# oss0430/SRFRD

Measured on NVIDIA B200. Metric: training seqs/sec; full-catalogue top-10 users/sec, higher is better.
Workload: dtype bf16

## Files before the change

### include/srfrd_b200.h

```cpp
#ifndef SRFRD_B200_H
#define SRFRD_B200_H

#include <stddef.h>
#include <stdint.h>

#ifdef __cplusplus
extern "C" {
#endif

#define SRFRD_ABI_VERSION 9
#if defined(__GNUC__)
#define SRFRD_API __attribute__((visibility("default")))
#else
#define SRFRD_API
#endif

SRFRD_API const char* srfrd_last_error(void);
SRFRD_API int srfrd_abi_version(void);
SRFRD_API int srfrd_device_check(void);

SRFRD_API int srfrd_embed_ln_fwd(const float* item_table, int64_t n_rows, int D, const float* pos_table,
                       const float* aux_table, int64_t n_aux, int F, int mode, const int64_t* seq,
                       const int64_t* aux_ids, int64_t B, int L, float item_scale, const float* ln_w,
                       const float* ln_b, float eps, void* x0_bf16, float* x0_f32, void* q_bf16, float* stats,
                       int ldx, float drop_p, uint64_t drop_seed, uint32_t drop_stream, const float* drop_step,
                       void* stream);

SRFRD_API int srfrd_srfu_labels(const int64_t* fake_ids, int64_t B, int L, int kind, int64_t* labels, void* stream);

SRFRD_API int srfrd_embed_bwd(const void* dx0_bf16, int ldx, const int64_t* seq, const int64_t* aux_ids, int64_t B, int L,
                    int D, int F, int mode, float item_scale, float* d_item, float* d_aux, void* stream);

SRFRD_API int srfrd_layernorm_fwd(const void* x_bf16, int ldx, const float* w, const float* b, float eps, void* y_bf16,
                        float* y_f32, int ldy, float* stats, int64_t T, int H, int64_t row_stride,
                        int64_t row_offset, void* stream);
SRFRD_API int srfrd_layernorm_bwd(const void* dy_bf16, const float* dy_f32, int lddy, const void* x_bf16, int ldx,
                        const float* stats, const float* w, const void* add_bf16, int ldadd,
                        const int64_t* row_ids, void* dx_bf16, int lddx, float* dw, float* db, int64_t T, int H,
                        void* stream);

typedef struct {
  const float* bias;
  const void* residual;
  const void* gate;
  const int64_t* row_ids;
  void* out_bf16;
  float* out_f32;
  int ldr, ldg, ldc;
  int relu;
  float drop_p;
  uint32_t drop_stream;
  uint64_t drop_seed;
  const float* drop_step;
  void* ln_out_bf16;
  const float* ln_w;
  const float* ln_b;
  float* ln_stats;
  int ld_ln;
  float ln_eps;
} srfrd_gemm_epilogue_t;

SRFRD_API int srfrd_gemm_tn(const void* A_bf16, int lda, const void* B_bf16, int ldb, int M, int N, int K,
                  const srfrd_gemm_epilogue_t* ep, void* stream);
SRFRD_API int srfrd_gemm_tn_plan(int M, int N, int K, int has_aux, int bf16_out, int fused_ln, int* out);
SRFRD_API int srfrd_gemm_debug_read(long long* host_dst);
SRFRD_API int srfrd_attn_debug_read(long long* host_dst);

SRFRD_API int srfrd_gemm_wgrad(const void* dY_bf16, int lda, const void* X_bf16, int ldb, int64_t T, int Mo, int No,
                     float* dW, int ldw, float* dbias, void* stream);
SRFRD_API int srfrd_gemm_ref(const void* A, int lda, const void* B, int ldb, float* C, int ldc, int M, int N, int K,
                   int a_mn_major, int b_mn_major, void* stream);

SRFRD_API int srfrd_colsum(const void* X_bf16, int64_t M, int N, int64_t ld, float* out, void* stream);
SRFRD_API int srfrd_add_segments(float* in, int64_t n, int seg_in, int seg_out, float* out, void* stream);

SRFRD_API int srfrd_dropout_apply(const void* x_bf16, int ldx, void* out_bf16, int ldo, int64_t M, int N, float drop_p,
                        uint64_t seed, uint32_t stream_id, const float* drop_step, void* stream);

typedef struct {
  const float* src; int src_ld;
  void* dst; int dst_ld;
  void* dst_t; int dst_t_ld;
  int rows, cols;
  int dst_is_f32;
} srfrd_cast_desc_t;
SRFRD_API int srfrd_cast_weights(const srfrd_cast_desc_t* descs_dev, int n, void* stream);
SRFRD_API int srfrd_f32_to_bf16_split(const float* src, int64_t src_ld, const int64_t* row_index, void* hi, void* lo,
                            int64_t rows, int cols, int dst_ld, void* stream);

SRFRD_API int srfrd_attention_fwd(const void* q, int ldq, const void* k, const void* v, int ldkv, void* o, int ldo,
                        float* stats, int64_t B, int L, int H, int heads, float drop_p, uint64_t seed, uint32_t stream_id,
                        const float* drop_step, void* stream);
SRFRD_API int srfrd_attention_bwd(const void* dout, int lddo, const void* q, int ldq, const void* k, const void* v, int ldkv,
                        const void* o, int ldo, float* stats, void* dq, int lddq, void* dk, void* dv, int lddkv, int64_t B,
                        int L, int H, int heads, float drop_p, uint64_t seed, uint32_t stream_id, const float* drop_step,
                        void* stream);

SRFRD_API int srfrd_score_fwd(const float* h, int ldh, const float* item_table, const float* fake_table, const int64_t* pos,
                    const int64_t* neg, const int64_t* prs, const int64_t* nrs, int64_t T, int D, int F, float* zp,
                    float* zn, void* stream);
SRFRD_API int srfrd_score_bwd(const float* h, int ldh, const float* item_table, const float* fake_table, const int64_t* pos,
                    const int64_t* neg, const int64_t* prs, const int64_t* nrs, const float* dzp, const float* dzn,
                    int64_t T, int D, int F, float* dh, int lddh, float* d_item, float* d_fake, void* stream);
SRFRD_API int srfrd_score_loss_fused(const float* h, int ldh, const float* item_table, const float* fake_table,
                           const int64_t* pos, const int64_t* neg, const int64_t* prs, const int64_t* nrs,
                           const float* w_pos, const float* w_neg, const float* norm, int64_t T, int D, int F,
                           float* zp, float* zn, float* loss_acc, float* dh, int lddh, float* d_item, float* d_fake,
                           void* stream);
SRFRD_API int srfrd_weight_sums(const int64_t* pos, const float* w_pos, const float* w_neg, int64_t T, float* out2,
                      void* stream);
SRFRD_API int srfrd_loss_finalize(float* acc2, const float* norm2, float* loss, void* stream);

SRFRD_API int srfrd_adam_tick(float* state3, float beta1, float beta2, void* stream);
SRFRD_API int srfrd_adam_step(float* p, float* g, float* m, float* v, int64_t n, float lr, float beta1, float beta2, float eps,
                    const float* state3, int zero_grad, void* stream);

SRFRD_API int srfrd_adam_step_fused(float* p, float* g, float* m, float* v, int64_t n, float lr, float beta1, float beta2,
                          float eps, float* state8, int zero_grad, float* acc2, const float* norm2, float* loss,
                          void* stream, const int64_t* l2_seg, int l2_n_seg, const float* l2_coef, const float* l2_reg);

SRFRD_API int srfrd_param_l2_plan(const int64_t* seg_host, int n_seg, int64_t* n_chunks);
SRFRD_API int srfrd_param_l2(const float* p, const int64_t* seg, int n_seg, int64_t n_chunks, float l2, float* coef,
                   float* reg, double* ws, void* stream);

#define SRFRD_TOPK_KMAX 64
SRFRD_API int srfrd_catalogue_topk_plan(int64_t U, int64_t n_rows, int64_t row_lo, int D, int n_split, int* chunks_out,
                                        int k);
SRFRD_API int srfrd_catalogue_topk_kmax(int D, int n_split, int* kmax_out);
SRFRD_API int srfrd_catalogue_topk(const void* feats_bf16, int64_t U, int64_t u_pad, int n_split, const void* table_bf16,
                         int64_t n_rows, int64_t row_lo, int64_t id_base, int D, int ld_feats, int ld_table,
                         int chunks, float* part_scores, int* part_ids, float* packed_out, void* stream, int k);
SRFRD_API int srfrd_merge_topk(const float* scores, const int* ids, int64_t U, int nlists, int k, float* out_scores,
                     int64_t* out_ids, void* stream);
SRFRD_API int srfrd_merge_topk_packed(const float* packed, int64_t U, int nlists, int k, float* out_scores,
                            int64_t* out_ids, void* stream);
SRFRD_API int srfrd_catalogue_rank(const void* feats_bf16, int64_t U, int64_t u_pad, int n_split,
                                   const void* table_bf16, int64_t n_rows, int64_t row_lo, int64_t id_base,
                                   int D, int ld_feats, int ld_table,
                                   const void* target_rows_bf16, int ld_target, const int64_t* target_ids,
                                   float* target_scores, int* rank_out, void* stream);

SRFRD_API int srfrd_sample_batch(const int64_t* offsets, const int* items, const int8_t* labels, const float* p_fake,
                       const int* eligible, int n_eligible, int itemnum, int B, int L, int policy, uint64_t seed,
                       const float* step, int64_t* users, int64_t* seq, int64_t* rsq, int64_t* pos, int64_t* prs,
                       int64_t* neg, int64_t* nrs, float* w_pos, void* stream);

SRFRD_API int srfrd_sample_candidates(const int64_t* offsets, const int* items, const int* users0, const int* target,
                            int64_t U, int itemnum, int C, uint64_t seed, int64_t* cand, void* stream);
SRFRD_API int srfrd_candidate_rank(const float* feats, int ldf, const float* item_table, int64_t n_rows, int D,
                         const int64_t* cand, int64_t U, int C, const float* fake_table, int F,
                         const int64_t* user_label, float* logits, int ldl, int* rank, int* err_flag, void* stream);
SRFRD_API int srfrd_add_user_term(float* logits, int ldl, int64_t U, int I, const float* feats_tail, int ldf,
                        const float* fake_table, const int64_t* label, int F, void* stream);

typedef struct {
  int* rows;
  int* cnt;
  int* seq_first;
  int* tok_row;
  int* row_tok;
  int64_t* row_ids;
  int* row_info;
  int* tile_row0;
  int* last_row;
  int64_t cap;
} srfrd_pack_t;
SRFRD_API int srfrd_pack_plan(const int64_t* seq, const int64_t* keep, int64_t B, int L, const srfrd_pack_t* pk, void* stream);
SRFRD_API int srfrd_set_row_limit(const int* rows_dev);
SRFRD_API int srfrd_embed_ln_fwd_packed(const float* item_table, int64_t n_rows, int D, const float* pos_table,
                              const float* aux_table, int64_t n_aux, int F, int mode, const int64_t* seq,
                              const int64_t* aux_ids, int64_t B, int L, float item_scale, const float* ln_w,
                              const float* ln_b, float eps, void* x0_bf16, void* q_bf16, float* stats, int ldx,
                              float drop_p, uint64_t drop_seed, uint32_t drop_stream, const float* drop_step,
                              const int* row_tok, const int* rows_dev, int64_t cap_rows, void* stream);
SRFRD_API int srfrd_layernorm_fwd_rows(const void* x_bf16, int ldx, const float* w, const float* b, float eps, float* y_f32,
                             int ldy, const int* row_index, int64_t n, int H, void* stream);
SRFRD_API int srfrd_attention_packed_supported(int L, int H, int heads);
SRFRD_API int srfrd_attention_packed_oproj_supported(int L, int H, int heads);
SRFRD_API int srfrd_attention_fwd_packed(const void* q, int ldq, const void* k, const void* v, int ldkv, void* o, int ldo,
                               const srfrd_pack_t* pk, int L, int H, int heads, float drop_p, uint64_t seed,
                               uint32_t stream_id, const float* drop_step, void* stream, const void* wo, int ldw,
                               const float* bo, const void* res, int ldres, const float* ln_w, const float* ln_b,
                               float ln_eps, float* ln_stats, void* r, int ldr, void* y, int ldy);
SRFRD_API int srfrd_attention_bwd_packed(const void* dout, int lddo, const void* q, int ldq, const void* k, const void* v,
                               int ldkv, void* dq, int lddq, void* dk, void* dv, int lddkv, const srfrd_pack_t* pk,
                               int L, int H, int heads, float drop_p, uint64_t seed, uint32_t stream_id,
                               const float* drop_step, void* stream, const void* dr, int lddr, const void* woT, int ldw);
SRFRD_API int srfrd_score_loss_fused_packed(const float* h, int ldh, const float* item_table, const float* fake_table,
                                  const int64_t* pos, const int64_t* neg, const int64_t* prs, const int64_t* nrs,
                                  const float* w_pos, const float* w_neg, const float* norm, int D, int F,
                                  float* loss_acc, float* dh, int lddh, float* d_item, float* d_fake,
                                  const int* row_tok, const int* rows_dev, int64_t cap_rows, void* stream);
SRFRD_API int srfrd_embed_bwd_packed(const void* dx0_bf16, int ldx, const int64_t* seq, const int64_t* aux_ids,
                           const int* row_tok, const int* rows_dev, int64_t cap_rows, int L, int D, int F, int mode,
                           float item_scale, float* d_item, float* d_aux, float* d_pos, void* stream);

typedef struct {
  const float* bias1; const float* bias2;
  const void* gate; int ldg;
  int relu1;
  float drop1_p, drop2_p; uint32_t drop1_stream, drop2_stream; uint64_t drop_seed; const float* drop_step;
  const void* residual; int ldr;
  int residual_is_a;
  const int64_t* row_ids;
  void* mid_out; int ldm;
  void* out; int ldc;
  void* ln_out; int ld_ln; const float* ln_w; const float* ln_b; float* ln_stats; float ln_eps;
} srfrd_mlp2_t;
SRFRD_API int srfrd_mlp2_tn(const void* A_bf16, int lda, const void* W1_bf16, int ldw1, const void* W2_bf16, int ldw2, int M, int N,
                  const srfrd_mlp2_t* ep, void* stream);

SRFRD_API int srfrd_attention_live_items(const int* tok_row, int64_t B, int L, int heads, int* q_lo, int* items, int* n_live,
                               void* stream);
SRFRD_API int srfrd_set_attention_live(const int* q_lo, const int* items, const int* n_live, const int* tok_row);

typedef struct {
  const void* src; int ld_s;
  void* dst; int ld_d;
  int W;
  int mode;
} srfrd_repack_part_t;
SRFRD_API int srfrd_unpack_rows(const srfrd_repack_part_t* parts, int n_parts, const srfrd_pack_t* pk, int64_t B, int L,
                      void* stream);
SRFRD_API int srfrd_pack_rows(const srfrd_repack_part_t* parts, int n_parts, const srfrd_pack_t* pk, int64_t B, int L,
                    void* stream);

SRFRD_API int srfrd_dp_adam_step(float* const* grad_ptrs_dev, float* const* param_ptrs_dev, uint32_t* const* signal_ptrs_dev,
                       int rank, int world, int64_t n, float* m, float* v, float lr, float beta1, float beta2, float eps,
                       float* state8, const float* norm2, uint32_t* local4, void* stream, const int64_t* l2_seg,
                       int l2_n_seg, const float* l2_coef, const float* l2_reg);

#ifdef __cplusplus
}
#endif
#endif
```

### srfrd_b200/_lib.py

```python
from __future__ import annotations

import ctypes as C
import os

_HERE = os.path.dirname(os.path.abspath(__file__))
LIB_PATH = os.environ.get("SRFRD_B200_LIB") or os.path.join(_HERE, "lib", "libsrfrd_b200.so")

vp, i32, i64, f32, u32, u64 = C.c_void_p, C.c_int, C.c_int64, C.c_float, C.c_uint32, C.c_uint64


class GemmEpilogue(C.Structure):
    _fields_ = [("bias", vp), ("residual", vp), ("gate", vp), ("row_ids", vp), ("out_bf16", vp), ("out_f32", vp),
                ("ldr", i32), ("ldg", i32), ("ldc", i32), ("relu", i32), ("drop_p", f32), ("drop_stream", u32),
                ("drop_seed", u64), ("drop_step", vp),
                ("ln_out_bf16", vp), ("ln_w", vp), ("ln_b", vp), ("ln_stats", vp), ("ld_ln", i32), ("ln_eps", f32)]


class CastDesc(C.Structure):
    _fields_ = [("src", vp), ("src_ld", i32), ("dst", vp), ("dst_ld", i32), ("dst_t", vp), ("dst_t_ld", i32),
                ("rows", i32), ("cols", i32), ("dst_is_f32", i32)]


class Mlp2Epilogue(C.Structure):
    _fields_ = [("bias1", vp), ("bias2", vp), ("gate", vp), ("ldg", i32), ("relu1", i32), ("drop1_p", f32), ("drop2_p", f32),
                ("drop1_stream", u32), ("drop2_stream", u32), ("drop_seed", u64), ("drop_step", vp), ("residual", vp), ("ldr", i32),
                ("residual_is_a", i32), ("row_ids", vp), ("mid_out", vp), ("ldm", i32), ("out", vp), ("ldc", i32),
                ("ln_out", vp), ("ld_ln", i32), ("ln_w", vp), ("ln_b", vp), ("ln_stats", vp), ("ln_eps", f32)]


class PackDesc(C.Structure):
    _fields_ = [("rows", vp), ("cnt", vp), ("seq_first", vp), ("tok_row", vp), ("row_tok", vp), ("row_ids", vp),
                ("row_info", vp), ("tile_row0", vp), ("last_row", vp), ("cap", i64)]


class RepackPart(C.Structure):
    _fields_ = [("src", vp), ("ld_s", i32), ("dst", vp), ("ld_d", i32), ("W", i32), ("mode", i32)]


SIGNATURES = {
    "srfrd_abi_version": [],
    "srfrd_device_check": [],
    "srfrd_embed_ln_fwd": [vp, i64, i32, vp, vp, i64, i32, i32, vp, vp, i64, i32, f32, vp, vp, f32, vp, vp, vp, vp, i32,
                           f32, u64, u32, vp, vp],
    "srfrd_srfu_labels": [vp, i64, i32, i32, vp, vp],
    "srfrd_embed_bwd": [vp, i32, vp, vp, i64, i32, i32, i32, i32, f32, vp, vp, vp],
    "srfrd_layernorm_fwd": [vp, i32, vp, vp, f32, vp, vp, i32, vp, i64, i32, i64, i64, vp],
    "srfrd_layernorm_bwd": [vp, vp, i32, vp, i32, vp, vp, vp, i32, vp, vp, i32, vp, vp, i64, i32, vp],
    "srfrd_gemm_tn": [vp, i32, vp, i32, i32, i32, i32, C.POINTER(GemmEpilogue), vp],
    "srfrd_mlp2_tn": [vp, i32, vp, i32, vp, i32, i32, i32, C.POINTER(Mlp2Epilogue), vp],
    "srfrd_gemm_tn_plan": [i32, i32, i32, i32, i32, i32, vp],
    "srfrd_gemm_debug_read": [vp],
    "srfrd_attn_debug_read": [vp],
    "srfrd_gemm_wgrad": [vp, i32, vp, i32, i64, i32, i32, vp, i32, vp, vp],
    "srfrd_gemm_ref": [vp, i32, vp, i32, vp, i32, i32, i32, i32, i32, i32, vp],
    "srfrd_colsum": [vp, i64, i32, i64, vp, vp],
    "srfrd_add_segments": [vp, i64, i32, i32, vp, vp],
    "srfrd_dropout_apply": [vp, i32, vp, i32, i64, i32, f32, u64, u32, vp, vp],
    "srfrd_cast_weights": [vp, i32, vp],
    "srfrd_f32_to_bf16_split": [vp, i64, vp, vp, vp, i64, i32, i32, vp],
    "srfrd_attention_fwd": [vp, i32, vp, vp, i32, vp, i32, vp, i64, i32, i32, i32, f32, u64, u32, vp, vp],
    "srfrd_attention_bwd": [vp, i32, vp, i32, vp, vp, i32, vp, i32, vp, vp, i32, vp, vp, i32, i64, i32, i32, i32, f32, u64,
                            u32, vp, vp],
    "srfrd_score_fwd": [vp, i32, vp, vp, vp, vp, vp, vp, i64, i32, i32, vp, vp, vp],
    "srfrd_score_bwd": [vp, i32, vp, vp, vp, vp, vp, vp, vp, vp, i64, i32, i32, vp, i32, vp, vp, vp],
    "srfrd_score_loss_fused": [vp, i32, vp, vp, vp, vp, vp, vp, vp, vp, vp, i64, i32, i32, vp, vp, vp, vp, i32, vp, vp, vp],
    "srfrd_weight_sums": [vp, vp, vp, i64, vp, vp],
    "srfrd_loss_finalize": [vp, vp, vp, vp],
    "srfrd_adam_tick": [vp, f32, f32, vp],
    "srfrd_adam_step": [vp, vp, vp, vp, i64, f32, f32, f32, f32, vp, i32, vp],
    "srfrd_adam_step_fused": [vp, vp, vp, vp, i64, f32, f32, f32, f32, vp, i32, vp, vp, vp, vp, vp, i32, vp, vp],
    "srfrd_param_l2_plan": [C.POINTER(i64), i32, C.POINTER(i64)],
    "srfrd_param_l2": [vp, vp, i32, i64, f32, vp, vp, vp, vp],
    "srfrd_catalogue_topk_plan": [i64, i64, i64, i32, i32, C.POINTER(i32), i32],
    "srfrd_catalogue_topk_kmax": [i32, i32, C.POINTER(i32)],
    "srfrd_catalogue_topk": [vp, i64, i64, i32, vp, i64, i64, i64, i32, i32, i32, i32, vp, vp, vp, vp, i32],
    "srfrd_merge_topk_packed": [vp, i64, i32, i32, vp, vp, vp],
    "srfrd_catalogue_rank": [vp, i64, i64, i32, vp, i64, i64, i64, i32, i32, i32, vp, i32, vp, vp, vp, vp],
    "srfrd_attention_live_items": [vp, i64, i32, i32, vp, vp, vp, vp],
    "srfrd_set_attention_live": [vp, vp, vp, vp],
    "srfrd_merge_topk": [vp, vp, i64, i32, i32, vp, vp, vp],
    "srfrd_unpack_rows": [C.POINTER(RepackPart), i32, C.POINTER(PackDesc), i64, i32, vp],
    "srfrd_pack_rows": [C.POINTER(RepackPart), i32, C.POINTER(PackDesc), i64, i32, vp],
    "srfrd_dp_adam_step": [vp, vp, vp, i32, i32, i64, vp, vp, f32, f32, f32, f32, vp, vp, vp, vp, vp, i32, vp, vp],
    "srfrd_pack_plan": [vp, vp, i64, i32, C.POINTER(PackDesc), vp],
    "srfrd_set_row_limit": [vp],
    "srfrd_embed_ln_fwd_packed": [vp, i64, i32, vp, vp, i64, i32, i32, vp, vp, i64, i32, f32, vp, vp, f32, vp, vp, vp, i32,
                                  f32, u64, u32, vp, vp, vp, i64, vp],
    "srfrd_layernorm_fwd_rows": [vp, i32, vp, vp, f32, vp, i32, vp, i64, i32, vp],
    "srfrd_attention_packed_supported": [i32, i32, i32],
    "srfrd_attention_packed_oproj_supported": [i32, i32, i32],
    "srfrd_attention_fwd_packed": [vp, i32, vp, vp, i32, vp, i32, C.POINTER(PackDesc), i32, i32, i32, f32, u64, u32, vp, vp,
                                   vp, i32, vp, vp, i32, vp, vp, f32, vp, vp, i32, vp, i32],
    "srfrd_attention_bwd_packed": [vp, i32, vp, i32, vp, vp, i32, vp, i32, vp, vp, i32, C.POINTER(PackDesc), i32, i32, i32,
                                   f32, u64, u32, vp, vp, vp, i32, vp, i32],
    "srfrd_score_loss_fused_packed": [vp, i32, vp, vp, vp, vp, vp, vp, vp, vp, vp, i32, i32, vp, vp, i32, vp, vp, vp, vp,
                                      i64, vp],
    "srfrd_embed_bwd_packed": [vp, i32, vp, vp, vp, vp, i64, i32, i32, i32, i32, f32, vp, vp, vp, vp],
    "srfrd_sample_candidates": [vp, vp, vp, vp, i64, i32, i32, u64, vp, vp],
    "srfrd_candidate_rank": [vp, i32, vp, i64, i32, vp, i64, i32, vp, i32, vp, vp, i32, vp, vp, vp],
    "srfrd_add_user_term": [vp, i32, i64, i32, vp, i32, vp, vp, i32, vp],
    "srfrd_sample_batch": [vp, vp, vp, vp, vp, i32, i32, i32, i32, i32, u64, vp, vp, vp, vp, vp, vp, vp, vp, vp, vp],
}

_lib = None
_device_ok = False
launch_count = 0


def load() -> C.CDLL:
    global _lib
    if _lib is not None:
        return _lib
    if not os.path.exists(LIB_PATH):
        raise RuntimeError(
            f"srfrd_b200: {LIB_PATH} is not built. Run `make -C srfrd_b200/csrc` (needs nvcc, sm_100a). "
            "There is no CPU fallback.")
    lib = C.CDLL(LIB_PATH)
    lib.srfrd_last_error.restype = C.c_char_p
    lib.srfrd_last_error.argtypes = []
    for name, argtypes in SIGNATURES.items():
        fn = getattr(lib, name)
        fn.argtypes = argtypes
        fn.restype = C.c_int
    if lib.srfrd_abi_version() != 9:
        raise RuntimeError("srfrd_b200: ABI version mismatch between _lib.py and the built library")
    _lib = lib
    return lib


def require_device() -> None:
    global _device_ok
    if _device_ok:
        return
    lib = load()
    if lib.srfrd_device_check() != 0:
        raise RuntimeError("srfrd_b200: " + lib.srfrd_last_error().decode())
    _device_ok = True


_profile = None


def set_profile(records) -> None:
    global _profile
    _profile = records


def call(name: str, *args) -> None:
    global launch_count
    lib = _lib or load()
    if _profile is not None:
        import torch
        e0, e1 = torch.cuda.Event(enable_timing=True), torch.cuda.Event(enable_timing=True)
        e0.record()
        rc = getattr(lib, name)(*args)
        e1.record()
        _profile.append((name, args, e0, e1))
    else:
        rc = getattr(lib, name)(*args)
    if rc != 0:
        raise RuntimeError(f"{name}: {lib.srfrd_last_error().decode()}")
    launch_count += 1
```

### srfrd_b200/csrc/ffn.cu

```cuda
#include <stdlib.h>

#include "common.cuh"
#include "srfrd_b200.h"

namespace srfrd {

static constexpr int MLP_THREADS = 160;
static constexpr int MT = 128;
static constexpr int MBLK = MT * 64 * 2;

struct MlpParams {
  int M, N, kb;
  int K, kbk;
  int single;
  int relu2; const bf16* gate2; int ldg2;
  const int* rows_dev;
  const float *bias1, *bias2;
  const bf16* gate; int ldg;
  int relu1;
  uint64_t drop_seed; const float* drop_step;
  uint32_t thresh1, thresh2, stream1, stream2; float scale1, scale2;
  const bf16* residual; int ldr;
  int residual_is_a;
  const int64_t* row_ids;
  const float *ln_w, *ln_b; float* ln_stats; float ln_eps; int has_ln;
};

__device__ __forceinline__ uint32_t swz_chunk(int r, int j) { return (uint32_t)(r * 128 + ((j ^ (r & 7)) << 4)); }
__device__ __forceinline__ void mlp_bar_sync() { asm volatile("bar.sync 1, 128;" ::: "memory"); }
__device__ __forceinline__ void mlp_tma_store(const CUtensorMap* tmap, const void* smem_src, int c0, int c1) {
  asm volatile("cp.async.bulk.tensor.2d.global.shared::cta.bulk_group [%0, {%2, %3}], [%1];" ::"l"(tmap),
               "r"(smem_u32(smem_src)), "r"(c0), "r"(c1)
               : "memory");
}
__device__ __forceinline__ void unpack8_bf16(const uint4& u, float* f) {
  const uint32_t w[4] = {u.x, u.y, u.z, u.w};
#pragma unroll
  for (int i = 0; i < 4; ++i) { f[2 * i] = __uint_as_float(w[i] << 16); f[2 * i + 1] = __uint_as_float(w[i] & 0xffff0000u); }
}

__global__ void __launch_bounds__(MLP_THREADS, 2)
mlp2_kernel(const __grid_constant__ CUtensorMap tmA, const __grid_constant__ CUtensorMap tmW1,
            const __grid_constant__ CUtensorMap tmW2, const __grid_constant__ CUtensorMap tmMid,
            const __grid_constant__ CUtensorMap tmOut, const __grid_constant__ CUtensorMap tmLn, MlpParams p) {
  extern __shared__ uint8_t smem_raw[];
  uint8_t* smem = reinterpret_cast<uint8_t*>((reinterpret_cast<uintptr_t>(smem_raw) + 1023) & ~uintptr_t(1023));
  const int wblk = (p.N * 128 + 1023) & ~1023;
  const int ablk = max(p.kb, p.kbk);
  uint8_t* sW1 = smem;
  uint8_t* sW2 = sW1 + p.kbk * wblk;
  uint8_t* sA = sW2 + (p.single ? 0 : p.kb) * wblk;
  uint8_t* sM = sA + ablk * MBLK;
  float* sb1 = reinterpret_cast<float*>(sM + p.kb * MBLK);
  float* sb2 = sb1 + 128;
  float* slw = sb2 + 128;
  float* slb = slw + 128;
  uint64_t* bars = reinterpret_cast<uint64_t*>(slb + 128);
  uint64_t *w_full = bars, *a_full = bars + 1, *a_free = bars + 2, *acc1_full = bars + 3, *mid_ready = bars + 4,
           *acc2_full = bars + 5;
  uint32_t* tmem_slot = reinterpret_cast<uint32_t*>(bars + 6);
  const int warp = threadIdx.x >> 5, lane = threadIdx.x & 31;

  if (warp == 4 && lane == 0) {
    tma_prefetch_desc(&tmA); tma_prefetch_desc(&tmW1); tma_prefetch_desc(&tmW2); tma_prefetch_desc(&tmMid);
    tma_prefetch_desc(&tmOut);
    if (p.has_ln) tma_prefetch_desc(&tmLn);
    mbar_init(w_full, 1); mbar_init(a_full, 1); mbar_init(a_free, 1); mbar_init(acc1_full, 1); mbar_init(mid_ready, 1);
    mbar_init(acc2_full, 1);
    fence_barrier_init();
  }
  if (warp == 4) { tmem_alloc(tmem_slot, 256); tmem_relinquish(); }
  pdl_prologue_done();
  const int M = p.rows_dev ? min(p.M, __ldg(p.rows_dev)) : p.M;
  const int n_tiles = (M + MT - 1) / MT;
  for (int i = threadIdx.x; i < 128; i += blockDim.x) {
    sb1[i] = (p.bias1 && i < p.N) ? __ldg(p.bias1 + i) : 0.f;
    sb2[i] = (p.bias2 && i < p.N) ? __ldg(p.bias2 + i) : 0.f;
    slw[i] = (p.has_ln && i < p.N) ? __ldg(p.ln_w + i) : 0.f;
    slb[i] = (p.has_ln && i < p.N) ? __ldg(p.ln_b + i) : 0.f;
  }
  tc_fence_before();
  __syncthreads();
  tc_fence_after();
  const uint32_t tmem_base = *tmem_slot;
  const uint32_t tAcc1 = tmem_base, tAcc2 = tmem_base + 128;

  if (warp == 4) {
    if ((int)blockIdx.x < n_tiles && elect_one()) {
      mbar_expect_tx(w_full, (p.kbk + (p.single ? 0 : p.kb)) * p.N * 128);
      for (int kb = 0; kb < p.kbk; ++kb) tma_load_2d(sW1 + kb * wblk, &tmW1, w_full, kb * 64, 0, SRFRD_EVICT_LAST);
      if (!p.single)
        for (int kb = 0; kb < p.kb; ++kb) tma_load_2d(sW2 + kb * wblk, &tmW2, w_full, kb * 64, 0, SRFRD_EVICT_LAST);
    }
    __syncwarp();
    const uint32_t idesc = umma_idesc_bf16(MT, p.N, 0, 0);
    const uint64_t dA = umma_smem_desc(smem_u32(sA), 0, 1024), dM = umma_smem_desc(smem_u32(sM), 0, 1024);
    const uint64_t dW1 = umma_smem_desc(smem_u32(sW1), 0, 1024), dW2 = umma_smem_desc(smem_u32(sW2), 0, 1024);
    uint32_t ph = 0;
    for (int tile = blockIdx.x; tile < n_tiles; tile += gridDim.x, ph ^= 1) {
      mbar_wait(a_free, ph ^ 1);
      if (elect_one()) {
        mbar_expect_tx(a_full, p.kbk * MBLK);
        for (int kb = 0; kb < p.kbk; ++kb) tma_load_2d(sA + kb * MBLK, &tmA, a_full, kb * 64, tile * MT, SRFRD_EVICT_FIRST);
      }
      __syncwarp();
      if (tile == (int)blockIdx.x) mbar_wait(w_full, 0);
      mbar_wait(a_full, ph);
      tc_fence_after();
      if (elect_one()) {
        for (int kb = 0; kb < p.kbk; ++kb) {
          const int ksteps = min(4, (p.K - kb * 64 + 15) / 16);
          for (int k = 0; k < ksteps; ++k)
            umma_bf16(p.single ? tAcc2 : tAcc1, dA + (uint64_t)(kb * (MBLK >> 4) + 2 * k),
                      dW1 + (uint64_t)(kb * (wblk >> 4) + 2 * k), idesc, (kb | k) != 0);
        }
        umma_commit(p.single ? acc2_full : acc1_full);
      }
      __syncwarp();
      if (p.single) continue;
      mbar_wait(mid_ready, ph);
      tc_fence_after();
      if (elect_one()) {
        for (int kb = 0; kb < p.kb; ++kb) {
          const int ksteps = min(4, (p.N - kb * 64 + 15) / 16);
          for (int k = 0; k < ksteps; ++k)
            umma_bf16(tAcc2, dM + (uint64_t)(kb * (MBLK >> 4) + 2 * k), dW2 + (uint64_t)(kb * (wblk >> 4) + 2 * k), idesc, (kb | k) != 0);
        }
        umma_commit(acc2_full);
      }
      __syncwarp();
    }
  } else {
    const int r = warp * 32 + lane;
    const uint32_t lane_off = (uint32_t)(warp * 32) << 16;
    const uint64_t seed = (p.thresh1 | p.thresh2) ? mix_seed(p.drop_seed, p.drop_step) : 0;
    const bool issuer = threadIdx.x == 0;
    uint32_t ph = 0;
    for (int tile = blockIdx.x; tile < n_tiles; tile += gridDim.x, ph ^= 1) {
      const int64_t row = (int64_t)tile * MT + r;
      const bool rok = row < M;
      if (!p.single) {
      mbar_wait(acc1_full, ph);
      tc_fence_after();
#pragma unroll 1
      for (int c = 0; c < p.N; c += 16) {
        uint32_t raw[16];
        tmem_ld16(tAcc1 + lane_off + c, raw);
        uint4 g0 = make_uint4(0, 0, 0, 0), g1 = g0;
        if (p.gate && rok) {
          const uint4* gp = reinterpret_cast<const uint4*>(p.gate + row * p.ldg + c);
          g0 = __ldg(gp); g1 = __ldg(gp + 1);
        }
        tmem_ld_wait();
        float v[16], gv[16];
        if (p.gate) { unpack8_bf16(g0, gv); unpack8_bf16(g1, gv + 8); }
#pragma unroll
        for (int i = 0; i < 16; ++i) {
          float x = __uint_as_float(raw[i]) + sb1[c + i];
          if (p.thresh1)
            x = dropout_keep(seed, p.stream1, (uint64_t)row * (uint64_t)p.N + (uint64_t)(c + i), p.thresh1) ? x * p.scale1 : 0.f;
          if (p.relu1) x = fmaxf(x, 0.f);
          if (p.gate) x = gv[i] > 0.f ? x : 0.f;
          v[i] = x;
        }
        uint8_t* blk = sM + (c >> 6) * MBLK;
        const int j = (c & 63) >> 3;
        *reinterpret_cast<uint4*>(blk + swz_chunk(r, j)) =
            make_uint4(pack_bf16x2(v[0], v[1]), pack_bf16x2(v[2], v[3]), pack_bf16x2(v[4], v[5]), pack_bf16x2(v[6], v[7]));
        *reinterpret_cast<uint4*>(blk + swz_chunk(r, j + 1)) =
            make_uint4(pack_bf16x2(v[8], v[9]), pack_bf16x2(v[10], v[11]), pack_bf16x2(v[12], v[13]), pack_bf16x2(v[14], v[15]));
      }
      tc_fence_before();
      fence_proxy_async();
      mlp_bar_sync();
      if (issuer) {
        mbar_arrive(mid_ready);
        for (int kb = 0; kb < p.kb; ++kb) mlp_tma_store(&tmMid, sM + kb * MBLK, kb * 64, tile * MT);
        asm volatile("cp.async.bulk.commit_group;" ::: "memory");
      }
      }
      const float rowm = (p.row_ids && rok) ? ((__ldg(p.row_ids + row) != 0) ? 1.f : 0.f) : 1.f;
      mbar_wait(acc2_full, ph);
      tc_fence_after();
      float ln_sum = 0.f, ln_sq = 0.f;
#pragma unroll 1
      for (int c = 0; c < p.N; c += 16) {
        uint32_t raw[16];
        tmem_ld16(tAcc2 + lane_off + c, raw);
        uint8_t* blk = sA + (c >> 6) * MBLK;
        const int j = (c & 63) >> 3;
        uint4 r0 = make_uint4(0, 0, 0, 0), r1 = r0;
        if (p.residual_is_a && c < p.K) {
          r0 = *reinterpret_cast<const uint4*>(blk + swz_chunk(r, j));
          r1 = *reinterpret_cast<const uint4*>(blk + swz_chunk(r, j + 1));
        } else if (p.residual && rok) {
          const uint4* rp = reinterpret_cast<const uint4*>(p.residual + row * p.ldr + c);
          r0 = __ldg(rp); r1 = __ldg(rp + 1);
        }
        uint4 q0 = make_uint4(0, 0, 0, 0), q1 = q0;
        if (p.gate2 && rok) {
          const uint4* gp = reinterpret_cast<const uint4*>(p.gate2 + row * p.ldg2 + c);
          q0 = __ldg(gp); q1 = __ldg(gp + 1);
        }
        tmem_ld_wait();
        float v[16], rv[16], gv2[16];
        unpack8_bf16(r0, rv); unpack8_bf16(r1, rv + 8);
        if (p.gate2) { unpack8_bf16(q0, gv2); unpack8_bf16(q1, gv2 + 8); }
#pragma unroll
        for (int i = 0; i < 16; ++i) {
          float x = __uint_as_float(raw[i]) + sb2[c + i];
          if (p.thresh2)
            x = dropout_keep(seed, p.stream2, (uint64_t)row * (uint64_t)p.N + (uint64_t)(c + i), p.thresh2) ? x * p.scale2 : 0.f;
          if (p.relu2) x = fmaxf(x, 0.f);
          if (p.gate2) x = gv2[i] > 0.f ? x : 0.f;
          x += rv[i];
          v[i] = x * rowm;
        }
        const uint4 p0 = make_uint4(pack_bf16x2(v[0], v[1]), pack_bf16x2(v[2], v[3]), pack_bf16x2(v[4], v[5]), pack_bf16x2(v[6], v[7]));
        const uint4 p1 = make_uint4(pack_bf16x2(v[8], v[9]), pack_bf16x2(v[10], v[11]), pack_bf16x2(v[12], v[13]), pack_bf16x2(v[14], v[15]));
        *reinterpret_cast<uint4*>(blk + swz_chunk(r, j)) = p0;
        *reinterpret_cast<uint4*>(blk + swz_chunk(r, j + 1)) = p1;
        if (p.has_ln) {
          float q[16];
          unpack8_bf16(p0, q); unpack8_bf16(p1, q + 8);
#pragma unroll
          for (int i = 0; i < 16; ++i) { ln_sum += q[i]; ln_sq = fmaf(q[i], q[i], ln_sq); }
        }
      }
      tc_fence_before();
      if (p.has_ln) {
        if (issuer) asm volatile("cp.async.bulk.wait_group.read 0;" ::: "memory");
        mlp_bar_sync();
        const float invn = 1.f / (float)p.N;
        const float mean = ln_sum * invn;
        const float var = fmaxf(ln_sq * invn - mean * mean, 0.f);
        const float rstd = rsqrtf(var + p.ln_eps), nb = -mean * rstd;
#pragma unroll 1
        for (int c = 0; c < p.N; c += 8) {
          const int j = (c & 63) >> 3;
          const uint4 xv = *reinterpret_cast<const uint4*>(sA + (c >> 6) * MBLK + swz_chunk(r, j));
          float q[8], y[8];
          unpack8_bf16(xv, q);
#pragma unroll
          for (int i = 0; i < 8; ++i) y[i] = fmaf(fmaf(q[i], rstd, nb), slw[c + i], slb[c + i]);
          *reinterpret_cast<uint4*>(sM + (c >> 6) * MBLK + swz_chunk(r, j)) =
              make_uint4(pack_bf16x2(y[0], y[1]), pack_bf16x2(y[2], y[3]), pack_bf16x2(y[4], y[5]), pack_bf16x2(y[6], y[7]));
        }
        if (p.ln_stats && rok) *reinterpret_cast<float2*>(p.ln_stats + 2 * row) = make_float2(mean, rstd);
      }
      fence_proxy_async();
      mlp_bar_sync();
      if (issuer) {
        for (int kb = 0; kb < p.kb; ++kb) mlp_tma_store(&tmOut, sA + kb * MBLK, kb * 64, tile * MT);
        if (p.has_ln)
          for (int kb = 0; kb < p.kb; ++kb) mlp_tma_store(&tmLn, sM + kb * MBLK, kb * 64, tile * MT);
        asm volatile("cp.async.bulk.commit_group;" ::: "memory");
        asm volatile("cp.async.bulk.wait_group.read 0;" ::: "memory");
        mbar_arrive(a_free);
      }
    }
    if (issuer) asm volatile("cp.async.bulk.wait_group 0;" ::: "memory");
  }
  tc_fence_before();
  __syncthreads();
  if (warp == 4) { tc_fence_after(); tmem_dealloc(tmem_base, 256); }
}

}

using namespace srfrd;

static int mlp_launch(MlpParams& p, const void* A, int lda, const void* W1, int ldw1, const void* W2, int ldw2, void* mid_out,
                      int ldm, void* out, int ldc, void* ln_out, int ld_ln, cudaStream_t stream) {
  p.kb = (p.N + 63) / 64; p.kbk = (p.K + 63) / 64; p.rows_dev = row_limit();
  p.has_ln = ln_out != nullptr;
  CUtensorMap tmA, tmW1, tmW2, tmMid, tmOut, tmLn;
  if (int rc = make_tmap_bf16_2d(&tmA, A, p.M, p.K, lda, MT, 64)) return rc;
  if (int rc = make_tmap_bf16_2d(&tmW1, W1, p.N, p.K, ldw1, p.N, 64)) return rc;
  tmW2 = tmW1; tmMid = tmA;
  if (!p.single) {
    if (int rc = make_tmap_bf16_2d(&tmW2, W2, p.N, p.N, ldw2, p.N, 64)) return rc;
    if (int rc = make_tmap_bf16_2d(&tmMid, mid_out, p.M, p.N, ldm, MT, 64)) return rc;
  }
  if (int rc = make_tmap_bf16_2d(&tmOut, out, p.M, p.N, ldc, MT, 64)) return rc;
  tmLn = tmOut;
  if (p.has_ln) if (int rc = make_tmap_bf16_2d(&tmLn, ln_out, p.M, p.N, ld_ln, MT, 64)) return rc;
  const int wblk = (p.N * 128 + 1023) & ~1023;
  const int ablk = p.kb > p.kbk ? p.kb : p.kbk;
  const size_t smem = 1024 + (size_t)(p.kbk + (p.single ? 0 : p.kb)) * wblk + (size_t)(ablk + p.kb) * MBLK + 4 * 128 * sizeof(float) + 128;
  static bool attr = false;
  if (!attr) {
    SRFRD_CUDA(cudaFuncSetAttribute(mlp2_kernel, cudaFuncAttributeMaxDynamicSharedMemorySize, 200 * 1024));
    attr = true;
  }
  SRFRD_REQUIRE(smem <= 200 * 1024, "mlp2_tn: shared memory %zu too large", smem);
  int64_t grid = ((int64_t)p.M + MT - 1) / MT;
  if (grid > 2 * num_sms()) grid = 2 * num_sms();
  SRFRD_CUDA(launch_pdl(mlp2_kernel, dim3((unsigned)grid), dim3(MLP_THREADS), smem, stream, tmA, tmW1, tmW2, tmMid, tmOut, tmLn, p));
  SRFRD_LAUNCH_CHECK();
  return 0;
}

namespace srfrd {
bool gemm_small_eligible(int M, int N, int K, const srfrd_gemm_epilogue_t* ep, int lda, int ldb) {
  if (!ep->out_bf16 || ep->out_f32 || N > 128 || N % 16 || K > 128 || K % 8 || lda % 8 || ldb % 8 || ep->ldc % 8) return false;
  if (((uintptr_t)ep->out_bf16 & 15) || (ep->residual && (ep->ldr % 8 || ((uintptr_t)ep->residual & 15)))) return false;
  if (ep->gate && (ep->ldg % 8 || ((uintptr_t)ep->gate & 15))) return false;
  if (ep->residual && ep->gate) return false;
  if (ep->ln_out_bf16 && (!ep->ln_w || !ep->ln_b || ep->ld_ln % 8 || ((uintptr_t)ep->ln_out_bf16 & 15))) return false;
  { const char* e = getenv("SRFRD_LEAN_GEMM"); if (!e || e[0] != '1') return false; }
  return row_limit() != nullptr || M <= 32768;
}
int gemm_small_launch(const void* A, int lda, const void* B, int ldb, int M, int N, int K, const srfrd_gemm_epilogue_t* ep,
                      cudaStream_t stream) {
  MlpParams p = {};
  p.M = M; p.N = N; p.K = K; p.single = 1;
  p.bias2 = ep->bias; p.relu2 = ep->relu; p.gate2 = (const bf16*)ep->gate; p.ldg2 = ep->ldg;
  p.residual = (const bf16*)ep->residual; p.ldr = ep->ldr;
  p.residual_is_a = (ep->residual == A && ep->ldr == lda && N <= K) ? 1 : 0;
  if (p.residual_is_a) p.residual = nullptr;
  p.row_ids = ep->row_ids;
  p.drop_seed = ep->drop_seed; p.drop_step = ep->drop_step; p.stream2 = ep->drop_stream;
  p.thresh2 = ep->drop_p > 0.f ? (uint32_t)((double)ep->drop_p * 4294967296.0) : 0;
  p.scale2 = ep->drop_p > 0.f ? 1.f / (1.f - ep->drop_p) : 1.f;
  p.scale1 = 1.f;
  p.ln_w = ep->ln_w; p.ln_b = ep->ln_b; p.ln_stats = ep->ln_stats; p.ln_eps = ep->ln_eps;
  return mlp_launch(p, A, lda, B, ldb, nullptr, 0, nullptr, 0, ep->out_bf16, ep->ldc, ep->ln_out_bf16, ep->ld_ln, stream);
}
}

extern "C" int srfrd_mlp2_tn(const void* A, int lda, const void* W1, int ldw1, const void* W2, int ldw2, int M, int N,
                             const srfrd_mlp2_t* ep, void* stream_) {
  cudaStream_t stream = (cudaStream_t)stream_;
  SRFRD_REQUIRE(A && W1 && W2 && ep && ep->mid_out && ep->out, "mlp2_tn: null pointer");
  SRFRD_REQUIRE(M > 0 && N >= 16 && N <= 128 && N % 16 == 0, "mlp2_tn: N = K must be a multiple of 16 up to 128 (got %d)", N);
  SRFRD_REQUIRE(lda % 8 == 0 && ldw1 % 8 == 0 && ldw2 % 8 == 0 && ep->ldm % 8 == 0 && ep->ldc % 8 == 0 && lda >= N && ldw1 >= N &&
                    ldw2 >= N && ep->ldm >= N && ep->ldc >= N, "mlp2_tn: bad leading dimensions");
  SRFRD_REQUIRE(!ep->gate || (ep->ldg % 8 == 0 && ((uintptr_t)ep->gate & 15) == 0), "mlp2_tn: bad gate");
  SRFRD_REQUIRE(!ep->residual || (ep->ldr % 8 == 0 && ((uintptr_t)ep->residual & 15) == 0), "mlp2_tn: bad residual");
  SRFRD_REQUIRE(!ep->ln_out || (ep->ln_w && ep->ln_b && ep->ld_ln % 8 == 0 && ep->ld_ln >= N), "mlp2_tn: bad LayerNorm arguments");
  SRFRD_REQUIRE(ep->drop1_p >= 0.f && ep->drop1_p < 1.f && ep->drop2_p >= 0.f && ep->drop2_p < 1.f, "mlp2_tn: dropout p must be in [0, 1)");
  MlpParams p = {};
  p.M = M; p.N = N; p.K = N; p.single = 0;
  p.bias1 = ep->bias1; p.bias2 = ep->bias2; p.gate = (const bf16*)ep->gate; p.ldg = ep->ldg; p.relu1 = ep->relu1;
  p.drop_seed = ep->drop_seed; p.drop_step = ep->drop_step; p.stream1 = ep->drop1_stream; p.stream2 = ep->drop2_stream;
  p.thresh1 = ep->drop1_p > 0.f ? (uint32_t)((double)ep->drop1_p * 4294967296.0) : 0;
  p.thresh2 = ep->drop2_p > 0.f ? (uint32_t)((double)ep->drop2_p * 4294967296.0) : 0;
  p.scale1 = ep->drop1_p > 0.f ? 1.f / (1.f - ep->drop1_p) : 1.f;
  p.scale2 = ep->drop2_p > 0.f ? 1.f / (1.f - ep->drop2_p) : 1.f;
  p.residual = (const bf16*)ep->residual; p.ldr = ep->ldr;
  p.residual_is_a = (ep->residual == nullptr && ep->residual_is_a) || (ep->residual == A && ep->ldr == lda);
  if (p.residual_is_a) p.residual = nullptr;
  p.row_ids = ep->row_ids;
  p.ln_w = ep->ln_w; p.ln_b = ep->ln_b; p.ln_stats = ep->ln_stats; p.ln_eps = ep->ln_eps;
  return mlp_launch(p, A, lda, W1, ldw1, W2, ldw2, ep->mid_out, ep->ldm, ep->out, ep->ldc, ep->ln_out, ep->ld_ln, stream);
}
```

### srfrd_b200/csrc/loss_scatter_adam.cu

```cuda
#include "common.cuh"
#include "srfrd_b200.h"

namespace srfrd {

static constexpr int MAXC = 16;

struct ScoreParams {
  const float* h; int ldh;
  const float* item_table;
  const float* fake_table;
  const int64_t *pos, *neg, *prs, *nrs;
  const float *w_pos, *w_neg;
  const float* norm;
  const float *dzp_in, *dzn_in;
  float *zp, *zn;
  float* loss_acc;
  float* dh; int lddh;
  float* d_item; float* d_fake;
  int64_t T; int D, F;
  int mode;
  const int* row_tok;
  const int* rows_dev;
  int group;
};

__device__ __forceinline__ float softplus(float x) { return fmaxf(x, 0.f) + log1pf(__expf(-fabsf(x))); }
__device__ __forceinline__ float sigmoidf(float x) { return 1.f / (1.f + __expf(-x)); }

template <int NC>
__global__ void __launch_bounds__(256, (NC <= 9 ? 2 : 1)) score_kernel(ScoreParams p) {
  __shared__ float red[2][8];
  pdl_prologue_done();
  const int lane = threadIdx.x & 31, warp = threadIdx.x >> 5, nw = blockDim.x >> 5;
  const int64_t warp0 = (int64_t)blockIdx.x * nw + warp, nwarps = (int64_t)gridDim.x * nw;
  const int W = p.D + (p.fake_table ? p.F : 0);
  float lp_acc = 0.f, ln_acc = 0.f;
  float inv_np = 0.f, inv_nn = 0.f;
  if (p.mode == 1) {
    const float a = __ldg(p.norm), b = __ldg(p.norm + 1);
    inv_np = a > 0.f ? 1.f / a : 0.f;
    inv_nn = b > 0.f ? 1.f / b : 0.f;
  }
  float fk1[NC], fk2[NC];
#pragma unroll
  for (int i = 0; i < NC; ++i) fk1[i] = fk2[i] = 0.f;
  const bool dh_vec = p.dh && (p.lddh == W) && (W % 4 == 0) && ((reinterpret_cast<uintptr_t>(p.dh) & 15) == 0);
  if (p.rows_dev) p.T = min(p.T, (int64_t)__ldg(p.rows_dev));
  const int G = p.group;
  for (int64_t t0 = warp0 * G; t0 < p.T; t0 += nwarps * G) {
    const int64_t tl = t0 + lane;
    bool in = lane < G && tl < p.T;
    int my_tok = 0;
    if (p.row_tok && in) { my_tok = __ldg(p.row_tok + tl); in = my_tok >= 0; }
    const int64_t my_src = p.row_tok ? (int64_t)my_tok : tl;
    int64_t my_pid = 0, my_nid = 0, my_pf = 0, my_nf = 0;
    float my_a = 0.f, my_b = 0.f;
    bool my_active = false;
    if (in) {
      my_pid = __ldg(p.pos + my_src);
      my_nid = __ldg(p.neg + my_src);
      if (p.mode == 1) {
        my_a = p.w_pos ? __ldg(p.w_pos + my_src) : (my_pid != 0 ? 1.f : 0.f);
        my_b = p.w_neg ? __ldg(p.w_neg + my_src) : my_a;
        my_active = (my_a != 0.f) || (my_b != 0.f) || p.zp;
      } else if (p.mode == 2) {
        my_a = __ldg(p.dzp_in + my_src);
        my_b = __ldg(p.dzn_in + my_src);
        my_active = (my_a != 0.f) || (my_b != 0.f);
      } else {
        my_active = true;
      }
      if (p.fake_table && my_active) { my_pf = __ldg(p.prs + my_src); my_nf = __ldg(p.nrs + my_src); }
    }
    unsigned mask = __ballot_sync(0xffffffffu, my_active);
    if (p.dh) {
      const int nrow = (int)min((int64_t)G, p.T - t0);
      if (dh_vec) {
        const int per_row = W >> 2, total = nrow * per_row;
        float4* base = reinterpret_cast<float4*>(p.dh + t0 * p.lddh);
        for (int i = lane; i < total; i += 32)
          if (!((mask >> (i / per_row)) & 1u)) base[i] = make_float4(0.f, 0.f, 0.f, 0.f);
      } else {
        for (int r = 0; r < nrow; ++r) {
          if ((mask >> r) & 1u) continue;
          for (int c = lane; c < W; c += 32) p.dh[(t0 + r) * p.lddh + c] = 0.f;
        }
      }
    }
    struct Tok {
      int64_t t, tsrc, pid, nid; int pf, nf; float ta, tb;
      float hv[NC], ep[NC], en[NC];
    };
    auto fetch = [&](Tok& k, int r) {
      k.t = t0 + r;
      k.tsrc = p.row_tok ? (int64_t)__shfl_sync(0xffffffffu, my_tok, r) : k.t;
      k.pid = __shfl_sync(0xffffffffu, my_pid, r); k.nid = __shfl_sync(0xffffffffu, my_nid, r);
      k.pf = (int)__shfl_sync(0xffffffffu, (int)my_pf, r); k.nf = (int)__shfl_sync(0xffffffffu, (int)my_nf, r);
      k.ta = __shfl_sync(0xffffffffu, my_a, r); k.tb = __shfl_sync(0xffffffffu, my_b, r);
#pragma unroll
      for (int i = 0; i < NC; ++i) {
        const int c = lane + 32 * i;
        k.hv[i] = k.ep[i] = k.en[i] = 0.f;
        if (c < W) {
          k.hv[i] = p.h[k.t * p.ldh + c];
          if (c < p.D) {
            k.ep[i] = __ldg(p.item_table + k.pid * p.D + c);
            k.en[i] = __ldg(p.item_table + k.nid * p.D + c);
          } else {
            k.ep[i] = __ldg(p.fake_table + (int64_t)k.pf * p.F + (c - p.D));
            k.en[i] = __ldg(p.fake_table + (int64_t)k.nf * p.F + (c - p.D));
          }
        }
      }
    };
    auto finish = [&](const Tok& k) {
      float sp = 0.f, sn = 0.f;
#pragma unroll
      for (int i = 0; i < NC; ++i) { sp = fmaf(k.hv[i], k.ep[i], sp); sn = fmaf(k.hv[i], k.en[i], sn); }
      const float zp = warp_sum(sp), zn = warp_sum(sn);
      if (p.zp && lane == 0) { p.zp[k.tsrc] = zp; p.zn[k.tsrc] = zn; }
      if (p.mode == 0) return;
      float dzp = k.ta, dzn = k.tb;
      if (p.mode == 1) {
        lp_acc += k.ta * softplus(-zp);
        ln_acc += k.tb * softplus(zn);
        dzp = k.ta * (sigmoidf(zp) - 1.f) * inv_np;
        dzn = k.tb * sigmoidf(zn) * inv_nn;
      }
#pragma unroll
      for (int i = 0; i < NC; ++i) {
        const int c = lane + 32 * i;
        if (c < W) {
          if (p.dh) p.dh[k.t * p.lddh + c] = dzp * k.ep[i] + dzn * k.en[i];
          if (c < p.D) {
            if (p.d_item && k.pid != 0 && dzp != 0.f) red_add_f32(p.d_item + k.pid * p.D + c, dzp * k.hv[i]);
            if (p.d_item && k.nid != 0 && dzn != 0.f) red_add_f32(p.d_item + k.nid * p.D + c, dzn * k.hv[i]);
          } else {
            const float gp = dzp * k.hv[i], gn = dzn * k.hv[i];
            fk1[i] += (k.pf == 1 ? gp : 0.f) + (k.nf == 1 ? gn : 0.f);
            fk2[i] += (k.pf == 2 ? gp : 0.f) + (k.nf == 2 ? gn : 0.f);
          }
        }
      }
    };
    if (NC <= 4) {
      if (mask) {
        Tok cur, nxt;
        { const int r = __ffs(mask) - 1; mask &= mask - 1; fetch(cur, r); }
        while (true) {
          const bool more = mask != 0;
          if (more) { const int r = __ffs(mask) - 1; mask &= mask - 1; fetch(nxt, r); }
          finish(cur);
          if (!more) break;
          cur = nxt;
        }
      }
    } else {
      while (mask) {
        const int r = __ffs(mask) - 1;
        mask &= mask - 1;
        Tok cur;
        fetch(cur, r);
        finish(cur);
      }
    }
  }
  if (p.d_fake) {
#pragma unroll
    for (int i = 0; i < NC; ++i) {
      const int c = lane + 32 * i;
      if (c >= p.D && c < W) {
        if (fk1[i] != 0.f) red_add_f32(p.d_fake + 1 * p.F + (c - p.D), fk1[i]);
        if (fk2[i] != 0.f) red_add_f32(p.d_fake + 2 * p.F + (c - p.D), fk2[i]);
      }
    }
  }
  if (p.mode == 1 && p.loss_acc) {
    if (lane == 0) { red[0][warp] = lp_acc; red[1][warp] = ln_acc; }
    __syncthreads();
    if (threadIdx.x == 0) {
      float a = 0.f, b = 0.f;
      for (int w = 0; w < nw; ++w) { a += red[0][w]; b += red[1][w]; }
      red_add_f32(p.loss_acc, a);
      red_add_f32(p.loss_acc + 1, b);
    }
  }
}

__global__ void __launch_bounds__(256) weight_sums_kernel(const int64_t* pos, const float* w_pos, const float* w_neg,
                                                          int64_t T, float* out) {
  __shared__ float red[2][8];
  float a = 0.f, b = 0.f;
  for (int64_t t = (int64_t)blockIdx.x * blockDim.x + threadIdx.x; t < T; t += (int64_t)gridDim.x * blockDim.x) {
    const float wp = w_pos ? w_pos[t] : (pos[t] != 0 ? 1.f : 0.f);
    a += wp;
    b += w_neg ? w_neg[t] : wp;
  }
  a = warp_sum(a); b = warp_sum(b);
  const int lane = threadIdx.x & 31, warp = threadIdx.x >> 5;
  if (lane == 0) { red[0][warp] = a; red[1][warp] = b; }
  __syncthreads();
  if (threadIdx.x == 0) {
    a = b = 0.f;
    for (int w = 0; w < (int)(blockDim.x >> 5); ++w) { a += red[0][w]; b += red[1][w]; }
    red_add_f32(out, a);
    red_add_f32(out + 1, b);
  }
}

__global__ void loss_finalize_kernel(float* acc, const float* norm, float* loss) {
  pdl_prologue_done();
  const float a = norm[0] > 0.f ? acc[0] / norm[0] : 0.f;
  const float b = norm[1] > 0.f ? acc[1] / norm[1] : 0.f;
  loss[0] = a + b;
  acc[0] = 0.f; acc[1] = 0.f;
}

struct EmbedBwdParams {
  const bf16* dx0; int ldx;
  const int64_t* seq;
  const int64_t* aux_ids;
  int L, D, F, mode;
  float item_scale;
  float* d_item;
  float* d_aux;
};

__global__ void embed_bwd_kernel(EmbedBwdParams p) {
  extern __shared__ int64_t ids[];
  pdl_prologue_done();
  const int64_t b = blockIdx.x;
  const int c = threadIdx.x;
  const int H = p.D + (p.mode == 1 ? p.F : 0);
  for (int l = threadIdx.x; l < p.L; l += blockDim.x) {
    ids[l] = p.seq[b * p.L + l];
    ids[p.L + l] = (p.mode == 1 && p.aux_ids) ? p.aux_ids[b * p.L + l] : 0;
  }
  __syncthreads();
  if (c >= H) return;
  float acc1 = 0.f, acc2 = 0.f, accu = 0.f;
  for (int l = 0; l < p.L; ++l) {
    const int64_t id = ids[l];
    if (id == 0) continue;
    const float v = bf2f(p.dx0[(b * p.L + l) * p.ldx + c]);
    if (c < p.D) {
      red_add_f32(p.d_item + id * p.D + c, v * p.item_scale);
      accu += v;
    } else {
      const int64_t f = ids[p.L + l];
      if (f == 1) acc1 += v;
      else if (f == 2) acc2 += v;
    }
  }
  if (p.mode == 1 && c >= p.D && p.d_aux) {
    if (acc1 != 0.f) red_add_f32(p.d_aux + 1 * p.F + (c - p.D), acc1);
    if (acc2 != 0.f) red_add_f32(p.d_aux + 2 * p.F + (c - p.D), acc2);
  }
  if (p.mode == 2 && c < p.D && p.d_aux && accu != 0.f)
    red_add_f32(p.d_aux + p.aux_ids[b] * p.D + c, accu);
}

static constexpr int EB_SLICE = 64;
__global__ void __launch_bounds__(512) embed_bwd_packed_kernel(EmbedBwdParams p, const int* row_tok, const int* rows_dev, int64_t cap,
                                                              float* d_pos) {
  extern __shared__ float spos[];
  pdl_prologue_done();
  const int x = threadIdx.x, y = threadIdx.y, RPB = blockDim.y;
  const int c = blockIdx.y * EB_SLICE + x;
  const int H = p.D + (p.mode == 1 ? p.F : 0);
  const int tid = y * blockDim.x + x, nthr = blockDim.x * blockDim.y;
  const bool pos_slice = blockIdx.y * EB_SLICE < p.D;
  if (pos_slice) for (int i = tid; i < p.L * EB_SLICE; i += nthr) spos[i] = 0.f;
  __syncthreads();
  const int64_t M = min(cap, (int64_t)__ldg(rows_dev));
  float acc1 = 0.f, acc2 = 0.f;
  for (int64_t r = (int64_t)blockIdx.x * RPB + y; r < M; r += (int64_t)gridDim.x * RPB) {
    const int tok = __ldg(row_tok + r);
    if (tok < 0 || c >= H) continue;
    const int64_t id = __ldg(p.seq + tok);
    if (id == 0) continue;
    const float v = bf2f(p.dx0[r * p.ldx + c]);
    if (c < p.D) {
      red_add_f32(p.d_item + id * p.D + c, v * p.item_scale);
      atomicAdd(&spos[(tok % p.L) * EB_SLICE + x], v);
      if (p.mode == 2 && p.d_aux) red_add_f32(p.d_aux + p.aux_ids[tok / p.L] * p.D + c, v);
    } else if (p.aux_ids) {
      const int64_t f = __ldg(p.aux_ids + tok);
      if (f == 1) acc1 += v;
      else if (f == 2) acc2 += v;
    }
  }
  if (p.mode == 1 && c >= p.D && c < H && p.d_aux) {
    if (acc1 != 0.f) red_add_f32(p.d_aux + 1 * p.F + (c - p.D), acc1);
    if (acc2 != 0.f) red_add_f32(p.d_aux + 2 * p.F + (c - p.D), acc2);
  }
  __syncthreads();
  if (d_pos && pos_slice)
    for (int i = tid; i < p.L * EB_SLICE; i += nthr) {
      const int l = i / EB_SLICE, cc = blockIdx.y * EB_SLICE + i % EB_SLICE;
      if (cc < p.D && spos[i] != 0.f) red_add_f32(d_pos + l * p.D + cc, spos[i]);
    }
}

__global__ void add_segments_kernel(float* in, int64_t n, int seg_in, int seg_out, float* out) {
  pdl_prologue_done();
  const int64_t i = (int64_t)blockIdx.x * blockDim.x + threadIdx.x;
  if (i >= n) return;
  const int c = (int)(i % seg_in);
  if (c < seg_out) out[(i / seg_in) * seg_out + c] += in[i];
  in[i] = 0.f;
}

__global__ void adam_tick_kernel(float* state, float beta1, float beta2) {
  pdl_prologue_done();
  const float step = state[0] + 1.f;
  state[0] = step;
  state[1] = (float)(1.0 - pow((double)beta1, (double)step));
  state[2] = (float)(1.0 - pow((double)beta2, (double)step));
  state[3] = __uint_as_float(__float_as_uint(state[3]) + 1u);
}

static constexpr int64_t L2_CHUNK = 8192;

__device__ __forceinline__ void l2_chunk_prefix(const int64_t* seg, int n_seg, int64_t* s_c0) {
  const int t = threadIdx.x;
  s_c0[t + 1] = t < n_seg ? (seg[2 * t + 1] + L2_CHUNK - 1) / L2_CHUNK : 0;
  if (t == 0) s_c0[0] = 0;
  __syncthreads();
  for (int d = 1; d < L2_THREADS; d <<= 1) {
    const int64_t a = t >= d ? s_c0[t + 1 - d] : 0;
    __syncthreads();
    s_c0[t + 1] += a;
    __syncthreads();
  }
}

__device__ __forceinline__ double block_sum_f64(double x, double* s_red) {
#pragma unroll
  for (int o = 16; o > 0; o >>= 1) x += __shfl_xor_sync(0xffffffffu, x, o);
  if ((threadIdx.x & 31) == 0) s_red[threadIdx.x >> 5] = x;
  __syncthreads();
  double s = 0.0;
  if (threadIdx.x == 0)
    for (int w = 0; w < L2_THREADS / 32; ++w) s += s_red[w];
  __syncthreads();
  return s;
}

__global__ void __launch_bounds__(L2_THREADS) param_l2_kernel(const float* __restrict__ p, const int64_t* __restrict__ seg,
                                                               int n_seg, int64_t n_chunks, float l2, float* coef, float* reg,
                                                               double* ws) {
  __shared__ int64_t s_c0[L2_THREADS + 1];
  __shared__ double s_red[L2_THREADS / 32];
  __shared__ double s_norm[L2_THREADS];
  __shared__ bool s_last;
  pdl_prologue_done();
  l2_chunk_prefix(seg, n_seg, s_c0);
  double* part = ws + 1;
  for (int64_t c = blockIdx.x; c < n_chunks; c += gridDim.x) {
    int lo = 0, hi = n_seg - 1;
    while (lo < hi) {
      const int mid = (lo + hi + 1) >> 1;
      if (s_c0[mid] <= c) lo = mid; else hi = mid - 1;
    }
    const int64_t off = seg[2 * lo], numel = seg[2 * lo + 1];
    const int64_t b = (c - s_c0[lo]) * L2_CHUNK;
    const int64_t e = min(numel, b + L2_CHUNK);
    const float4* p4 = reinterpret_cast<const float4*>(p + off);
    double acc = 0.0;
#pragma unroll
    for (int k = 0; k < (int)(L2_CHUNK / 4 / L2_THREADS); ++k) {
      const int64_t j = b + 4 * ((int64_t)k * L2_THREADS + threadIdx.x);
      if (j < e) {
        const float4 x = __ldcg(p4 + j / 4);
        const float xs[4] = {x.x, x.y, x.z, x.w};
#pragma unroll
        for (int q = 0; q < 4; ++q)
          if (j + q < e) acc = fma((double)xs[q], (double)xs[q], acc);
      }
    }
    const double s = block_sum_f64(acc, s_red);
    if (threadIdx.x == 0) part[c] = s;
  }
  __threadfence();
  __syncthreads();
  if (threadIdx.x == 0) s_last = atomicAdd(reinterpret_cast<unsigned*>(ws), 1u) == gridDim.x - 1;
  __syncthreads();
  if (!s_last) return;
  __threadfence();
  const int warp = threadIdx.x >> 5, lane = threadIdx.x & 31;
  for (int t = warp; t < n_seg; t += L2_THREADS / 32) {
    double s = 0.0;
    for (int64_t c = s_c0[t] + lane; c < s_c0[t + 1]; c += 32) s += __ldcg(part + c);
#pragma unroll
    for (int o = 16; o > 0; o >>= 1) s += __shfl_xor_sync(0xffffffffu, s, o);
    if (lane == 0) {
      const double nrm = sqrt(s);
      s_norm[t] = nrm;
      coef[t] = nrm > 0.0 ? (float)((double)l2 / nrm) : 0.f;
    }
  }
  __syncthreads();
  if (threadIdx.x == 0) {
    double tot = 0.0;
    for (int t = 0; t < n_seg; ++t) tot += s_norm[t];
    reg[0] = (float)((double)l2 * tot);
    *reinterpret_cast<unsigned*>(ws) = 0u;
  }
}

template <bool L2>
__global__ void __launch_bounds__(256) adam_fused_kernel(float* __restrict__ p, float* __restrict__ g, float* __restrict__ m,
                                                         float* __restrict__ v, int64_t n, float lr, float beta1, float beta2,
                                                         float eps, float* state, int zero_grad, float* acc, const float* norm,
                                                         float* loss, L2Segments l2s) {
  __shared__ float s_bc[2];
  pdl_prologue_done();
  if (threadIdx.x == 0) {
    const float step = state[0] + 1.f;
    s_bc[0] = (float)(1.0 - pow((double)beta1, (double)step));
    s_bc[1] = (float)(1.0 - pow((double)beta2, (double)step));
  }
  if (blockIdx.x == 0 && threadIdx.x == 32 && acc) {
    const float a = norm[0] > 0.f ? acc[0] / norm[0] : 0.f;
    const float b = norm[1] > 0.f ? acc[1] / norm[1] : 0.f;
    if constexpr (L2) loss[0] = a + b + l2s.reg[0];
    else loss[0] = a + b;
    acc[0] = 0.f; acc[1] = 0.f;
  }
  int64_t* s_off = nullptr;
  float* s_coef = nullptr;
  if constexpr (L2) {
    s_off = l2_smem().off;
    s_coef = l2_smem().coef;
    l2_load_starts(l2s, s_off, s_coef);
  }
  __syncthreads();
  const float step_size = lr / s_bc[0];
  const float inv_sqrt_bc2 = rsqrtf(s_bc[1]);
  const int64_t n4 = n >> 2;
  int t = 0;
  if constexpr (L2) t = l2_find(s_off, l2s.n_seg, (int64_t)blockIdx.x * blockDim.x + threadIdx.x);
  for (int64_t i = (int64_t)blockIdx.x * blockDim.x + threadIdx.x; i < n4; i += (int64_t)gridDim.x * blockDim.x) {
    float4 pp = reinterpret_cast<float4*>(p)[i], gg = reinterpret_cast<float4*>(g)[i];
    float4 mm = reinterpret_cast<float4*>(m)[i], vv = reinterpret_cast<float4*>(v)[i];
    float* pa = &pp.x; float* ga = &gg.x; float* ma = &mm.x; float* va = &vv.x;
    if constexpr (L2) {
      t = l2_advance(s_off, l2s.n_seg, t, i);
      const float c = s_coef[t];
#pragma unroll
      for (int j = 0; j < 4; ++j) ga[j] += c * pa[j];
    }
#pragma unroll
    for (int j = 0; j < 4; ++j) {
      ma[j] = beta1 * ma[j] + (1.f - beta1) * ga[j];
      va[j] = beta2 * va[j] + (1.f - beta2) * ga[j] * ga[j];
      pa[j] -= step_size * ma[j] / (sqrtf(va[j]) * inv_sqrt_bc2 + eps);
    }
    reinterpret_cast<float4*>(p)[i] = pp;
    reinterpret_cast<float4*>(m)[i] = mm;
    reinterpret_cast<float4*>(v)[i] = vv;
    if (zero_grad) reinterpret_cast<float4*>(g)[i] = make_float4(0.f, 0.f, 0.f, 0.f);
  }
  if (blockIdx.x == 0 && threadIdx.x < (n & 3)) {
    const int64_t i = (n4 << 2) + threadIdx.x;
    m[i] = beta1 * m[i] + (1.f - beta1) * g[i];
    v[i] = beta2 * v[i] + (1.f - beta2) * g[i] * g[i];
    p[i] -= step_size * m[i] / (sqrtf(v[i]) * inv_sqrt_bc2 + eps);
    if (zero_grad) g[i] = 0.f;
  }
  __syncthreads();
  if (threadIdx.x == 0) {
    int* done = reinterpret_cast<int*>(state + 4);
    if (atomicAdd(done, 1) == (int)gridDim.x - 1) {
      *done = 0;
      state[0] = state[0] + 1.f;
      state[1] = s_bc[0];
      state[2] = s_bc[1];
      state[3] = __uint_as_float(__float_as_uint(state[3]) + 1u);
    }
  }
}

__global__ void __launch_bounds__(256) adam_kernel(float* __restrict__ p, float* __restrict__ g, float* __restrict__ m,
                                                   float* __restrict__ v, int64_t n, float lr, float beta1, float beta2,
                                                   float eps, const float* __restrict__ state, int zero_grad) {
  pdl_prologue_done();
  const float step_size = lr / state[1];
  const float inv_sqrt_bc2 = rsqrtf(state[2]);
  const int64_t n4 = n >> 2;
  for (int64_t i = (int64_t)blockIdx.x * blockDim.x + threadIdx.x; i < n4; i += (int64_t)gridDim.x * blockDim.x) {
    float4 pp = reinterpret_cast<float4*>(p)[i], gg = reinterpret_cast<float4*>(g)[i];
    float4 mm = reinterpret_cast<float4*>(m)[i], vv = reinterpret_cast<float4*>(v)[i];
    float* pa = &pp.x; float* ga = &gg.x; float* ma = &mm.x; float* va = &vv.x;
#pragma unroll
    for (int j = 0; j < 4; ++j) {
      ma[j] = beta1 * ma[j] + (1.f - beta1) * ga[j];
      va[j] = beta2 * va[j] + (1.f - beta2) * ga[j] * ga[j];
      pa[j] -= step_size * ma[j] / (sqrtf(va[j]) * inv_sqrt_bc2 + eps);
    }
    reinterpret_cast<float4*>(p)[i] = pp;
    reinterpret_cast<float4*>(m)[i] = mm;
    reinterpret_cast<float4*>(v)[i] = vv;
    if (zero_grad) reinterpret_cast<float4*>(g)[i] = make_float4(0.f, 0.f, 0.f, 0.f);
  }
  if (blockIdx.x == 0 && threadIdx.x < (n & 3)) {
    const int64_t i = (n4 << 2) + threadIdx.x;
    m[i] = beta1 * m[i] + (1.f - beta1) * g[i];
    v[i] = beta2 * v[i] + (1.f - beta2) * g[i] * g[i];
    p[i] -= step_size * m[i] / (sqrtf(v[i]) * inv_sqrt_bc2 + eps);
    if (zero_grad) g[i] = 0.f;
  }
}

}

using namespace srfrd;

static int score_launch(ScoreParams& p, void* stream) {
  const int W = p.D + (p.fake_table ? p.F : 0);
  SRFRD_REQUIRE(W <= 32 * MAXC, "score: width %d unsupported", W);
  if (p.T == 0) return 0;
  if (p.group != 8) p.group = 32;
  int64_t blocks = (p.T + 8 * p.group - 1) / (8 * p.group);
  const int64_t cap = (int64_t)num_sms() * 8;
  if (blocks > cap) blocks = cap;
  const int nc = (W + 31) / 32;
#define SCORE_CALL(NC) SRFRD_CUDA(launch_pdl(score_kernel<NC>, dim3((unsigned)blocks), dim3(256), 0, (cudaStream_t)stream, p))
  if (nc <= 1) SCORE_CALL(1);
  else if (nc <= 2) SCORE_CALL(2);
  else if (nc <= 3) SCORE_CALL(3);
  else if (nc <= 4) SCORE_CALL(4);
  else if (nc <= 6) SCORE_CALL(6);
  else if (nc <= 9) SCORE_CALL(9);
  else SCORE_CALL(MAXC);
#undef SCORE_CALL
  SRFRD_LAUNCH_CHECK();
  return 0;
}

extern "C" int srfrd_score_fwd(const float* h, int ldh, const float* item_table, const float* fake_table,
                               const int64_t* pos, const int64_t* neg, const int64_t* prs, const int64_t* nrs,
                               int64_t T, int D, int F, float* zp, float* zn, void* stream) {
  SRFRD_REQUIRE(h && item_table && pos && neg && zp && zn, "score_fwd: null pointer");
  SRFRD_REQUIRE(!fake_table || (prs && nrs), "score_fwd: fake ids required with a fake table");
  ScoreParams p = {};
  p.h = h; p.ldh = ldh; p.item_table = item_table; p.fake_table = fake_table; p.pos = pos; p.neg = neg; p.prs = prs;
  p.nrs = nrs; p.T = T; p.D = D; p.F = F; p.zp = zp; p.zn = zn; p.mode = 0;
  return score_launch(p, stream);
}

extern "C" int srfrd_score_bwd(const float* h, int ldh, const float* item_table, const float* fake_table,
                               const int64_t* pos, const int64_t* neg, const int64_t* prs, const int64_t* nrs,
                               const float* dzp, const float* dzn, int64_t T, int D, int F, float* dh, int lddh,
                               float* d_item, float* d_fake, void* stream) {
  SRFRD_REQUIRE(h && item_table && pos && neg && dzp && dzn && dh, "score_bwd: null pointer");
  SRFRD_REQUIRE(!fake_table || (prs && nrs), "score_bwd: fake ids required with a fake table");
  ScoreParams p = {};
  p.h = h; p.ldh = ldh; p.item_table = item_table; p.fake_table = fake_table; p.pos = pos; p.neg = neg; p.prs = prs;
  p.nrs = nrs; p.T = T; p.D = D; p.F = F; p.dzp_in = dzp; p.dzn_in = dzn; p.dh = dh; p.lddh = lddh; p.d_item = d_item;
  p.d_fake = d_fake; p.mode = 2;
  return score_launch(p, stream);
}

extern "C" int srfrd_score_loss_fused(const float* h, int ldh, const float* item_table, const float* fake_table,
                                      const int64_t* pos, const int64_t* neg, const int64_t* prs, const int64_t* nrs,
                                      const float* w_pos, const float* w_neg, const float* norm, int64_t T, int D,
                                      int F, float* zp, float* zn, float* loss_acc, float* dh, int lddh, float* d_item,
                                      float* d_fake, void* stream) {
  SRFRD_REQUIRE(h && item_table && pos && neg && norm && loss_acc, "score_loss_fused: null pointer");
  SRFRD_REQUIRE(!fake_table || (prs && nrs), "score_loss_fused: fake ids required with a fake table");
  SRFRD_REQUIRE((zp == nullptr) == (zn == nullptr), "score_loss_fused: pass both logit outputs or neither");
  ScoreParams p = {};
  p.h = h; p.ldh = ldh; p.item_table = item_table; p.fake_table = fake_table; p.pos = pos; p.neg = neg; p.prs = prs;
  p.nrs = nrs; p.w_pos = w_pos; p.w_neg = w_neg; p.norm = norm; p.T = T; p.D = D; p.F = F; p.zp = zp; p.zn = zn;
  p.loss_acc = loss_acc; p.dh = dh; p.lddh = lddh; p.d_item = d_item; p.d_fake = d_fake; p.mode = 1;
  return score_launch(p, stream);
}

extern "C" int srfrd_score_loss_fused_packed(const float* h, int ldh, const float* item_table, const float* fake_table,
                                             const int64_t* pos, const int64_t* neg, const int64_t* prs, const int64_t* nrs,
                                             const float* w_pos, const float* w_neg, const float* norm, int D, int F,
                                             float* loss_acc, float* dh, int lddh, float* d_item, float* d_fake,
                                             const int* row_tok, const int* rows_dev, int64_t cap_rows, void* stream) {
  SRFRD_REQUIRE(h && item_table && pos && neg && norm && loss_acc && row_tok && rows_dev, "score_loss_fused_packed: null pointer");
  SRFRD_REQUIRE(!fake_table || (prs && nrs), "score_loss_fused_packed: fake ids required with a fake table");
  ScoreParams p = {};
  p.h = h; p.ldh = ldh; p.item_table = item_table; p.fake_table = fake_table; p.pos = pos; p.neg = neg; p.prs = prs;
  p.nrs = nrs; p.w_pos = w_pos; p.w_neg = w_neg; p.norm = norm; p.T = cap_rows; p.D = D; p.F = F;
  p.loss_acc = loss_acc; p.dh = dh; p.lddh = lddh; p.d_item = d_item; p.d_fake = d_fake; p.mode = 1;
  p.row_tok = row_tok; p.rows_dev = rows_dev; p.group = 8;
  return score_launch(p, stream);
}

extern "C" int srfrd_weight_sums(const int64_t* pos, const float* w_pos, const float* w_neg, int64_t T, float* out2,
                                 void* stream) {
  SRFRD_REQUIRE(pos && out2, "weight_sums: null pointer");
  SRFRD_CUDA(cudaMemsetAsync(out2, 0, 2 * sizeof(float), (cudaStream_t)stream));
  if (T == 0) return 0;
  int64_t blocks = (T + 2047) / 2048;
  if (blocks > num_sms() * 2) blocks = num_sms() * 2;
  weight_sums_kernel<<<(unsigned)blocks, 256, 0, (cudaStream_t)stream>>>(pos, w_pos, w_neg, T, out2);
  SRFRD_LAUNCH_CHECK();
  return 0;
}

extern "C" int srfrd_loss_finalize(float* acc2, const float* norm2, float* loss, void* stream) {
  SRFRD_REQUIRE(acc2 && norm2 && loss, "loss_finalize: null pointer");
  SRFRD_CUDA(launch_pdl(loss_finalize_kernel, dim3(1), dim3(1), 0, (cudaStream_t)stream, acc2, norm2, loss));
  SRFRD_LAUNCH_CHECK();
  return 0;
}

extern "C" int srfrd_embed_bwd(const void* dx0, int ldx, const int64_t* seq, const int64_t* aux_ids, int64_t B, int L,
                               int D, int F, int mode, float item_scale, float* d_item, float* d_aux, void* stream) {
  SRFRD_REQUIRE(dx0 && seq && d_item, "embed_bwd: null pointer");
  SRFRD_REQUIRE(mode >= 0 && mode <= 2, "embed_bwd: bad mode");
  SRFRD_REQUIRE(mode != 2 || aux_ids, "embed_bwd: labels required for mode 2");
  const int H = D + (mode == 1 ? F : 0);
  SRFRD_REQUIRE(H <= 1024, "embed_bwd: width %d unsupported", H);
  if (B == 0) return 0;
  EmbedBwdParams p;
  p.dx0 = (const bf16*)dx0; p.ldx = ldx; p.seq = seq; p.aux_ids = aux_ids; p.L = L; p.D = D; p.F = F; p.mode = mode;
  p.item_scale = item_scale; p.d_item = d_item; p.d_aux = d_aux;
  const int threads = (H + 31) & ~31;
  SRFRD_CUDA(launch_pdl(embed_bwd_kernel, dim3((unsigned)B), dim3(threads), 2 * L * sizeof(int64_t), (cudaStream_t)stream, p));
  SRFRD_LAUNCH_CHECK();
  return 0;
}

extern "C" int srfrd_embed_bwd_packed(const void* dx0, int ldx, const int64_t* seq, const int64_t* aux_ids,
                                      const int* row_tok, const int* rows_dev, int64_t cap_rows, int L, int D, int F,
                                      int mode, float item_scale, float* d_item, float* d_aux, float* d_pos, void* stream) {
  SRFRD_REQUIRE(dx0 && seq && d_item && row_tok && rows_dev, "embed_bwd_packed: null pointer");
  SRFRD_REQUIRE(mode >= 0 && mode <= 2, "embed_bwd_packed: bad mode");
  SRFRD_REQUIRE(mode != 2 || aux_ids, "embed_bwd_packed: labels required for mode 2");
  const int H = D + (mode == 1 ? F : 0);
  SRFRD_REQUIRE(H <= 512, "embed_bwd_packed: width %d unsupported", H);
  if (cap_rows == 0) return 0;
  EmbedBwdParams p;
  p.dx0 = (const bf16*)dx0; p.ldx = ldx; p.seq = seq; p.aux_ids = aux_ids; p.L = L; p.D = D; p.F = F; p.mode = mode;
  p.item_scale = item_scale; p.d_item = d_item; p.d_aux = d_aux;
  const int slices = (H + EB_SLICE - 1) / EB_SLICE;
  const int tx = EB_SLICE, ty = 8;
  const size_t smem = (size_t)L * EB_SLICE * sizeof(float);
  SRFRD_REQUIRE(smem <= 200 * 1024, "embed_bwd_packed: L = %d too long for the shared positional accumulator", L);
  static bool attr = false;
  if (!attr) {
    SRFRD_CUDA(cudaFuncSetAttribute(embed_bwd_packed_kernel, cudaFuncAttributeMaxDynamicSharedMemorySize, 200 * 1024));
    attr = true;
  }
  int per_sm = (int)((200 * 1024) / (smem + 1024));
  if (per_sm > 4) per_sm = 4;
  if (per_sm < 1) per_sm = 1;
  int64_t gx = ((int64_t)num_sms() * per_sm + slices - 1) / slices;
  const int64_t need = (cap_rows + ty - 1) / ty;
  if (gx > need) gx = need;
  if (gx < 1) gx = 1;
  const dim3 grid((unsigned)gx, (unsigned)slices);
  SRFRD_CUDA(launch_pdl(embed_bwd_packed_kernel, grid, dim3(tx, ty), smem, (cudaStream_t)stream, p, row_tok, rows_dev, cap_rows,
                        d_pos));
  SRFRD_LAUNCH_CHECK();
  return 0;
}

extern "C" int srfrd_add_segments(float* in, int64_t n, int seg_in, int seg_out, float* out, void* stream) {
  SRFRD_REQUIRE(in && out && seg_in > 0 && seg_out <= seg_in, "add_segments: bad arguments");
  if (n == 0) return 0;
  SRFRD_CUDA(launch_pdl(add_segments_kernel, dim3((unsigned)((n + 255) / 256)), dim3(256), 0, (cudaStream_t)stream, in, n, seg_in,
                        seg_out, out));
  SRFRD_LAUNCH_CHECK();
  return 0;
}

extern "C" int srfrd_adam_tick(float* state3, float beta1, float beta2, void* stream) {
  SRFRD_REQUIRE(state3, "adam_tick: null state");
  SRFRD_CUDA(launch_pdl(adam_tick_kernel, dim3(1), dim3(1), 0, (cudaStream_t)stream, state3, beta1, beta2));
  SRFRD_LAUNCH_CHECK();
  return 0;
}

extern "C" int srfrd_adam_step(float* p, float* g, float* m, float* v, int64_t n, float lr, float beta1, float beta2,
                               float eps, const float* state3, int zero_grad, void* stream) {
  SRFRD_REQUIRE(p && g && m && v && state3, "adam_step: null pointer");
  SRFRD_REQUIRE((((uintptr_t)p | (uintptr_t)g | (uintptr_t)m | (uintptr_t)v) & 15) == 0, "adam_step: buffers must be 16-byte aligned");
  if (n == 0) return 0;
  int64_t blocks = (n / 4 + 255) / 256;
  if (blocks < 1) blocks = 1;
  if (blocks > num_sms() * 8) blocks = num_sms() * 8;
  SRFRD_CUDA(launch_pdl(adam_kernel, dim3((unsigned)blocks), dim3(256), 0, (cudaStream_t)stream, p, g, m, v, n, lr, beta1, beta2,
                        eps, state3, zero_grad));
  SRFRD_LAUNCH_CHECK();
  return 0;
}

extern "C" int srfrd_adam_step_fused(float* p, float* g, float* m, float* v, int64_t n, float lr, float beta1, float beta2,
                                     float eps, float* state8, int zero_grad, float* acc2, const float* norm2, float* loss,
                                     void* stream, const int64_t* l2_seg, int l2_n_seg, const float* l2_coef,
                                     const float* l2_reg) {
  SRFRD_REQUIRE(p && g && m && v && state8, "adam_step_fused: null pointer");
  SRFRD_REQUIRE(!acc2 || (norm2 && loss), "adam_step_fused: the loss read-out needs norm and loss");
  SRFRD_REQUIRE((((uintptr_t)p | (uintptr_t)g | (uintptr_t)m | (uintptr_t)v) & 15) == 0, "adam_step_fused: buffers must be 16-byte aligned");
  const bool l2 = l2_seg != nullptr;
  SRFRD_REQUIRE(!l2 || (l2_coef && l2_reg && acc2), "adam_step_fused: the l2 term needs coef, reg and the loss read-out");
  SRFRD_REQUIRE(!l2 || (l2_n_seg >= 1 && l2_n_seg <= L2_THREADS && n % 4 == 0),
                "adam_step_fused: l2 needs 1..%d segments and n a multiple of 4", L2_THREADS);
  int64_t blocks = (n / 4 + 255) / 256;
  if (blocks < 1) blocks = 1;
  if (blocks > num_sms() * 8) blocks = num_sms() * 8;
  const L2Segments l2s{l2_seg, l2_n_seg, l2_coef, l2_reg};
  if (l2)
    SRFRD_CUDA(launch_pdl(adam_fused_kernel<true>, dim3((unsigned)blocks), dim3(256), 0, (cudaStream_t)stream, p, g, m, v, n,
                          lr, beta1, beta2, eps, state8, zero_grad, acc2, norm2, loss, l2s));
  else
    SRFRD_CUDA(launch_pdl(adam_fused_kernel<false>, dim3((unsigned)blocks), dim3(256), 0, (cudaStream_t)stream, p, g, m, v, n,
                          lr, beta1, beta2, eps, state8, zero_grad, acc2, norm2, loss, l2s));
  SRFRD_LAUNCH_CHECK();
  return 0;
}

extern "C" int srfrd_param_l2_plan(const int64_t* seg_host, int n_seg, int64_t* n_chunks) {
  SRFRD_REQUIRE(seg_host && n_chunks, "param_l2_plan: null pointer");
  SRFRD_REQUIRE(n_seg >= 1 && n_seg <= L2_THREADS, "param_l2_plan: %d segments (1..%d supported)", n_seg, L2_THREADS);
  int64_t c = 0, end = 0;
  for (int t = 0; t < n_seg; ++t) {
    const int64_t off = seg_host[2 * t], numel = seg_host[2 * t + 1];
    SRFRD_REQUIRE(off % 4 == 0 && off >= end && numel >= 0, "param_l2_plan: segment %d must start 4-aligned after the last", t);
    end = off + numel;
    c += (numel + L2_CHUNK - 1) / L2_CHUNK;
  }
  *n_chunks = c;
  return 0;
}

extern "C" int srfrd_param_l2(const float* p, const int64_t* seg, int n_seg, int64_t n_chunks, float l2, float* coef,
                              float* reg, double* ws, void* stream) {
  SRFRD_REQUIRE(p && seg && coef && reg && ws, "param_l2: null pointer");
  SRFRD_REQUIRE(((uintptr_t)p & 15) == 0, "param_l2: the parameter buffer must be 16-byte aligned");
  SRFRD_REQUIRE(n_seg >= 1 && n_seg <= L2_THREADS && n_chunks >= 0, "param_l2: bad segment / chunk count");
  int64_t grid = n_chunks < 1 ? 1 : n_chunks;
  if (grid > num_sms() * 8) grid = num_sms() * 8;
  SRFRD_CUDA(launch_pdl(param_l2_kernel, dim3((unsigned)grid), dim3(L2_THREADS), 0, (cudaStream_t)stream, p, seg, n_seg,
                        n_chunks, l2, coef, reg, ws));
  SRFRD_LAUNCH_CHECK();
  return 0;
}
```

### srfrd_b200/engine.py

```python
from __future__ import annotations

import math
import os
from contextlib import contextmanager, nullcontext
from dataclasses import dataclass
from typing import Dict, List, Optional, Tuple

import torch

from . import ops

bf16 = torch.bfloat16
LN_EPS = 1e-8

KINDS = ("SRFR", "SRFRN", "SRFU_B", "SRFU_F", "SRFU_R", "SASRec")


@dataclass
class ModelSpec:
    kind: str
    item_number: int
    max_len: int
    D: int
    F: int = 0
    n_labels: int = 0
    num_blocks: int = 2
    num_heads: int = 1
    dropout: float = 0.0

    def __post_init__(self):
        if self.kind not in KINDS:
            raise ValueError(f"unknown model kind {self.kind}")
        if self.H % self.num_heads:
            raise ValueError("hidden size must be divisible by num_heads")
        if (self.H // self.num_heads) % 2:
            raise ValueError(f"srfrd_b200: head width {self.H // self.num_heads} must be even (bf16 pairs)")

    @property
    def H(self) -> int:
        return self.D + self.F if self.kind in ("SRFR", "SRFRN") else self.D

    @property
    def Dout(self) -> int:
        return self.H if self.kind == "SRFRN" else self.D

    @property
    def Hp(self) -> int:
        return (self.H + 15) // 16 * 16

    @property
    def Dp(self) -> int:
        return (self.D + 15) // 16 * 16

    @property
    def Doutp(self) -> int:
        return self.Hp if self.kind == "SRFRN" else self.Dp

    @property
    def padded(self) -> bool:
        return self.Hp != self.H or self.Dp != self.D

    @property
    def mode(self) -> int:
        return 1 if self.kind in ("SRFR", "SRFRN") else (2 if self.kind.startswith("SRFU") else 0)

    @property
    def item_scale(self) -> float:
        return float(self.D ** 0.5) if self.kind == "SASRec" else 1.0

    @property
    def item_key(self) -> str:
        return "item_emb.weight" if self.kind == "SASRec" else "embedding_layer.item_embed.weight"

    @property
    def pos_key(self) -> str:
        return "pos_emb.weight" if self.kind == "SASRec" else "embedding_layer.pos_embed.weight"

    @property
    def aux_key(self) -> Optional[str]:
        if self.mode == 1:
            return "embedding_layer.fake_embed.weight"
        if self.mode == 2:
            return "embedding_layer.user_label_embed.weight"
        return None

    def param_shapes(self) -> List[Tuple[str, Tuple[int, ...]]]:
        H, D, L, N = self.H, self.D, self.max_len, self.item_number
        out: List[Tuple[str, Tuple[int, ...]]] = []
        if self.kind == "SASRec":
            out += [("item_emb.weight", (N + 1, D)), ("pos_emb.weight", (L, D))]
        elif self.mode == 1:
            out += [("embedding_layer.item_embed.weight", (N + 1, D)),
                    ("embedding_layer.fake_embed.weight", (3, self.F)),
                    ("embedding_layer.pos_embed.weight", (L, D))]
        else:
            out += [("embedding_layer.item_embed.weight", (N + 1, D)),
                    ("embedding_layer.user_label_embed.weight", (self.n_labels, D)),
                    ("embedding_layer.pos_embed.weight", (L, D))]
        for i in range(self.num_blocks):
            out += [(f"attention_layernorms.{i}.weight", (H,)), (f"attention_layernorms.{i}.bias", (H,))]
        for i in range(self.num_blocks):
            out += [(f"attention_layers.{i}.in_proj_weight", (3 * H, H)), (f"attention_layers.{i}.in_proj_bias", (3 * H,)),
                    (f"attention_layers.{i}.out_proj.weight", (H, H)), (f"attention_layers.{i}.out_proj.bias", (H,))]
        for i in range(self.num_blocks):
            out += [(f"forward_layernorms.{i}.weight", (H,)), (f"forward_layernorms.{i}.bias", (H,))]
        for i in range(self.num_blocks):
            out += [(f"forward_layers.{i}.conv1.weight", (H, H, 1)), (f"forward_layers.{i}.conv1.bias", (H,)),
                    (f"forward_layers.{i}.conv2.weight", (H, H, 1)), (f"forward_layers.{i}.conv2.bias", (H,))]
        if self.kind == "SRFR":
            out += [("last_conv.weight", (D, H, 1)), ("last_conv.bias", (D,))]
        out += [("last_layernorm.weight", (self.Dout,)), ("last_layernorm.bias", (self.Dout,))]
        return out


class FlatParams:

    def __init__(self, spec: ModelSpec, device, alloc=None):
        self.spec = spec
        self.offsets: Dict[str, Tuple[int, Tuple[int, ...]]] = {}
        off = 0
        for name, shape in spec.param_shapes():
            n = int(math.prod(shape))
            self.offsets[name] = (off, shape)
            off += (n + 3) // 4 * 4
        self.numel = off
        zeros = (lambda n: alloc(n).zero_()) if alloc is not None else (lambda n: torch.zeros(n, dtype=torch.float32, device=device))
        self.data_ext = zeros(off + 4)
        self.data = self.data_ext[:off]
        self.data_tail = self.data_ext[off:]
        self.grad_bucket = zeros(off + 4)
        self.grad = self.grad_bucket[:off]
        self.grad_tail = self.grad_bucket[off:]

    def segments(self) -> List[Tuple[int, int]]:
        return [(off, int(math.prod(shape))) for off, shape in self.offsets.values()]

    def view(self, name: str, grad: bool = False) -> torch.Tensor:
        off, shape = self.offsets[name]
        buf = self.grad if grad else self.data
        return buf[off:off + int(math.prod(shape))].view(shape)

    def mat(self, name: str, grad: bool = False) -> torch.Tensor:
        v = self.view(name, grad)
        return v.view(v.shape[0], -1)


class HotPath:

    def __init__(self, spec: ModelSpec, params: FlatParams):
        self.spec, self.P = spec, params
        self.device = params.data.device
        self._ws_tokens = 0
        self._ws: Dict[str, torch.Tensor] = {}
        self.ws_generation = 0
        self.fwd_version = 0
        self.host_drop_counter = 0
        self._build_shadows()
        self.step_state = torch.zeros(8, dtype=torch.float32, device=self.device)
        self.side = torch.cuda.Stream(device=self.device)
        self.side2 = torch.cuda.Stream(device=self.device)
        self.overlap = os.environ.get("SRFRD_OVERLAP", "1") != "0"
        self.drop_seed = 0x5EED5EED
        self.saved: Optional[dict] = None
        self._plans: Dict[Tuple[int, int], ops.PackedPlan] = {}
        self.packed_default = os.environ.get("SRFRD_PACKED", "1") != "0"
        self.fuse_ffn = os.environ.get("SRFRD_FUSE_FFN", "1") != "0"

    def _build_shadows(self):
        s, P, dev = self.spec, self.P, self.device
        H, D, Hp, Dp = s.H, s.D, s.Hp, s.Dp
        self.sh: Dict[str, torch.Tensor] = {}
        self.vsh: Dict[str, torch.Tensor] = {}
        entries = []
        zb = lambda r, c: torch.zeros(r, c, dtype=bf16, device=dev)

        def vec(name, src, n_pad, dst_off=0, dst=None):
            if not s.padded:
                return
            if dst is None:
                dst = self.vsh.setdefault(name, torch.zeros(n_pad, dtype=torch.float32, device=dev))
            entries.append((src.view(1, -1), dst[dst_off:dst_off + src.numel()].view(1, -1), None))

        for i in range(s.num_blocks):
            win = P.mat(f"attention_layers.{i}.in_proj_weight")
            bin_ = P.view(f"attention_layers.{i}.in_proj_bias")
            self.sh[f"wq{i}"] = zb(Hp, Hp)
            self.sh[f"wkv{i}"] = zb(2 * Hp, Hp)
            self.sh[f"wqT{i}"] = zb(Hp, Hp)
            self.sh[f"wkvT{i}"] = zb(Hp, 2 * Hp)
            entries.append((win[:H], self.sh[f"wq{i}"][:H, :H], self.sh[f"wqT{i}"][:H, :H]))
            entries.append((win[H:2 * H], self.sh[f"wkv{i}"][:H, :H], self.sh[f"wkvT{i}"][:H, :H]))
            entries.append((win[2 * H:], self.sh[f"wkv{i}"][Hp:Hp + H, :H], self.sh[f"wkvT{i}"][:H, Hp:Hp + H]))
            vec(f"bq{i}", bin_[:H], Hp)
            vec(f"bkv{i}", bin_[H:2 * H], 2 * Hp)
            vec(f"bkv{i}", bin_[2 * H:], 2 * Hp, dst_off=Hp)
            for tag, key in (("wo", f"attention_layers.{i}.out_proj"), ("w1", f"forward_layers.{i}.conv1"),
                             ("w2", f"forward_layers.{i}.conv2")):
                self.sh[f"{tag}{i}"] = zb(Hp, Hp)
                self.sh[f"{tag}T{i}"] = zb(Hp, Hp)
                entries.append((P.mat(key + ".weight"), self.sh[f"{tag}{i}"][:H, :H], self.sh[f"{tag}T{i}"][:H, :H]))
                vec(f"b{tag[1]}{i}", P.view(key + ".bias"), Hp)
        if s.kind == "SRFR":
            self.sh["wc"] = zb(Dp, Hp)
            self.sh["wcT"] = zb(Hp, Dp)
            entries.append((P.mat("last_conv.weight"), self.sh["wc"][:D, :H], self.sh["wcT"][:H, :D]))
            vec("bc", P.view("last_conv.bias"), Dp)
        self._cast_table, self._cast_n = ops.make_cast_table(entries, dev)
        self.shadows_version = -1

    def bias(self, tag: str, i: Optional[int] = None) -> torch.Tensor:
        s, P = self.spec, self.P
        if s.padded:
            return self.vsh[tag if i is None else f"{tag}{i}"]
        if tag == "bq":
            return P.view(f"attention_layers.{i}.in_proj_bias")[:s.H]
        if tag == "bkv":
            return P.view(f"attention_layers.{i}.in_proj_bias")[s.H:]
        if tag == "bc":
            return P.view("last_conv.bias")
        key = {"bo": f"attention_layers.{i}.out_proj.bias", "b1": f"forward_layers.{i}.conv1.bias",
               "b2": f"forward_layers.{i}.conv2.bias"}[tag]
        return P.view(key)

    def refresh_shadows(self):
        ops.cast_weights(self._cast_table, self._cast_n)

    @contextmanager
    def _branch(self, second: bool = False):
        if not self.overlap:
            yield
            return
        main = torch.cuda.current_stream()
        st = self.side2 if second else self.side
        st.wait_stream(main)
        with torch.cuda.stream(st):
            yield

    def _join(self, second: bool = False):
        if self.overlap:
            torch.cuda.current_stream().wait_stream(self.side2 if second else self.side)

    def _workspace(self, T: int, L: int) -> Dict[str, torch.Tensor]:
        if T <= self._ws_tokens:
            return self._ws
        s, dev = self.spec, self.device
        Lmax = max(L, s.max_len)
        H, nb = s.Hp, s.num_blocks
        ws: Dict[str, torch.Tensor] = {}

        def act(name, w=H, dtype=bf16):
            ws[name] = torch.zeros(T, w, dtype=dtype, device=dev)

        for i in range(nb + 1):
            act(f"x{i}")
        for i in range(nb):
            for n in ("Q", "q", "o", "r", "y", "h1"):
                act(f"{n}{i}")
            act(f"kv{i}", 2 * H)
            act(f"st1_{i}", 2, torch.float32)
            act(f"st2_{i}", 2, torch.float32)
            if Lmax > 128:
                ws[f"ast{i}"] = torch.zeros(T * s.num_heads, 4, dtype=torch.float32, device=dev)
        if s.kind == "SRFR":
            act("c", s.Dp)
        act("stF", 2, torch.float32)
        act("hfin", s.Doutp, torch.float32)
        act("dh", s.Doutp, torch.float32)
        for n in ("gA", "gC", "gD", "gX"):
            act(n)
        for i in range(nb):
            for n in ("gda1_", "gdr_", "gdq_"):
                act(f"{n}{i}")
            act(f"gdz_{i}")
            act(f"gdkv_{i}", 2 * H)
        if s.kind == "SRFR":
            act("gc", s.Dp)
        if s.dropout > 0:
            for i in range(nb):
                act(f"gE_{i}")
        ws["pos_tmp"] = torch.zeros(Lmax * H, dtype=torch.float32, device=dev)
        self._ws, self._ws_tokens = ws, T
        self.ws_generation += 1
        return ws

    def packed_ok(self, B: int, L: int) -> bool:
        return self.packed_mode(B, L) is not None

    def packed_mode(self, B: int, L: int) -> Optional[str]:
        s = self.spec
        if s.padded or s.H % 16 or s.D % 8 or B > 16384 or B < 1:
            return None
        if ops.attention_packed_supported(L, s.H, s.num_heads):
            return "tile"
        if os.environ.get("SRFRD_HYBRID", "1") != "0" and L <= 4096:
            return "hybrid"
        return None

    def _hybrid_ws(self, Td: int) -> Dict[str, torch.Tensor]:
        hw = getattr(self, "_hws", None)
        if hw is not None and hw["_rows"] >= Td:
            return hw
        s, dev = self.spec, self.device
        Hp = s.Hp
        hw = {"_rows": Td}
        z = lambda w: torch.zeros(Td, w, dtype=bf16, device=dev)
        for i in range(s.num_blocks):
            hw[f"qd{i}"], hw[f"kvd{i}"], hw[f"od{i}"] = z(Hp), z(2 * Hp), z(Hp)
        hw["dod"], hw["dqd"], hw["dkvd"] = z(Hp), z(Hp), z(2 * Hp)
        self._hws = hw
        self.ws_generation += 1
        return hw

    def _live_tiles(self, B: int, L: int) -> "ops.LiveTiles":
        key = (B, L)
        lt = getattr(self, "_lives", None)
        if lt is None:
            lt = self._lives = {}
        if key not in lt:
            if len(lt) >= 4:
                lt.clear()
                self.ws_generation += 1
            lt[key] = ops.LiveTiles(B, L, self.spec.num_heads, self.device)
        return lt[key]

    def _plan(self, B: int, L: int) -> "ops.PackedPlan":
        key = (B, L)
        if key not in self._plans:
            if len(self._plans) >= 4:
                self._plans.clear()
                self.ws_generation += 1
            self._plans[key] = ops.PackedPlan(B, L, self.device)
        return self._plans[key]

    def forward(self, seq: torch.Tensor, fake_ids: Optional[torch.Tensor], training: bool,
                last_only: bool = False, save: Optional[bool] = None, packed: bool = False,
                keep: Optional[torch.Tensor] = None) -> torch.Tensor:
        s, P = self.spec, self.P
        B, L = seq.shape
        if L > s.max_len:
            raise RuntimeError(f"sequence length {L} exceeds max_len {s.max_len} (pos_embed rows, SRFR_model.py:12)")
        if packed:
            return self._forward_packed(seq, fake_ids, training, last_only, save, keep)
        T, H, Hp, nb = B * L, s.H, s.Hp, s.num_blocks
        ws = self._workspace(T, L)
        self.fwd_version += 1
        p_drop = s.dropout if training else 0.0
        step = self.step_state[3:4] if p_drop > 0 else None
        seed = (self.drop_seed + self.host_drop_counter * 0x9E3779B97F4A7C15) & 0xFFFFFFFFFFFFFFFF
        seq = seq.contiguous()
        aux_ids = None
        if s.mode == 1:
            aux_ids = None if fake_ids is None else fake_ids.contiguous()
        elif s.mode == 2:
            aux_ids = torch.empty(B, dtype=torch.int64, device=self.device)
            ops.srfu_labels(fake_ids.contiguous(), {"SRFU_B": 0, "SRFU_F": 1, "SRFU_R": 2}[s.kind], aux_ids)
            need = {"SRFU_B": 3, "SRFU_F": L + 1, "SRFU_R": 11}[s.kind]
            if s.n_labels < need and B > 0 and int(aux_ids.max()) >= s.n_labels:
                raise IndexError(f"index out of range in self: {s.kind} user label {int(aux_ids.max())} needs "
                                 f"number_of_labels >= {need}, got {s.n_labels}")
        aux_table = P.view(s.aux_key) if s.aux_key else None
        x = [ws[f"x{i}"][:T] for i in range(nb + 1)]
        ops.embed_ln_fwd(P.view(s.item_key), P.view(s.pos_key), aux_table, s.mode, seq, aux_ids, s.item_scale,
                         P.view("attention_layernorms.0.weight"), P.view("attention_layernorms.0.bias"), LN_EPS,
                         x0_bf16=x[0], q_bf16=ws["Q0"][:T], stats=ws["st1_0"][:T],
                         drop_p=p_drop if s.kind == "SASRec" else 0.0, drop_seed=seed, drop_stream=1, drop_step=step)
        seq_flat = seq.view(-1)
        fuse_ln = (H == Hp) and Hp <= 128 and os.environ.get("SRFRD_FUSE_LN", "1") != "0"
        for i in range(nb):
            Q, q, kv, o, r, y, h1 = (ws[f"{n}{i}"][:T] for n in ("Q", "q", "kv", "o", "r", "y", "h1"))
            with self._branch():
                ops.gemm_tn(x[i], self.sh[f"wkv{i}"], out_bf16=kv, bias=self.bias("bkv", i))
            if i > 0 and not fuse_ln:
                ops.layernorm_fwd(x[i], P.view(f"attention_layernorms.{i}.weight"), P.view(f"attention_layernorms.{i}.bias"),
                                  LN_EPS, y_bf16=Q, stats=ws[f"st1_{i}"][:T], H=H)
            ops.gemm_tn(Q, self.sh[f"wq{i}"], out_bf16=q, bias=self.bias("bq", i))
            self._join()
            ops.attention_fwd(q, kv[:, :Hp], kv[:, Hp:], o, B, L, H, s.num_heads, p_drop, seed, 10 + 4 * i, step,
                              stats=ws.get(f"ast{i}"))
            if fuse_ln:
                ops.gemm_tn(o, self.sh[f"wo{i}"], out_bf16=r, bias=self.bias("bo", i), residual=Q, ln_out=y,
                            ln_w=P.view(f"forward_layernorms.{i}.weight"), ln_b=P.view(f"forward_layernorms.{i}.bias"),
                            ln_eps=LN_EPS, ln_stats=ws[f"st2_{i}"][:T])
            else:
                ops.gemm_tn(o, self.sh[f"wo{i}"], out_bf16=r, bias=self.bias("bo", i), residual=Q)
                ops.layernorm_fwd(r, P.view(f"forward_layernorms.{i}.weight"), P.view(f"forward_layernorms.{i}.bias"), LN_EPS,
                                  y_bf16=y, stats=ws[f"st2_{i}"][:T], H=H)
            ops.gemm_tn(y, self.sh[f"w1{i}"], out_bf16=h1, bias=self.bias("b1", i), relu=True,
                        drop_p=p_drop, drop_seed=seed, drop_stream=11 + 4 * i, drop_step=step)
            nxt = {}
            if fuse_ln and i + 1 < nb:
                nxt = dict(ln_out=ws[f"Q{i + 1}"][:T], ln_w=P.view(f"attention_layernorms.{i + 1}.weight"),
                           ln_b=P.view(f"attention_layernorms.{i + 1}.bias"), ln_eps=LN_EPS, ln_stats=ws[f"st1_{i + 1}"][:T])
            ops.gemm_tn(h1, self.sh[f"w2{i}"], out_bf16=x[i + 1], bias=self.bias("b2", i),
                        residual=y, row_ids=seq_flat, drop_p=p_drop, drop_seed=seed, drop_stream=12 + 4 * i, drop_step=step,
                        **nxt)
        fin_in = x[nb]
        if s.kind == "SRFR":
            ops.gemm_tn(x[nb], self.sh["wc"], out_bf16=ws["c"][:T], bias=self.bias("bc"))
            fin_in = ws["c"][:T]
        hfin = ws["hfin"][:T]
        if last_only:
            out = ws["hfin"][:B]
            ops.layernorm_fwd(fin_in, P.view("last_layernorm.weight"), P.view("last_layernorm.bias"), LN_EPS, y_f32=out,
                              T=B, H=s.Dout, row_stride=L, row_offset=L - 1)
            return out[:, :s.Dout]
        ops.layernorm_fwd(fin_in, P.view("last_layernorm.weight"), P.view("last_layernorm.bias"), LN_EPS, y_f32=hfin,
                          stats=ws["stF"][:T], H=s.Dout)
        if training if save is None else save:
            self.saved = dict(seq=seq, aux_ids=aux_ids, B=B, L=L, p_drop=p_drop, seed=seed, step=step,
                              version=self.fwd_version)
        return hfin.view(B, L, s.Doutp)[..., :s.Dout]

    def backward(self, dh: torch.Tensor, version: Optional[int] = None) -> None:
        s, P, sv = self.spec, self.P, self.saved
        if sv is None:
            raise RuntimeError("backward() without a training forward()")
        if sv["version"] != self.fwd_version or (version is not None and version != sv["version"]):
            raise RuntimeError("srfrd_b200: backward() of a stale forward -- another forward() (training, validation or "
                               "predict) ran on this model after the one being back-propagated and overwrote the shared "
                               "activation workspace; run backward() before the next forward()")
        if sv.get("plan") is not None:
            return self._backward_packed(dh)
        B, L = sv["B"], sv["L"]
        T, H, Hp, nb = B * L, s.H, s.Hp, s.num_blocks
        ws = self._ws
        seq_flat = sv["seq"].view(-1)
        p_drop, seed, step = sv["p_drop"], sv["seed"], sv["step"]
        gA, gC, gD, gX = (ws[n][:T] for n in ("gA", "gC", "gD", "gX"))
        G = lambda name: P.view(name, grad=True)
        GM = lambda name: P.mat(name, grad=True)
        x = [ws[f"x{i}"][:T] for i in range(nb + 1)]
        dz_top = ws[f"gdz_{nb - 1}"][:T]

        if s.kind == "SRFR":
            gc = ws["gc"][:T]
            ops.layernorm_bwd(dh, ws["c"][:T], ws["stF"][:T], P.view("last_layernorm.weight"), gc,
                              G("last_layernorm.weight"), G("last_layernorm.bias"), H=s.D)
            with self._branch():
                ops.gemm_wgrad(gc, x[nb], GM("last_conv.weight"), G("last_conv.bias"), Mo=s.D, No=H)
            ops.gemm_tn(gc, self.sh["wcT"], out_bf16=dz_top, row_ids=seq_flat)
        else:
            ops.layernorm_bwd(dh, x[nb], ws["stF"][:T], P.view("last_layernorm.weight"), dz_top,
                              G("last_layernorm.weight"), G("last_layernorm.bias"), row_ids=seq_flat, H=s.Dout)

        for i in reversed(range(nb)):
            Q, q, kv, o, r, y, h1 = (ws[f"{n}{i}"][:T] for n in ("Q", "q", "kv", "o", "r", "y", "h1"))
            dz, da1, dr, dq, dkv = (ws[f"{n}{i}"][:T] for n in ("gdz_", "gda1_", "gdr_", "gdq_", "gdkv_"))
            dx_out = ws[f"gdz_{i - 1}"][:T] if i > 0 else gA
            dz2 = dz
            if p_drop > 0:
                dz2 = ws[f"gE_{i}"][:T]
                ops.dropout_apply(dz, dz2, Hp, p_drop, seed, 12 + 4 * i, step)
            with self._branch():
                ops.gemm_wgrad(dz2, h1, GM(f"forward_layers.{i}.conv2.weight"), G(f"forward_layers.{i}.conv2.bias"), Mo=H, No=H)
            ops.gemm_tn(dz2, self.sh[f"w2T{i}"], out_bf16=da1, gate=h1, drop_p=p_drop, drop_seed=seed,
                        drop_stream=11 + 4 * i, drop_step=step)
            with self._branch():
                ops.gemm_wgrad(da1, y, GM(f"forward_layers.{i}.conv1.weight"), G(f"forward_layers.{i}.conv1.bias"), Mo=H, No=H)
            ops.gemm_tn(da1, self.sh[f"w1T{i}"], out_bf16=gC, residual=dz)
            ops.layernorm_bwd(gC, r, ws[f"st2_{i}"][:T], P.view(f"forward_layernorms.{i}.weight"), dr,
                              G(f"forward_layernorms.{i}.weight"), G(f"forward_layernorms.{i}.bias"), H=H)
            with self._branch():
                ops.gemm_wgrad(dr, o, GM(f"attention_layers.{i}.out_proj.weight"), G(f"attention_layers.{i}.out_proj.bias"),
                               Mo=H, No=H)
            ops.gemm_tn(dr, self.sh[f"woT{i}"], out_bf16=gC)
            ops.attention_bwd(gC, q, kv[:, :Hp], kv[:, Hp:], dq, dkv[:, :Hp], dkv[:, Hp:], B, L, H, s.num_heads, p_drop,
                              seed, 10 + 4 * i, step, o=o, stats=ws.get(f"ast{i}"))
            gin = GM(f"attention_layers.{i}.in_proj_weight")
            gbin = G(f"attention_layers.{i}.in_proj_bias")
            with self._branch():
                ops.gemm_wgrad(dq, Q, gin[:H], gbin[:H], Mo=H, No=H)
                if Hp == H:
                    ops.gemm_wgrad(dkv, x[i], gin[H:], gbin[H:], Mo=2 * H, No=H)
                else:
                    ops.gemm_wgrad(dkv[:, :Hp], x[i], gin[H:2 * H], gbin[H:2 * H], Mo=H, No=H)
                    ops.gemm_wgrad(dkv[:, Hp:], x[i], gin[2 * H:], gbin[2 * H:], Mo=H, No=H)
            with self._branch(second=True):
                ops.gemm_tn(dkv, self.sh[f"wkvT{i}"], out_bf16=gX)
            ops.gemm_tn(dq, self.sh[f"wqT{i}"], out_bf16=gD, residual=dr)
            self._join(second=True)
            ops.layernorm_bwd(gD, x[i], ws[f"st1_{i}"][:T], P.view(f"attention_layernorms.{i}.weight"), dx_out,
                              G(f"attention_layernorms.{i}.weight"), G(f"attention_layernorms.{i}.bias"),
                              add=gX, row_ids=seq_flat, H=H)

        dx0 = gA
        if s.kind == "SASRec" and p_drop > 0:
            ops.dropout_apply(gA, gC, H, p_drop, seed, 1, step)
            dx0 = gC
        aux_grad = G(s.aux_key) if s.aux_key else None
        ops.embed_bwd(dx0, sv["seq"], sv["aux_ids"], s.D, s.F if s.mode == 1 else 0, s.mode, s.item_scale,
                      G(s.item_key), aux_grad)
        pos_tmp = ws["pos_tmp"][:L * Hp]
        ops.colsum(dx0, pos_tmp, M=B, N=L * Hp, ld=L * Hp)
        ops.add_segments(pos_tmp, L * Hp, Hp, s.D, G(s.pos_key))
        self._join()
        self.saved = None

    def _forward_packed(self, seq, fake_ids, training, last_only, save, keep):
        s, P = self.spec, self.P
        B, L = seq.shape
        H, Hp, nb = s.H, s.Hp, s.num_blocks
        plan = self._plan(B, L)
        T = plan.cap
        ws = self._workspace(T, L)
        self.fwd_version += 1
        p_drop = s.dropout if training else 0.0
        step = self.step_state[3:4] if p_drop > 0 else None
        seed = (self.drop_seed + self.host_drop_counter * 0x9E3779B97F4A7C15) & 0xFFFFFFFFFFFFFFFF
        seq = seq.contiguous()
        aux_ids = None
        if s.mode == 1:
            aux_ids = None if fake_ids is None else fake_ids.contiguous()
        elif s.mode == 2:
            aux_ids = torch.empty(B, dtype=torch.int64, device=self.device)
            ops.srfu_labels(fake_ids.contiguous(), {"SRFU_B": 0, "SRFU_F": 1, "SRFU_R": 2}[s.kind], aux_ids)
            need = {"SRFU_B": 3, "SRFU_F": L + 1, "SRFU_R": 11}[s.kind]
            if s.n_labels < need and int(aux_ids.max()) >= s.n_labels:
                raise IndexError(f"index out of range in self: {s.kind} user label {int(aux_ids.max())} needs "
                                 f"number_of_labels >= {need}, got {s.n_labels}")
        aux_table = P.view(s.aux_key) if s.aux_key else None
        plan.build(seq, None if keep is None else keep.contiguous())
        hyb = self._hybrid_ws(B * L) if self.packed_mode(B, L) == "hybrid" else None
        live = None
        if hyb is not None and os.environ.get("SRFRD_LIVE_TILES", "1") != "0":
            live = self._live_tiles(B, L)
            live.build(plan)
        x = [ws[f"x{i}"][:T] for i in range(nb + 1)]
        row_ids = plan.row_ids
        fuse_ln = Hp <= 128 and os.environ.get("SRFRD_FUSE_LN", "1") != "0"
        fuse_oproj = self._fuse_oproj(hyb, L, fuse_ln) & 1
        with ops.row_limit(plan.rows):
            ops.embed_ln_fwd_packed(P.view(s.item_key), P.view(s.pos_key), aux_table, s.mode, seq, aux_ids, s.item_scale,
                                    P.view("attention_layernorms.0.weight"), P.view("attention_layernorms.0.bias"), LN_EPS,
                                    x[0], ws["Q0"][:T], ws["st1_0"][:T], plan,
                                    drop_p=p_drop if s.kind == "SASRec" else 0.0, drop_seed=seed, drop_stream=1, drop_step=step)
            for i in range(nb):
                Q, q, kv, o, r, y, h1 = (ws[f"{n}{i}"][:T] for n in ("Q", "q", "kv", "o", "r", "y", "h1"))
                with self._branch():
                    ops.gemm_tn(x[i], self.sh[f"wkv{i}"], out_bf16=kv, bias=self.bias("bkv", i))
                if i > 0 and not fuse_ln:
                    ops.layernorm_fwd(x[i], P.view(f"attention_layernorms.{i}.weight"), P.view(f"attention_layernorms.{i}.bias"),
                                      LN_EPS, y_bf16=Q, stats=ws[f"st1_{i}"][:T], H=H)
                ops.gemm_tn(Q, self.sh[f"wq{i}"], out_bf16=q, bias=self.bias("bq", i))
                self._join()
                if fuse_oproj:
                    ops.attention_fwd_packed(q, kv[:, :Hp], kv[:, Hp:], o, plan, L, H, s.num_heads, p_drop, seed, 10 + 4 * i, step,
                                             wo=self.sh[f"wo{i}"], bias=self.bias("bo", i), residual=Q, r=r, y=y,
                                             ln_w=P.view(f"forward_layernorms.{i}.weight"),
                                             ln_b=P.view(f"forward_layernorms.{i}.bias"), ln_eps=LN_EPS,
                                             ln_stats=ws[f"st2_{i}"][:T])
                elif hyb is None:
                    ops.attention_fwd_packed(q, kv[:, :Hp], kv[:, Hp:], o, plan, L, H, s.num_heads, p_drop, seed, 10 + 4 * i, step)
                else:
                    qd, kvd, od = hyb[f"qd{i}"][:B * L], hyb[f"kvd{i}"][:B * L], hyb[f"od{i}"][:B * L]
                    ops.unpack_rows([(q, qd, Hp, 0), (kv, kvd, 2 * Hp, 0)], plan)
                    with (live.active() if live is not None else nullcontext()):
                        ops.attention_fwd(qd, kvd[:, :Hp], kvd[:, Hp:], od, B, L, H, s.num_heads, p_drop, seed, 10 + 4 * i, step,
                                          stats=ws.get(f"ast{i}"))
                    ops.pack_rows([(od, o, Hp, 0)], plan)
                if fuse_oproj:
                    pass
                elif fuse_ln:
                    ops.gemm_tn(o, self.sh[f"wo{i}"], out_bf16=r, bias=self.bias("bo", i), residual=Q, ln_out=y,
                                ln_w=P.view(f"forward_layernorms.{i}.weight"), ln_b=P.view(f"forward_layernorms.{i}.bias"),
                                ln_eps=LN_EPS, ln_stats=ws[f"st2_{i}"][:T])
                else:
                    ops.gemm_tn(o, self.sh[f"wo{i}"], out_bf16=r, bias=self.bias("bo", i), residual=Q)
                    ops.layernorm_fwd(r, P.view(f"forward_layernorms.{i}.weight"), P.view(f"forward_layernorms.{i}.bias"),
                                      LN_EPS, y_bf16=y, stats=ws[f"st2_{i}"][:T], H=H)
                nxt = {}
                if fuse_ln and i + 1 < nb:
                    nxt = dict(ln_out=ws[f"Q{i + 1}"][:T], ln_w=P.view(f"attention_layernorms.{i + 1}.weight"),
                               ln_b=P.view(f"attention_layernorms.{i + 1}.bias"), ln_eps=LN_EPS,
                               ln_stats=ws[f"st1_{i + 1}"][:T])
                if self.fuse_ffn and Hp <= 128:
                    ops.mlp2_tn(y, self.sh[f"w1{i}"], self.sh[f"w2{i}"], h1, x[i + 1], bias1=self.bias("b1", i),
                                bias2=self.bias("b2", i), relu1=True, drop1_p=p_drop, drop2_p=p_drop, drop1_stream=11 + 4 * i,
                                drop2_stream=12 + 4 * i, drop_seed=seed, drop_step=step, residual_is_a=True, row_ids=row_ids,
                                **nxt)
                else:
                    ops.gemm_tn(y, self.sh[f"w1{i}"], out_bf16=h1, bias=self.bias("b1", i), relu=True,
                                drop_p=p_drop, drop_seed=seed, drop_stream=11 + 4 * i, drop_step=step)
                    ops.gemm_tn(h1, self.sh[f"w2{i}"], out_bf16=x[i + 1], bias=self.bias("b2", i), residual=y, row_ids=row_ids,
                                drop_p=p_drop, drop_seed=seed, drop_stream=12 + 4 * i, drop_step=step, **nxt)
            fin_in = x[nb]
            if s.kind == "SRFR":
                ops.gemm_tn(x[nb], self.sh["wc"], out_bf16=ws["c"][:T], bias=self.bias("bc"))
                fin_in = ws["c"][:T]
            if not last_only:
                ops.layernorm_fwd(fin_in, P.view("last_layernorm.weight"), P.view("last_layernorm.bias"), LN_EPS,
                                  y_f32=ws["hfin"][:T], stats=ws["stF"][:T], H=s.Dout)
        if last_only:
            out = ws["hfin"][:B]
            ops.layernorm_fwd_rows(fin_in, P.view("last_layernorm.weight"), P.view("last_layernorm.bias"), LN_EPS, out,
                                   plan.last_row, B, s.Dout)
            return out[:, :s.Dout]
        if training if save is None else save:
            self.saved = dict(seq=seq, aux_ids=aux_ids, B=B, L=L, p_drop=p_drop, seed=seed, step=step,
                              version=self.fwd_version, plan=plan, hyb=hyb, live=live)
        return ws["hfin"][:T]

    def _fuse_oproj(self, hyb, L, fuse_ln) -> int:
        s = self.spec
        if hyb is not None or s.num_heads != 1 or not fuse_ln or s.Hp != s.H:
            return 0
        return ops.attention_packed_oproj_supported(L, s.H, s.num_heads)

    def _backward_packed(self, dh: torch.Tensor) -> None:
        s, P, sv = self.spec, self.P, self.saved
        plan, hyb, live = sv["plan"], sv.get("hyb"), sv.get("live")
        B, L = sv["B"], sv["L"]
        T, H, Hp, nb = plan.cap, s.H, s.Hp, s.num_blocks
        ws = self._ws
        row_ids = plan.row_ids
        p_drop, seed, step = sv["p_drop"], sv["seed"], sv["step"]
        gA, gC, gD, gX = (ws[n][:T] for n in ("gA", "gC", "gD", "gX"))
        G = lambda name: P.view(name, grad=True)
        GM = lambda name: P.mat(name, grad=True)
        x = [ws[f"x{i}"][:T] for i in range(nb + 1)]
        dz_top = ws[f"gdz_{nb - 1}"][:T]
        fuse_oproj = self._fuse_oproj(hyb, L, Hp <= 128 and os.environ.get("SRFRD_FUSE_LN", "1") != "0") & 2
        with ops.row_limit(plan.rows):
            if s.kind == "SRFR":
                gc = ws["gc"][:T]
                ops.layernorm_bwd(dh, ws["c"][:T], ws["stF"][:T], P.view("last_layernorm.weight"), gc,
                                  G("last_layernorm.weight"), G("last_layernorm.bias"), H=s.D)
                with self._branch():
                    ops.gemm_wgrad(gc, x[nb], GM("last_conv.weight"), G("last_conv.bias"), Mo=s.D, No=H)
                ops.gemm_tn(gc, self.sh["wcT"], out_bf16=dz_top, row_ids=row_ids)
            else:
                ops.layernorm_bwd(dh, x[nb], ws["stF"][:T], P.view("last_layernorm.weight"), dz_top,
                                  G("last_layernorm.weight"), G("last_layernorm.bias"), row_ids=row_ids, H=s.Dout)
            for i in reversed(range(nb)):
                Q, q, kv, o, r, y, h1 = (ws[f"{n}{i}"][:T] for n in ("Q", "q", "kv", "o", "r", "y", "h1"))
                dz, da1, dr, dq, dkv = (ws[f"{n}{i}"][:T] for n in ("gdz_", "gda1_", "gdr_", "gdq_", "gdkv_"))
                dx_out = ws[f"gdz_{i - 1}"][:T] if i > 0 else gA
                dz2 = dz
                if p_drop > 0:
                    dz2 = ws[f"gE_{i}"][:T]
                    ops.dropout_apply(dz, dz2, Hp, p_drop, seed, 12 + 4 * i, step)
                with self._branch():
                    ops.gemm_wgrad(dz2, h1, GM(f"forward_layers.{i}.conv2.weight"), G(f"forward_layers.{i}.conv2.bias"), Mo=H, No=H)
                if self.fuse_ffn and Hp <= 128:
                    ops.mlp2_tn(dz2, self.sh[f"w2T{i}"], self.sh[f"w1T{i}"], da1, gC, gate=h1, drop1_p=p_drop,
                                drop1_stream=11 + 4 * i, drop_seed=seed, drop_step=step, residual=dz)
                    with self._branch():
                        ops.gemm_wgrad(da1, y, GM(f"forward_layers.{i}.conv1.weight"), G(f"forward_layers.{i}.conv1.bias"),
                                       Mo=H, No=H)
                else:
                    ops.gemm_tn(dz2, self.sh[f"w2T{i}"], out_bf16=da1, gate=h1, drop_p=p_drop, drop_seed=seed,
                                drop_stream=11 + 4 * i, drop_step=step)
                    with self._branch():
                        ops.gemm_wgrad(da1, y, GM(f"forward_layers.{i}.conv1.weight"), G(f"forward_layers.{i}.conv1.bias"),
                                       Mo=H, No=H)
                    ops.gemm_tn(da1, self.sh[f"w1T{i}"], out_bf16=gC, residual=dz)
                ops.layernorm_bwd(gC, r, ws[f"st2_{i}"][:T], P.view(f"forward_layernorms.{i}.weight"), dr,
                                  G(f"forward_layernorms.{i}.weight"), G(f"forward_layernorms.{i}.bias"), H=H)
                with self._branch():
                    ops.gemm_wgrad(dr, o, GM(f"attention_layers.{i}.out_proj.weight"),
                                   G(f"attention_layers.{i}.out_proj.bias"), Mo=H, No=H)
                if not fuse_oproj:
                    ops.gemm_tn(dr, self.sh[f"woT{i}"], out_bf16=gC)
                if fuse_oproj:
                    ops.attention_bwd_packed(None, q, kv[:, :Hp], kv[:, Hp:], dq, dkv[:, :Hp], dkv[:, Hp:], plan, L, H,
                                             s.num_heads, p_drop, seed, 10 + 4 * i, step, dr=dr, woT=self.sh[f"woT{i}"])
                elif hyb is None:
                    ops.attention_bwd_packed(gC, q, kv[:, :Hp], kv[:, Hp:], dq, dkv[:, :Hp], dkv[:, Hp:], plan, L, H,
                                             s.num_heads, p_drop, seed, 10 + 4 * i, step)
                else:
                    Td = B * L
                    qd, kvd, od = hyb[f"qd{i}"][:Td], hyb[f"kvd{i}"][:Td], hyb[f"od{i}"][:Td]
                    dod, dqd, dkvd = hyb["dod"][:Td], hyb["dqd"][:Td], hyb["dkvd"][:Td]
                    ops.unpack_rows([(gC, dod, Hp, 1)], plan)
                    with (live.active() if live is not None else nullcontext()):
                        ops.attention_bwd(dod, qd, kvd[:, :Hp], kvd[:, Hp:], dqd, dkvd[:, :Hp], dkvd[:, Hp:], B, L, H,
                                          s.num_heads, p_drop, seed, 10 + 4 * i, step, o=od, stats=ws.get(f"ast{i}"))
                    ops.pack_rows([(dqd, dq, Hp, 0), (dkvd, dkv, 2 * Hp, 1)], plan)
                gin = GM(f"attention_layers.{i}.in_proj_weight")
                gbin = G(f"attention_layers.{i}.in_proj_bias")
                with self._branch():
                    ops.gemm_wgrad(dq, Q, gin[:H], gbin[:H], Mo=H, No=H)
                    ops.gemm_wgrad(dkv, x[i], gin[H:], gbin[H:], Mo=2 * H, No=H)
                with self._branch(second=True):
                    ops.gemm_tn(dkv, self.sh[f"wkvT{i}"], out_bf16=gX)
                ops.gemm_tn(dq, self.sh[f"wqT{i}"], out_bf16=gD, residual=dr)
                self._join(second=True)
                ops.layernorm_bwd(gD, x[i], ws[f"st1_{i}"][:T], P.view(f"attention_layernorms.{i}.weight"), dx_out,
                                  G(f"attention_layernorms.{i}.weight"), G(f"attention_layernorms.{i}.bias"),
                                  add=gX, row_ids=row_ids, H=H)
            dx0 = gA
            if s.kind == "SASRec" and p_drop > 0:
                ops.dropout_apply(gA, gC, H, p_drop, seed, 1, step)
                dx0 = gC
        aux_grad = G(s.aux_key) if s.aux_key else None
        ops.embed_bwd_packed(dx0, sv["seq"], sv["aux_ids"], plan, s.D, s.F if s.mode == 1 else 0, s.mode, s.item_scale,
                             G(s.item_key), aux_grad, G(s.pos_key))
        self._join()
        self.saved = None

    def fake_table(self) -> Optional[torch.Tensor]:
        return self.P.view("embedding_layer.fake_embed.weight") if self.spec.kind == "SRFRN" else None

    def fake_table_grad(self) -> Optional[torch.Tensor]:
        return self.P.view("embedding_layer.fake_embed.weight", grad=True) if self.spec.kind == "SRFRN" else None
```

### srfrd_b200/ops.py

```python
from __future__ import annotations

import ctypes as C
from typing import Optional

import torch

from . import _lib
from contextlib import contextmanager

from ._lib import CastDesc, GemmEpilogue, Mlp2Epilogue, PackDesc, RepackPart, call

bf16 = torch.bfloat16


def _p(t: Optional[torch.Tensor]):
    return None if t is None else t.data_ptr()


def _stream():
    return torch.cuda.current_stream().cuda_stream


def _chk(t: torch.Tensor, dtype, name: str):
    if not t.is_cuda:
        raise RuntimeError(f"srfrd_b200: {name} must be a CUDA tensor (there is no CPU fallback)")
    if t.dtype != dtype:
        raise RuntimeError(f"srfrd_b200: {name} must be {dtype}, got {t.dtype}")
    if t.stride(-1) != 1:
        raise RuntimeError(f"srfrd_b200: {name} must be contiguous in its last dimension")


def embed_ln_fwd(item_table, pos_table, aux_table, mode, seq, aux_ids, item_scale, ln_w, ln_b, eps,
                 x0_bf16=None, x0_f32=None, q_bf16=None, stats=None, drop_p=0.0, drop_seed=0, drop_stream=0,
                 drop_step=None):
    _lib.require_device()
    B, L = seq.shape
    D = item_table.shape[1]
    F = aux_table.shape[1] if (aux_table is not None and mode == 1) else 0
    _chk(item_table, torch.float32, "item_table"); _chk(seq, torch.int64, "seq")
    ldx = (x0_bf16 if x0_bf16 is not None else q_bf16).stride(0) if (x0_bf16 is not None or q_bf16 is not None) else D + F
    call("srfrd_embed_ln_fwd", _p(item_table), item_table.shape[0], D, _p(pos_table), _p(aux_table),
         0 if aux_table is None else aux_table.shape[0], F, mode, _p(seq), _p(aux_ids), B, L, float(item_scale),
         _p(ln_w), _p(ln_b), float(eps), _p(x0_bf16), _p(x0_f32), _p(q_bf16), _p(stats), ldx, float(drop_p),
         int(drop_seed), int(drop_stream), _p(drop_step), _stream())


def srfu_labels(fake_ids, kind: int, labels):
    _lib.require_device()
    B, L = fake_ids.shape
    call("srfrd_srfu_labels", _p(fake_ids), B, L, kind, _p(labels), _stream())


def embed_bwd(dx0, seq, aux_ids, D, F, mode, item_scale, d_item, d_aux):
    B, L = seq.shape
    call("srfrd_embed_bwd", _p(dx0), dx0.stride(0), _p(seq), _p(aux_ids), B, L, D, F, mode, float(item_scale),
         _p(d_item), _p(d_aux), _stream())


def layernorm_fwd(x, w, b, eps, y_bf16=None, y_f32=None, stats=None, T=None, H=None, row_stride=1, row_offset=0):
    _lib.require_device()
    T = x.shape[0] if T is None else T
    H = x.shape[1] if H is None else H
    y = y_bf16 if y_bf16 is not None else y_f32
    call("srfrd_layernorm_fwd", _p(x), x.stride(0), _p(w), _p(b), float(eps), _p(y_bf16), _p(y_f32), y.stride(0),
         _p(stats), T, H, row_stride, row_offset, _stream())


def layernorm_bwd(dy, x, stats, w, dx, dw, db, add=None, row_ids=None, H=None):
    T = x.shape[0]
    H = x.shape[1] if H is None else H
    dyb = dy if dy.dtype == bf16 else None
    dyf = dy if dy.dtype == torch.float32 else None
    call("srfrd_layernorm_bwd", _p(dyb), _p(dyf), dy.stride(0), _p(x), x.stride(0), _p(stats), _p(w), _p(add),
         0 if add is None else add.stride(0), _p(row_ids), _p(dx), dx.stride(0), _p(dw), _p(db), T, H, _stream())


def gemm_tn(A, B, out_bf16=None, out_f32=None, bias=None, residual=None, gate=None, row_ids=None, relu=False,
            drop_p=0.0, drop_seed=0, drop_stream=0, drop_step=None, M=None, ln_out=None, ln_w=None, ln_b=None, ln_eps=0.0,
            ln_stats=None):
    _lib.require_device()
    M = A.shape[0] if M is None else M
    K = A.shape[1]
    N = B.shape[0]
    out = out_bf16 if out_bf16 is not None else out_f32
    ep = GemmEpilogue(_p(bias), _p(residual), _p(gate), _p(row_ids), _p(out_bf16), _p(out_f32),
                      0 if residual is None else residual.stride(0), 0 if gate is None else gate.stride(0),
                      out.stride(0), int(relu), float(drop_p), int(drop_stream), int(drop_seed), _p(drop_step),
                      _p(ln_out), _p(ln_w), _p(ln_b), _p(ln_stats), 0 if ln_out is None else ln_out.stride(0), float(ln_eps))
    call("srfrd_gemm_tn", _p(A), A.stride(0), _p(B), B.stride(0), M, N, K, C.byref(ep), _stream())


def gemm_wgrad(dY, X, dW, dbias=None, Mo=None, No=None):
    T = dY.shape[0]
    Mo = dY.shape[1] if Mo is None else Mo
    No = X.shape[1] if No is None else No
    call("srfrd_gemm_wgrad", _p(dY), dY.stride(0), _p(X), X.stride(0), T, Mo, No, _p(dW), dW.stride(0), _p(dbias),
         _stream())


def gemm_ref(A, B, Cout, a_mn_major=False, b_mn_major=False):
    _lib.require_device()
    M, N = Cout.shape
    K = A.shape[0] if a_mn_major else A.shape[1]
    call("srfrd_gemm_ref", _p(A), A.stride(0), _p(B), B.stride(0), _p(Cout), Cout.stride(0), M, N, K,
         int(a_mn_major), int(b_mn_major), _stream())


def colsum(X, out, M=None, N=None, ld=None):
    M = X.shape[0] if M is None else M
    N = X.shape[1] if N is None else N
    ld = X.stride(0) if ld is None else ld
    call("srfrd_colsum", _p(X), M, N, ld, _p(out), _stream())


def add_segments(src, n, seg_in, seg_out, out):
    call("srfrd_add_segments", _p(src), n, seg_in, seg_out, _p(out), _stream())


def dropout_apply(x, out, N, drop_p, seed, stream_id, drop_step=None):
    call("srfrd_dropout_apply", _p(x), x.stride(0), _p(out), out.stride(0), x.shape[0], N, float(drop_p), int(seed),
         int(stream_id), _p(drop_step), _stream())


def cast_weights(descs_dev, n):
    call("srfrd_cast_weights", _p(descs_dev), n, _stream())


def make_cast_table(entries, device):
    arr = (CastDesc * len(entries))()
    for i, (src, dst, dst_t) in enumerate(entries):
        is_f32 = int(dst is not None and dst.dtype == torch.float32)
        arr[i] = CastDesc(src.data_ptr(), src.stride(0), _p(dst), 0 if dst is None else dst.stride(0), _p(dst_t),
                          0 if dst_t is None else dst_t.stride(0), src.shape[0], src.shape[1], is_f32)
    raw = bytes(arr)
    host = torch.frombuffer(bytearray(raw), dtype=torch.uint8)
    return host.to(device), len(entries)


def f32_to_bf16_split(src, hi, lo=None, row_index=None):
    _lib.require_device()
    rows = src.shape[0] if row_index is None else row_index.numel()
    cols = src.shape[1]
    call("srfrd_f32_to_bf16_split", _p(src), src.stride(0), _p(row_index), _p(hi), _p(lo), rows, cols, hi.stride(0),
         _stream())


def attention_fwd(q, k, v, o, B, L, H, heads, drop_p=0.0, seed=0, stream_id=0, drop_step=None, stats=None):
    _lib.require_device()
    call("srfrd_attention_fwd", _p(q), q.stride(0), _p(k), _p(v), k.stride(0), _p(o), o.stride(0), _p(stats), B, L, H, heads,
         float(drop_p), int(seed), int(stream_id), _p(drop_step), _stream())


def attention_bwd(dout, q, k, v, dq, dk, dv, B, L, H, heads, drop_p=0.0, seed=0, stream_id=0, drop_step=None, o=None,
                  stats=None):
    call("srfrd_attention_bwd", _p(dout), dout.stride(0), _p(q), q.stride(0), _p(k), _p(v), k.stride(0), _p(o),
         0 if o is None else o.stride(0), _p(stats), _p(dq), dq.stride(0), _p(dk), _p(dv), dk.stride(0), B, L, H, heads,
         float(drop_p), int(seed), int(stream_id), _p(drop_step), _stream())


def score_fwd(h, item_table, fake_table, pos, neg, prs, nrs, zp, zn):
    _lib.require_device()
    T = pos.numel()
    D = item_table.shape[1]
    F = 0 if fake_table is None else fake_table.shape[1]
    call("srfrd_score_fwd", _p(h), h.stride(0), _p(item_table), _p(fake_table), _p(pos), _p(neg), _p(prs), _p(nrs), T,
         D, F, _p(zp), _p(zn), _stream())


def score_bwd(h, item_table, fake_table, pos, neg, prs, nrs, dzp, dzn, dh, d_item, d_fake):
    T = pos.numel()
    D = item_table.shape[1]
    F = 0 if fake_table is None else fake_table.shape[1]
    call("srfrd_score_bwd", _p(h), h.stride(0), _p(item_table), _p(fake_table), _p(pos), _p(neg), _p(prs), _p(nrs),
         _p(dzp), _p(dzn), T, D, F, _p(dh), dh.stride(0), _p(d_item), _p(d_fake), _stream())


def score_loss_fused(h, item_table, fake_table, pos, neg, prs, nrs, w_pos, w_neg, norm, loss_acc, dh, d_item, d_fake,
                     zp=None, zn=None):
    T = pos.numel()
    D = item_table.shape[1]
    F = 0 if fake_table is None else fake_table.shape[1]
    call("srfrd_score_loss_fused", _p(h), h.stride(0), _p(item_table), _p(fake_table), _p(pos), _p(neg), _p(prs),
         _p(nrs), _p(w_pos), _p(w_neg), _p(norm), T, D, F, _p(zp), _p(zn), _p(loss_acc), _p(dh),
         0 if dh is None else dh.stride(0), _p(d_item), _p(d_fake), _stream())


def weight_sums(pos, w_pos, w_neg, out2):
    _lib.require_device()
    call("srfrd_weight_sums", _p(pos), _p(w_pos), _p(w_neg), pos.numel(), _p(out2), _stream())


def loss_finalize(acc2, norm2, loss):
    call("srfrd_loss_finalize", _p(acc2), _p(norm2), _p(loss), _stream())


def adam_tick(state3, beta1, beta2):
    call("srfrd_adam_tick", _p(state3), float(beta1), float(beta2), _stream())


def adam_step(p, g, m, v, lr, beta1, beta2, eps, state3, zero_grad=True):
    _lib.require_device()
    call("srfrd_adam_step", _p(p), _p(g), _p(m), _p(v), p.numel(), float(lr), float(beta1), float(beta2), float(eps),
         _p(state3), int(zero_grad), _stream())


def adam_step_fused(p, g, m, v, lr, beta1, beta2, eps, state8, zero_grad=True, acc2=None, norm2=None, loss=None,
                    l2: Optional["ParamL2"] = None):
    _lib.require_device()
    call("srfrd_adam_step_fused", _p(p), _p(g), _p(m), _p(v), p.numel(), float(lr), float(beta1), float(beta2), float(eps),
         _p(state8), int(zero_grad), _p(acc2), _p(norm2), _p(loss), _stream(), *_l2_args(l2))


class ParamL2:

    def __init__(self, segments, l2: float, device):
        host = (C.c_int64 * (2 * len(segments)))(*[int(x) for s in segments for x in s])
        n_chunks = C.c_int64(0)
        call("srfrd_param_l2_plan", host, len(segments), C.byref(n_chunks))
        self.n_seg, self.n_chunks, self.l2 = len(segments), int(n_chunks.value), float(l2)
        self.seg = torch.tensor([int(x) for s in segments for x in s], dtype=torch.int64).to(device)
        self.coef = torch.zeros(self.n_seg, dtype=torch.float32, device=device)
        self.reg = torch.zeros(1, dtype=torch.float32, device=device)
        self.ws = torch.zeros(self.n_chunks + 1, dtype=torch.float64, device=device)

    def launch(self, p: torch.Tensor):
        _lib.require_device()
        _chk(p, torch.float32, "p")
        call("srfrd_param_l2", _p(p), _p(self.seg), self.n_seg, self.n_chunks, self.l2, _p(self.coef), _p(self.reg),
             _p(self.ws), _stream())


def _l2_args(l2: Optional[ParamL2]):
    return (None, 0, None, None) if l2 is None else (_p(l2.seg), l2.n_seg, _p(l2.coef), _p(l2.reg))


def catalogue_topk_plan(U, n_rows, row_lo, D, n_split, k=10) -> int:
    out = C.c_int(0)
    call("srfrd_catalogue_topk_plan", U, n_rows, row_lo, D, n_split, C.byref(out), int(k))
    return out.value


def catalogue_topk_kmax(D, n_split) -> int:
    out = C.c_int(0)
    call("srfrd_catalogue_topk_kmax", D, n_split, C.byref(out))
    return out.value


def catalogue_topk(feats, U, u_pad, n_split, table, row_lo, id_base, chunks, part_scores, part_ids, packed=None, k=10):
    _lib.require_device()
    D = table.shape[1]
    call("srfrd_catalogue_topk", _p(feats), U, u_pad, n_split, _p(table), table.shape[0], row_lo, id_base, D,
         feats.stride(0), table.stride(0), chunks, _p(part_scores), _p(part_ids), _p(packed), _stream(), int(k))


def catalogue_rank(feats, U, u_pad, n_split, table, row_lo, id_base, target_rows, target_ids, rank_out,
                   target_scores=None):
    _lib.require_device()
    D = table.shape[1]
    call("srfrd_catalogue_rank", _p(feats), U, u_pad, n_split, _p(table), table.shape[0], row_lo, id_base, D,
         feats.stride(0), table.stride(0), _p(target_rows), target_rows.stride(0), _p(target_ids), _p(target_scores),
         _p(rank_out), _stream())


def merge_topk_packed(packed, U, nlists, k, out_scores, out_ids):
    _lib.require_device()
    call("srfrd_merge_topk_packed", _p(packed), U, nlists, k, _p(out_scores), _p(out_ids), _stream())


def merge_topk(scores, ids, U, nlists, k, out_scores, out_ids):
    _lib.require_device()
    call("srfrd_merge_topk", _p(scores), _p(ids), U, nlists, k, _p(out_scores), _p(out_ids), _stream())


def sample_batch(offsets, items, labels, p_fake, eligible, itemnum, B, L, policy, seed, step, out, w_pos=None):
    _lib.require_device()
    call("srfrd_sample_batch", _p(offsets), _p(items), _p(labels), _p(p_fake), _p(eligible), eligible.numel(), int(itemnum),
         B, L, int(policy), int(seed), _p(step), _p(out.get("users")), _p(out["seq"]), _p(out["rsq"]), _p(out["pos"]),
         _p(out["prs"]), _p(out["neg"]), _p(out["nrs"]), _p(w_pos), _stream())


def sample_candidates(offsets, items, users0, target, itemnum, C, seed, cand):
    _lib.require_device()
    call("srfrd_sample_candidates", _p(offsets), _p(items), _p(users0), _p(target), users0.numel(), int(itemnum), int(C),
         int(seed), _p(cand), _stream())


def candidate_rank(feats, item_table, cand, D, fake_table=None, user_label=None, logits=None, rank=None, err_flag=None):
    _lib.require_device()
    _chk(feats, torch.float32, "feats"); _chk(item_table, torch.float32, "item_table"); _chk(cand, torch.int64, "cand")
    U, Cn = cand.shape
    F = 0 if fake_table is None else fake_table.shape[1]
    call("srfrd_candidate_rank", _p(feats), feats.stride(0), _p(item_table), item_table.shape[0], int(D), _p(cand), U, Cn,
         _p(fake_table), F, _p(user_label), _p(logits), 0 if logits is None else logits.stride(0), _p(rank), _p(err_flag),
         _stream())


def add_user_term(logits, feats_tail, fake_table, label):
    _lib.require_device()
    U, I = logits.shape
    call("srfrd_add_user_term", _p(logits), logits.stride(0), U, I, _p(feats_tail), feats_tail.stride(0), _p(fake_table),
         _p(label), fake_table.shape[1], _stream())


class PackedPlan:

    def __init__(self, B: int, L: int, device):
        self.B, self.L = B, L
        self.cap = (B * (L + 1) + 127) // 128 * 128
        i32 = lambda n: torch.zeros(n, dtype=torch.int32, device=device)
        self.rows, self.cnt, self.seq_first = i32(4), i32(B), i32(B + 1)
        self.tok_row, self.row_tok = i32(B * L), i32(self.cap)
        self.row_ids = torch.zeros(self.cap, dtype=torch.int64, device=device)
        self.row_info = i32(4 * self.cap)
        self.tile_row0, self.last_row = i32(B + 130), i32(B)
        self.desc = PackDesc(_p(self.rows), _p(self.cnt), _p(self.seq_first), _p(self.tok_row), _p(self.row_tok),
                             _p(self.row_ids), _p(self.row_info), _p(self.tile_row0), _p(self.last_row), self.cap)

    def build(self, seq, keep=None):
        _lib.require_device()
        B, L = seq.shape
        assert (B, L) == (self.B, self.L)
        _chk(seq, torch.int64, "seq")
        call("srfrd_pack_plan", _p(seq), _p(keep), B, L, C.byref(self.desc), _stream())


@contextmanager
def row_limit(rows_dev):
    call("srfrd_set_row_limit", _p(rows_dev))
    try:
        yield
    finally:
        call("srfrd_set_row_limit", None)


class LiveTiles:

    def __init__(self, B: int, L: int, heads: int, device):
        nq = (L + 127) // 128
        self.B, self.L, self.heads = B, L, heads
        self.q_lo = torch.zeros(B, dtype=torch.int32, device=device)
        self.items = torch.zeros(B * heads * nq, dtype=torch.int32, device=device)
        self.n_live = torch.zeros(1, dtype=torch.int32, device=device)

    def build(self, plan: "PackedPlan"):
        _lib.require_device()
        assert (plan.B, plan.L) == (self.B, self.L)
        self.tok_row = plan.tok_row
        call("srfrd_attention_live_items", _p(plan.tok_row), self.B, self.L, self.heads, _p(self.q_lo), _p(self.items),
             _p(self.n_live), _stream())

    @contextmanager
    def active(self):
        call("srfrd_set_attention_live", _p(self.q_lo), _p(self.items), _p(self.n_live), _p(self.tok_row))
        try:
            yield
        finally:
            call("srfrd_set_attention_live", None, None, None, None)


def attention_packed_supported(L: int, H: int, heads: int) -> bool:
    return bool(_lib.load().srfrd_attention_packed_supported(int(L), int(H), int(heads)))


def embed_ln_fwd_packed(item_table, pos_table, aux_table, mode, seq, aux_ids, item_scale, ln_w, ln_b, eps, x0_bf16, q_bf16,
                        stats, plan: PackedPlan, drop_p=0.0, drop_seed=0, drop_stream=0, drop_step=None):
    _lib.require_device()
    B, L = seq.shape
    D = item_table.shape[1]
    F = aux_table.shape[1] if (aux_table is not None and mode == 1) else 0
    call("srfrd_embed_ln_fwd_packed", _p(item_table), item_table.shape[0], D, _p(pos_table), _p(aux_table),
         0 if aux_table is None else aux_table.shape[0], F, mode, _p(seq), _p(aux_ids), B, L, float(item_scale), _p(ln_w),
         _p(ln_b), float(eps), _p(x0_bf16), _p(q_bf16), _p(stats), x0_bf16.stride(0), float(drop_p), int(drop_seed),
         int(drop_stream), _p(drop_step), _p(plan.row_tok), _p(plan.rows), plan.cap, _stream())


def layernorm_fwd_rows(x, w, b, eps, y_f32, row_index, n, H):
    _lib.require_device()
    call("srfrd_layernorm_fwd_rows", _p(x), x.stride(0), _p(w), _p(b), float(eps), _p(y_f32), y_f32.stride(0), _p(row_index),
         n, H, _stream())


def attention_packed_oproj_supported(L: int, H: int, heads: int) -> int:
    return int(_lib.load().srfrd_attention_packed_oproj_supported(int(L), int(H), int(heads)))


def attention_fwd_packed(q, k, v, o, plan: PackedPlan, L, H, heads, drop_p=0.0, seed=0, stream_id=0, drop_step=None,
                         wo=None, bias=None, residual=None, r=None, y=None, ln_w=None, ln_b=None, ln_eps=0.0, ln_stats=None):
    _lib.require_device()
    st = lambda t: 0 if t is None else t.stride(0)
    call("srfrd_attention_fwd_packed", _p(q), q.stride(0), _p(k), _p(v), k.stride(0), _p(o), o.stride(0), C.byref(plan.desc),
         L, H, heads, float(drop_p), int(seed), int(stream_id), _p(drop_step), _stream(), _p(wo), st(wo), _p(bias),
         _p(residual), st(residual), _p(ln_w), _p(ln_b), float(ln_eps), _p(ln_stats), _p(r), st(r), _p(y), st(y))


def attention_bwd_packed(dout, q, k, v, dq, dk, dv, plan: PackedPlan, L, H, heads, drop_p=0.0, seed=0, stream_id=0,
                         drop_step=None, dr=None, woT=None):
    st = lambda t: 0 if t is None else t.stride(0)
    call("srfrd_attention_bwd_packed", _p(dout), st(dout), _p(q), q.stride(0), _p(k), _p(v), k.stride(0), _p(dq),
         dq.stride(0), _p(dk), _p(dv), dk.stride(0), C.byref(plan.desc), L, H, heads, float(drop_p), int(seed),
         int(stream_id), _p(drop_step), _stream(), _p(dr), st(dr), _p(woT), st(woT))


def score_loss_fused_packed(h, item_table, fake_table, pos, neg, prs, nrs, w_pos, w_neg, norm, loss_acc, dh, d_item, d_fake,
                            plan: PackedPlan):
    D = item_table.shape[1]
    F = 0 if fake_table is None else fake_table.shape[1]
    call("srfrd_score_loss_fused_packed", _p(h), h.stride(0), _p(item_table), _p(fake_table), _p(pos), _p(neg), _p(prs),
         _p(nrs), _p(w_pos), _p(w_neg), _p(norm), D, F, _p(loss_acc), _p(dh), dh.stride(0), _p(d_item), _p(d_fake),
         _p(plan.row_tok), _p(plan.rows), plan.cap, _stream())


def embed_bwd_packed(dx0, seq, aux_ids, plan: PackedPlan, D, F, mode, item_scale, d_item, d_aux, d_pos):
    B, L = seq.shape
    call("srfrd_embed_bwd_packed", _p(dx0), dx0.stride(0), _p(seq), _p(aux_ids), _p(plan.row_tok), _p(plan.rows), plan.cap,
         L, D, F, mode, float(item_scale), _p(d_item), _p(d_aux), _p(d_pos), _stream())


def dp_adam_step(grad_ptrs_dev: int, param_ptrs_dev: int, signal_ptrs_dev: int, rank, world, n, m, v, lr, beta1, beta2, eps,
                 state8, norm2, local4, l2: Optional[ParamL2] = None):
    _lib.require_device()
    call("srfrd_dp_adam_step", grad_ptrs_dev, param_ptrs_dev, signal_ptrs_dev, int(rank), int(world), int(n), _p(m), _p(v),
         float(lr), float(beta1), float(beta2), float(eps), _p(state8), _p(norm2), _p(local4), _stream(), *_l2_args(l2))


def _parts(parts):
    arr = (RepackPart * len(parts))()
    for i, (src, dst, W, mode) in enumerate(parts):
        arr[i] = RepackPart(_p(src), src.stride(0), _p(dst), dst.stride(0), int(W), int(mode))
    return arr


def unpack_rows(parts, plan: PackedPlan):
    _lib.require_device()
    arr = _parts(parts)
    call("srfrd_unpack_rows", arr, len(parts), C.byref(plan.desc), plan.B, plan.L, _stream())


def pack_rows(parts, plan: PackedPlan):
    _lib.require_device()
    arr = _parts(parts)
    call("srfrd_pack_rows", arr, len(parts), C.byref(plan.desc), plan.B, plan.L, _stream())


def mlp2_tn(A, W1, W2, mid_out, out, bias1=None, bias2=None, gate=None, relu1=False, drop1_p=0.0, drop2_p=0.0, drop1_stream=0,
            drop2_stream=0, drop_seed=0, drop_step=None, residual=None, residual_is_a=False, row_ids=None, ln_out=None,
            ln_w=None, ln_b=None, ln_stats=None, ln_eps=0.0, M=None):
    _lib.require_device()
    M = A.shape[0] if M is None else M
    N = W1.shape[0]
    ep = Mlp2Epilogue(_p(bias1), _p(bias2), _p(gate), 0 if gate is None else gate.stride(0), int(relu1), float(drop1_p),
                      float(drop2_p), int(drop1_stream), int(drop2_stream), int(drop_seed), _p(drop_step), _p(residual),
                      0 if residual is None else residual.stride(0), int(residual_is_a), _p(row_ids), _p(mid_out),
                      mid_out.stride(0), _p(out), out.stride(0), _p(ln_out), 0 if ln_out is None else ln_out.stride(0),
                      _p(ln_w), _p(ln_b), _p(ln_stats), float(ln_eps))
    call("srfrd_mlp2_tn", _p(A), A.stride(0), _p(W1), W1.stride(0), _p(W2), W2.stride(0), M, N, C.byref(ep), _stream())
```

### srfrd_b200/trainer.py

```python
from __future__ import annotations

import time
from typing import Dict, Optional

import numpy as np
import torch

from . import ops, parallel
from .engine import HotPath

__all__ = ["simulate", "FusedTrainer", "DeviceSampler", "discriminator_weights"]

POLICIES = {"none": 0, "mask": 1, "soft": 2}


class DeviceSampler:

    def __init__(self, data, maxlen: int, device, seed: int = 0):
        dev = torch.device(device)
        self.L, self.itemnum, self.seed = maxlen, int(data.itemnum), int(seed)
        self.offsets = torch.as_tensor(np.asarray(data.offsets, np.int64)).to(dev)
        self.items = torch.as_tensor(np.asarray(data.items, np.int32)).to(dev)
        self.labels = torch.as_tensor(np.asarray(data.labels, np.int8)).to(dev)
        pf = getattr(data, "p_fake", None)
        self.p_fake = None if pf is None else torch.as_tensor(np.asarray(pf, np.float32)).to(dev)
        lens = np.diff(np.asarray(data.offsets, np.int64))
        self.eligible = torch.as_tensor(np.nonzero(lens > 1)[0].astype(np.int32)).to(dev)
        if self.eligible.numel() == 0:
            raise ValueError("no user has more than one training interaction")
        self.device = dev
        self.draws = 0

    def alloc(self, B: int):
        z = lambda: torch.zeros(B, self.L, dtype=torch.int64, device=self.device)
        return dict(users=torch.zeros(B, dtype=torch.int64, device=self.device), seq=z(), rsq=z(), pos=z(), prs=z(),
                    neg=z(), nrs=z())

    def sample_into(self, out, w_pos=None, policy: str = "none", step=None):
        B = out["seq"].shape[0]
        ops.sample_batch(self.offsets, self.items, self.labels, self.p_fake, self.eligible, self.itemnum, B, self.L,
                         POLICIES[policy], self.seed + (0 if step is not None else self.draws), step, out, w_pos)
        self.draws += 1

    def next_batch(self, batch_size: int):
        out = self.alloc(batch_size)
        self.sample_into(out)
        return out["users"], out["seq"], out["rsq"], out["pos"], out["prs"], out["neg"], out["nrs"]



def discriminator_weights(pos: torch.Tensor, p_fake: Optional[torch.Tensor], policy: str = "none") -> torch.Tensor:
    valid = (pos != 0).to(torch.float32)
    if policy == "none" or p_fake is None:
        return valid
    if policy == "mask":
        return valid * (p_fake < 0.5).to(torch.float32)
    if policy == "soft":
        return valid * (1.0 - p_fake.to(torch.float32))
    raise ValueError(f"unknown discriminator weighting policy {policy!r}")


class FusedTrainer:

    def __init__(self, model, lr: float = 1e-3, betas=(0.9, 0.98), eps: float = 1e-8, process_group=None,
                 use_graph: bool = True, l2_emb: float = 0.0, packed: Optional[bool] = None):
        self.model = model
        self._dp = None
        if process_group is not None and torch.distributed.get_world_size(process_group) > 1:
            self._dp = self._setup_fused_dp(model, process_group)
        self.eng: HotPath = model._sync_flat()
        self.P = self.eng.P
        self.spec = self.eng.spec
        self.lr, self.betas, self.eps = lr, betas, eps
        self.pg = process_group
        self.use_graph = use_graph
        self.packed = self.eng.packed_default if packed is None else bool(packed)
        dev = self.eng.device
        self.m = torch.zeros_like(self.P.data)
        self.v = torch.zeros_like(self.P.data)
        self.scal = torch.zeros(8, dtype=torch.float32, device=dev)
        self.comm = torch.cuda.Stream(device=dev)
        self._static: Optional[Dict[str, torch.Tensor]] = None
        self._graph: Optional[torch.cuda.CUDAGraph] = None
        self._graph_key = None
        self._eager_key = None
        self._has_w = (False, False)
        self.l2_emb = float(l2_emb)
        self._l2 = self._setup_l2(model) if self.l2_emb != 0.0 else None
        self.P.grad_bucket.zero_()
        self.eng.refresh_shadows()
        self.steps = 0

    def _setup_l2(self, model) -> ops.ParamL2:
        segs = self.P.segments()
        base = self.P.data.data_ptr()
        mine = sorted((p.data_ptr(), p.numel()) for p in model.parameters())
        assert mine == [(base + 4 * off, n) for off, n in segs], \
            "srfrd_b200: l2_emb: the flat parameter segments do not cover exactly model.parameters()"
        return ops.ParamL2(segs, self.l2_emb, self.eng.device)

    @staticmethod
    def _setup_fused_dp(model, pg):
        import os
        if os.environ.get("SRFRD_FUSED_DP", "1") == "0":
            return None
        try:
            import torch.distributed._symmetric_memory as symm
            dev = next(model.parameters()).device
            gname = pg.group_name
            try:
                symm.enable_symm_mem_for_group(gname)
            except Exception:
                pass
            eng = model.rehome(lambda n: symm.empty(n, dtype=torch.float32, device=dev))
            P = eng.P
            sig = symm.empty(64, dtype=torch.int32, device=dev).zero_()
            torch.cuda.synchronize()
            hg, hp, hs = (symm.rendezvous(t, gname) for t in (P.grad_bucket, P.data_ext, sig))
            dp = dict(g=int(hg.buffer_ptrs_dev), p=int(hp.buffer_ptrs_dev), s=int(hs.buffer_ptrs_dev), rank=int(hg.rank),
                      world=int(hg.world_size), keep=(hg, hp, hs, sig),
                      local=torch.zeros(4, dtype=torch.int32, device=dev))
            torch.cuda.synchronize()
            torch.distributed.barrier(group=pg)
            return dp
        except Exception as ex:
            import warnings
            warnings.warn(f"srfrd_b200: fused data-parallel optimizer unavailable ({type(ex).__name__}: {ex}); "
                          "falling back to the NCCL all-reduce + replicated Adam")
            return None

    @property
    def loss_dev(self) -> torch.Tensor:
        return self.P.data_tail[0] if self._dp is not None else self.scal[4]

    _KEYS = ("seq", "rsq", "pos", "prs", "neg", "nrs")

    @staticmethod
    def _carve(flat: torch.Tensor, B: int, L: int):
        n = B * L
        out = {k: flat[i * n:(i + 1) * n].view(B, L) for i, k in enumerate(FusedTrainer._KEYS)}
        w = flat[6 * n:7 * n].view(torch.float32)
        out["w_pos"], out["w_neg"] = w[:n].view(B, L), w[n:].view(B, L)
        return out

    def _alloc_static(self, B: int, L: int):
        dev = self.eng.device
        self._static_flat = torch.zeros(7 * B * L, dtype=torch.int64, device=dev)
        self._static = self._carve(self._static_flat, B, L)
        self._stage_flat = None
        self._graph = None

    def _step_body(self, has_wp: bool, has_wn: bool):
        st, eng, P, s = self._static, self.eng, self.P, self.spec
        B, L = st["seq"].shape
        T = B * L
        pos, neg = st["pos"].view(-1), st["neg"].view(-1)
        w_pos = st["w_pos"].view(-1) if has_wp else None
        w_neg = st["w_neg"].view(-1) if has_wn else None
        norm, acc, loss = self.scal[0:2], P.grad_tail[0:2], self.scal[4:5]
        smp = getattr(self, "_sampler", None)
        if smp is not None:
            smp.sample_into(st, st["w_pos"] if has_wp else None, self._sampler_policy, step=eng.step_state[3:4])
        self.comm.wait_stream(torch.cuda.current_stream())
        with torch.cuda.stream(self.comm):
            ops.weight_sums(pos, w_pos, w_neg, norm)
            if self.pg is not None:
                parallel.allreduce_sum_(norm, self.pg)
            if self._l2 is not None:
                self._l2.launch(P.data)
        packed = self.packed and eng.packed_ok(B, L)
        hidden = eng.forward(st["seq"], st["rsq"], training=True, packed=packed, keep=st["pos"] if packed else None)
        ws = eng._ws
        ft = eng.fake_table()
        torch.cuda.current_stream().wait_stream(self.comm)
        prs_ = st["prs"].view(-1) if ft is not None else None
        nrs_ = st["nrs"].view(-1) if ft is not None else None
        if packed:
            plan = eng.saved["plan"]
            Tp = plan.cap
            ops.score_loss_fused_packed(ws["hfin"][:Tp], P.view(s.item_key), ft, pos, neg, prs_, nrs_, w_pos, w_neg, norm, acc,
                                        ws["dh"][:Tp], P.view(s.item_key, grad=True), eng.fake_table_grad(), plan)
            eng.backward(ws["dh"][:Tp])
        else:
            ops.score_loss_fused(ws["hfin"][:T], P.view(s.item_key), ft, pos, neg, prs_, nrs_, w_pos, w_neg, norm, acc,
                                 ws["dh"][:T], P.view(s.item_key, grad=True), eng.fake_table_grad())
            eng.backward(ws["dh"][:T])
        if self._dp is not None:
            d = self._dp
            ops.dp_adam_step(d["g"], d["p"], d["s"], d["rank"], d["world"], P.numel, self.m, self.v, self.lr, self.betas[0],
                             self.betas[1], self.eps, eng.step_state, norm, d["local"], l2=self._l2)
        else:
            if self.pg is not None:
                parallel.allreduce_sum_(P.grad_bucket, self.pg)
            ops.adam_step_fused(P.data, P.grad, self.m, self.v, self.lr, self.betas[0], self.betas[1], self.eps,
                                eng.step_state, zero_grad=True, acc2=acc, norm2=norm, loss=loss, l2=self._l2)
        eng.refresh_shadows()

    def load_batch(self, batch: Dict[str, torch.Tensor], w_pos=None, w_neg=None, non_blocking: bool = True):
        B, L = batch["seq"].shape
        if self._static is None or self._static["seq"].shape != (B, L):
            self._alloc_static(B, L)
        st = self._static
        for k in ("seq", "rsq", "pos", "prs", "neg", "nrs"):
            src = batch.get(k)
            if src is None:
                st[k].zero_()
            else:
                st[k].copy_(torch.as_tensor(src), non_blocking=non_blocking)
        if w_pos is not None:
            st["w_pos"].copy_(torch.as_tensor(w_pos), non_blocking=non_blocking)
        if w_neg is not None:
            st["w_neg"].copy_(torch.as_tensor(w_neg), non_blocking=non_blocking)
        self._has_w = (w_pos is not None, w_neg is not None)

    def pack_batch(self, batch: Dict[str, torch.Tensor], w_pos=None, w_neg=None) -> torch.Tensor:
        B, L = batch["seq"].shape
        flat = torch.zeros(7 * B * L, dtype=torch.int64, device=self.eng.device)
        v = self._carve(flat, B, L)
        for k in self._KEYS:
            if batch.get(k) is not None:
                v[k].copy_(torch.as_tensor(batch[k]))
        if w_pos is not None:
            v["w_pos"].copy_(torch.as_tensor(w_pos))
        if w_neg is not None:
            v["w_neg"].copy_(torch.as_tensor(w_neg))
        flat._srfrd_shape, flat._srfrd_w = (B, L), (w_pos is not None, w_neg is not None)
        return flat

    def step_packed(self, flat: torch.Tensor) -> torch.Tensor:
        B, L = flat._srfrd_shape
        if self._static is None or self._static["seq"].shape != (B, L):
            self._alloc_static(B, L)
        self._static_flat.copy_(flat, non_blocking=True)
        self._has_w = flat._srfrd_w
        return self.run_step()

    def prefetch(self, batch: Dict[str, torch.Tensor], w_pos=None, w_neg=None):
        B, L = batch["seq"].shape
        if self._static is None or self._static["seq"].shape != (B, L):
            self._alloc_static(B, L)
        if self._stage_flat is None:
            self._stage_flat = torch.zeros_like(self._static_flat)
            self._stage = self._carve(self._stage_flat, B, L)
            self._copy_stream = torch.cuda.Stream(device=self.eng.device)
            self._stage_free = torch.cuda.Event()
            self._stage_full = torch.cuda.Event()
            self._stage_free.record()
        with torch.cuda.stream(self._copy_stream):
            self._copy_stream.wait_event(self._stage_free)
            for k in self._KEYS:
                src = batch.get(k)
                if src is None:
                    self._stage[k].zero_()
                else:
                    self._stage[k].copy_(torch.as_tensor(src), non_blocking=True)
            if w_pos is not None:
                self._stage["w_pos"].copy_(torch.as_tensor(w_pos), non_blocking=True)
            if w_neg is not None:
                self._stage["w_neg"].copy_(torch.as_tensor(w_neg), non_blocking=True)
            self._stage_full.record()
        self._stage_w = (w_pos is not None, w_neg is not None)

    def step_prefetched(self) -> torch.Tensor:
        main = torch.cuda.current_stream()
        main.wait_event(self._stage_full)
        self._static_flat.copy_(self._stage_flat)
        self._stage_free.record(main)
        self._has_w = self._stage_w
        return self.run_step()

    def run_step(self) -> torch.Tensor:
        key = (tuple(self._static["seq"].shape), self._has_w, id(getattr(self, "_sampler", None)), self.eng.ws_generation)
        if self.use_graph and self._graph is not None and self._graph_key == key:
            self._graph.replay()
        elif self.use_graph and self.steps >= 1 and self._eager_key == key[:3] + (self.eng.ws_generation,):
            g = torch.cuda.CUDAGraph()
            torch.cuda.synchronize()
            with torch.cuda.graph(g):
                self._step_body(*self._has_w)
            self._graph, self._graph_key = g, key
            g.replay()
        else:
            self._step_body(*self._has_w)
            self._eager_key = key[:3] + (self.eng.ws_generation,)
        self.steps += 1
        return self.loss_dev

    def step(self, batch, w_pos=None, w_neg=None) -> torch.Tensor:
        self.load_batch(batch, w_pos, w_neg)
        return self.run_step()

    def step_sampled(self, sampler: "DeviceSampler", batch_size: int, policy: str = "none") -> torch.Tensor:
        if self._static is None or self._static["seq"].shape != (batch_size, sampler.L):
            self._alloc_static(batch_size, sampler.L)
        self._sampler, self._sampler_policy = sampler, policy
        self._has_w = (policy != "none", False)
        out = self.run_step()
        self._sampler = None
        return out

    def state_dict(self):
        return {k: v.detach().clone() for k, v in self.model.state_dict().items()}


def simulate(model, optimizer, criterion, sampler, config, wandb=None, model_index=0, num_batch=None, device=None,
             dataset=None, evaluation=None, log_every: int = 1):
    T, t0 = 0.0, time.time()
    metricsbyepoch = dict()
    device = device if device is not None else next(model.parameters()).device
    num_batch = num_batch if num_batch is not None else getattr(config, "num_batch")
    for epoch in range(config.num_epochs):
        if config.inference_only:
            break
        epoch_loss = 0.0
        model.train()
        for step in range(num_batch):
            u, seq, rsq, pos, prs, neg, nrs = sampler.next_batch()
            seq, rsq, pos, prs, neg, nrs = (torch.as_tensor(np.array(a)).long().to(device)
                                            for a in (seq, rsq, pos, prs, neg, nrs))
            hidden_state, pos_logits, neg_logits = model(user_ids=None, input_ids=seq, fake_ids=rsq, positive_ids=pos,
                                                         positive_fake_ids=prs, negative_ids=neg, negative_fake_ids=nrs)
            pos_labels = torch.ones(pos_logits.shape, device=device)
            neg_labels = torch.zeros(neg_logits.shape, device=device)
            optimizer.zero_grad()
            indices = torch.where(pos != 0)
            loss = criterion(pos_logits[indices], pos_labels[indices])
            loss += criterion(neg_logits[indices], neg_labels[indices])
            if getattr(config, "l2_emb", 0.0):
                for param in model.parameters():
                    loss += config.l2_emb * torch.norm(param)
            loss.backward()
            optimizer.step()
            if step % log_every == 0:
                li = loss.item()
                if wandb is not None:
                    wandb.log({"Training Loss by iteration": li})
                epoch_loss += li
        if wandb is not None:
            wandb.log({"Training Loss by Epoch": epoch_loss, "Epochs": epoch + 1})
        if (epoch + 1) % 10 == 0 and evaluation is not None and dataset is not None:
            model.eval()
            T += time.time() - t0
            t_test = evaluation(model, dataset, config.maxlen, device)
            if wandb is not None:
                wandb.log({"NDCG@10": t_test[0], "HT@10": t_test[1]})
            metricsbyepoch[epoch + 1] = {"NDCG@10": t_test[0], "HT@10": t_test[1]}
            t0 = time.time()
            model.train()
    return metricsbyepoch
```

Measured before the change: 9.890 million.

## Fold LayerNorm backward into score-loss and FFN mlp2 epilogues

Fuses the final LayerNorm forward and backward into the packed score/loss kernel, which now normalizes the raw residual itself and writes dx directly. It also folds each block's LayerNorm backward into the mlp2 backward epilogue, accumulating dgamma and dbeta in shared memory. This removes the standalone layernorm_fwd/bwd launches and their intermediate activation round-trips. The cost is more shared memory and register pressure in both kernels, extra shuffle reductions, and bf16 rounding of the intermediate gradient.

```diff
diff --git a/include/srfrd_b200.h b/include/srfrd_b200.h
--- a/include/srfrd_b200.h
+++ b/include/srfrd_b200.h
@@ -8,7 +8,7 @@
 extern "C" {
 #endif
 
-#define SRFRD_ABI_VERSION 9
+#define SRFRD_ABI_VERSION 10
 #if defined(__GNUC__)
 #define SRFRD_API __attribute__((visibility("default")))
 #else
@@ -190,7 +190,9 @@
                                   const int64_t* pos, const int64_t* neg, const int64_t* prs, const int64_t* nrs,
                                   const float* w_pos, const float* w_neg, const float* norm, int D, int F,
                                   float* loss_acc, float* dh, int lddh, float* d_item, float* d_fake,
-                                  const int* row_tok, const int* rows_dev, int64_t cap_rows, void* stream);
+                                  const int* row_tok, const int* rows_dev, int64_t cap_rows, void* stream,
+                                  const void* ln_x, int ldx, const float* ln_w, const float* ln_b, float ln_eps,
+                                  const int64_t* ln_row_ids, void* dx, int lddx, float* ln_dw, float* ln_db);
 SRFRD_API int srfrd_embed_bwd_packed(const void* dx0_bf16, int ldx, const int64_t* seq, const int64_t* aux_ids,
                            const int* row_tok, const int* rows_dev, int64_t cap_rows, int L, int D, int F, int mode,
                            float item_scale, float* d_item, float* d_aux, float* d_pos, void* stream);
@@ -206,6 +208,7 @@
   void* mid_out; int ldm;
   void* out; int ldc;
   void* ln_out; int ld_ln; const float* ln_w; const float* ln_b; float* ln_stats; float ln_eps;
+  const void* lnb_x; int ldlx; const float* lnb_stats; const float* lnb_w; float* lnb_dw; float* lnb_db;
 } srfrd_mlp2_t;
 SRFRD_API int srfrd_mlp2_tn(const void* A_bf16, int lda, const void* W1_bf16, int ldw1, const void* W2_bf16, int ldw2, int M, int N,
                   const srfrd_mlp2_t* ep, void* stream);
diff --git a/srfrd_b200/_lib.py b/srfrd_b200/_lib.py
--- a/srfrd_b200/_lib.py
+++ b/srfrd_b200/_lib.py
@@ -25,7 +25,8 @@
     _fields_ = [("bias1", vp), ("bias2", vp), ("gate", vp), ("ldg", i32), ("relu1", i32), ("drop1_p", f32), ("drop2_p", f32),
                 ("drop1_stream", u32), ("drop2_stream", u32), ("drop_seed", u64), ("drop_step", vp), ("residual", vp), ("ldr", i32),
                 ("residual_is_a", i32), ("row_ids", vp), ("mid_out", vp), ("ldm", i32), ("out", vp), ("ldc", i32),
-                ("ln_out", vp), ("ld_ln", i32), ("ln_w", vp), ("ln_b", vp), ("ln_stats", vp), ("ln_eps", f32)]
+                ("ln_out", vp), ("ld_ln", i32), ("ln_w", vp), ("ln_b", vp), ("ln_stats", vp), ("ln_eps", f32),
+                ("lnb_x", vp), ("ldlx", i32), ("lnb_stats", vp), ("lnb_w", vp), ("lnb_dw", vp), ("lnb_db", vp)]
 
 
 class PackDesc(C.Structure):
@@ -94,7 +95,7 @@
     "srfrd_attention_bwd_packed": [vp, i32, vp, i32, vp, vp, i32, vp, i32, vp, vp, i32, C.POINTER(PackDesc), i32, i32, i32,
                                    f32, u64, u32, vp, vp, vp, i32, vp, i32],
     "srfrd_score_loss_fused_packed": [vp, i32, vp, vp, vp, vp, vp, vp, vp, vp, vp, i32, i32, vp, vp, i32, vp, vp, vp, vp,
-                                      i64, vp],
+                                      i64, vp, vp, i32, vp, vp, f32, vp, vp, i32, vp, vp],
     "srfrd_embed_bwd_packed": [vp, i32, vp, vp, vp, vp, i64, i32, i32, i32, i32, f32, vp, vp, vp, vp],
     "srfrd_sample_candidates": [vp, vp, vp, vp, i64, i32, i32, u64, vp, vp],
     "srfrd_candidate_rank": [vp, i32, vp, i64, i32, vp, i64, i32, vp, i32, vp, vp, i32, vp, vp, vp],
@@ -122,7 +123,7 @@
         fn = getattr(lib, name)
         fn.argtypes = argtypes
         fn.restype = C.c_int
-    if lib.srfrd_abi_version() != 9:
+    if lib.srfrd_abi_version() != 10:
         raise RuntimeError("srfrd_b200: ABI version mismatch between _lib.py and the built library")
     _lib = lib
     return lib
diff --git a/srfrd_b200/csrc/ffn.cu b/srfrd_b200/csrc/ffn.cu
--- a/srfrd_b200/csrc/ffn.cu
+++ b/srfrd_b200/csrc/ffn.cu
@@ -24,6 +24,7 @@
   int residual_is_a;
   const int64_t* row_ids;
   const float *ln_w, *ln_b; float* ln_stats; float ln_eps; int has_ln;
+  const bf16* lnb_x; int ldlx; const float* lnb_stats; float *lnb_dw, *lnb_db; int has_lnb;
 };
 
 __device__ __forceinline__ uint32_t swz_chunk(int r, int j) { return (uint32_t)(r * 128 + ((j ^ (r & 7)) << 4)); }
@@ -55,7 +56,9 @@
   float* sb2 = sb1 + 128;
   float* slw = sb2 + 128;
   float* slb = slw + 128;
-  uint64_t* bars = reinterpret_cast<uint64_t*>(slb + 128);
+  float* sdw = slb + 128;
+  float* sdb = sdw + 4 * 128;
+  uint64_t* bars = reinterpret_cast<uint64_t*>(sdb + 4 * 128);
   uint64_t *w_full = bars, *a_full = bars + 1, *a_free = bars + 2, *acc1_full = bars + 3, *mid_ready = bars + 4,
            *acc2_full = bars + 5;
   uint32_t* tmem_slot = reinterpret_cast<uint32_t*>(bars + 6);
@@ -76,9 +79,10 @@
   for (int i = threadIdx.x; i < 128; i += blockDim.x) {
     sb1[i] = (p.bias1 && i < p.N) ? __ldg(p.bias1 + i) : 0.f;
     sb2[i] = (p.bias2 && i < p.N) ? __ldg(p.bias2 + i) : 0.f;
-    slw[i] = (p.has_ln && i < p.N) ? __ldg(p.ln_w + i) : 0.f;
+    slw[i] = ((p.has_ln | p.has_lnb) && i < p.N) ? __ldg(p.ln_w + i) : 0.f;
     slb[i] = (p.has_ln && i < p.N) ? __ldg(p.ln_b + i) : 0.f;
   }
+  for (int i = threadIdx.x; i < 4 * 128; i += blockDim.x) sdw[i] = sdb[i] = 0.f;
   tc_fence_before();
   __syncthreads();
   tc_fence_after();
@@ -180,6 +184,13 @@
       }
       }
       const float rowm = (p.row_ids && rok) ? ((__ldg(p.row_ids + row) != 0) ? 1.f : 0.f) : 1.f;
+      float2 bst = make_float2(0.f, 0.f);
+      if (p.has_lnb && rok) bst = __ldg(reinterpret_cast<const float2*>(p.lnb_stats + 2 * row));
+      const float brstd = bst.y, bnb = -bst.x * bst.y;
+      if (p.has_lnb) {
+        if (issuer) asm volatile("cp.async.bulk.wait_group.read 0;" ::: "memory");
+        mlp_bar_sync();
+      }
       mbar_wait(acc2_full, ph);
       tc_fence_after();
       float ln_sum = 0.f, ln_sq = 0.f;
@@ -197,6 +208,11 @@
           const uint4* rp = reinterpret_cast<const uint4*>(p.residual + row * p.ldr + c);
           r0 = __ldg(rp); r1 = __ldg(rp + 1);
         }
+        uint4 x0 = make_uint4(0, 0, 0, 0), x1 = x0;
+        if (p.has_lnb && rok) {
+          const uint4* xp = reinterpret_cast<const uint4*>(p.lnb_x + row * p.ldlx + c);
+          x0 = __ldg(xp); x1 = __ldg(xp + 1);
+        }
         uint4 q0 = make_uint4(0, 0, 0, 0), q1 = q0;
         if (p.gate2 && rok) {
           const uint4* gp = reinterpret_cast<const uint4*>(p.gate2 + row * p.ldg2 + c);
@@ -225,6 +241,62 @@
           unpack8_bf16(p0, q); unpack8_bf16(p1, q + 8);
 #pragma unroll
           for (int i = 0; i < 16; ++i) { ln_sum += q[i]; ln_sq = fmaf(q[i], q[i], ln_sq); }
+        }
+        if (p.has_lnb) {
+          uint8_t* xs = sM + (c >> 6) * MBLK;
+          *reinterpret_cast<uint4*>(xs + swz_chunk(r, j)) = x0;
+          *reinterpret_cast<uint4*>(xs + swz_chunk(r, j + 1)) = x1;
+          float q[16], xv[16], cw[16], cb[16];
+          unpack8_bf16(p0, q); unpack8_bf16(p1, q + 8);
+          unpack8_bf16(x0, xv); unpack8_bf16(x1, xv + 8);
+#pragma unroll
+          for (int i = 0; i < 16; ++i) {
+            const float dy = rok ? q[i] : 0.f;
+            const float xh = fmaf(xv[i], brstd, bnb);
+            const float g = dy * slw[c + i];
+            ln_sum += g;
+            ln_sq = fmaf(g, xh, ln_sq);
+            cw[i] = dy * xh;
+            cb[i] = dy;
+          }
+#pragma unroll
+          for (int o = 16, n = 8; o >= 2; o >>= 1, n >>= 1) {
+            const bool up = (lane & o) != 0;
+#pragma unroll
+            for (int i = 0; i < n; ++i) {
+              const float sw_ = up ? cw[i] : cw[i + n], sb_ = up ? cb[i] : cb[i + n];
+              const float kw = up ? cw[i + n] : cw[i], kb = up ? cb[i + n] : cb[i];
+              cw[i] = kw + __shfl_xor_sync(0xffffffffu, sw_, o);
+              cb[i] = kb + __shfl_xor_sync(0xffffffffu, sb_, o);
+            }
+          }
+          cw[0] += __shfl_xor_sync(0xffffffffu, cw[0], 1);
+          cb[0] += __shfl_xor_sync(0xffffffffu, cb[0], 1);
+          if (!(lane & 1)) {
+            const int col = warp * 128 + c + ((lane >> 4) & 1) * 8 + ((lane >> 3) & 1) * 4 + ((lane >> 2) & 1) * 2 + ((lane >> 1) & 1);
+            sdw[col] += cw[0];
+            sdb[col] += cb[0];
+          }
+        }
+      }
+      if (p.has_lnb) {
+        const float invn = 1.f / (float)p.N;
+        const float sg = ln_sum * invn, sgx = ln_sq * invn;
+#pragma unroll 1
+        for (int c = 0; c < p.N; c += 8) {
+          const uint32_t off = (c >> 6) * MBLK + swz_chunk(r, (c & 63) >> 3);
+          uint8_t* ptr = sA + off;
+          const uint4 dv = *reinterpret_cast<const uint4*>(ptr);
+          const uint4 xr = *reinterpret_cast<const uint4*>(sM + off);
+          float q[8], xv[8], o[8];
+          unpack8_bf16(dv, q); unpack8_bf16(xr, xv);
+#pragma unroll
+          for (int i = 0; i < 8; ++i) {
+            const float xh = fmaf(xv[i], brstd, bnb);
+            o[i] = brstd * fmaf(-sgx, xh, fmaf(q[i], slw[c + i], -sg));
+          }
+          *reinterpret_cast<uint4*>(ptr) =
+              make_uint4(pack_bf16x2(o[0], o[1]), pack_bf16x2(o[2], o[3]), pack_bf16x2(o[4], o[5]), pack_bf16x2(o[6], o[7]));
         }
       }
       tc_fence_before();
@@ -260,6 +332,14 @@
       }
     }
     if (issuer) asm volatile("cp.async.bulk.wait_group 0;" ::: "memory");
+    if (p.has_lnb && (int)blockIdx.x < n_tiles) {
+      mlp_bar_sync();
+      const int i = threadIdx.x;
+      if (i < p.N) {
+        red_add_f32(p.lnb_dw + i, (sdw[i] + sdw[128 + i]) + (sdw[256 + i] + sdw[384 + i]));
+        red_add_f32(p.lnb_db + i, (sdb[i] + sdb[128 + i]) + (sdb[256 + i] + sdb[384 + i]));
+      }
+    }
   }
   tc_fence_before();
   __syncthreads();
@@ -274,6 +354,7 @@
                       int ldm, void* out, int ldc, void* ln_out, int ld_ln, cudaStream_t stream) {
   p.kb = (p.N + 63) / 64; p.kbk = (p.K + 63) / 64; p.rows_dev = row_limit();
   p.has_ln = ln_out != nullptr;
+  p.has_lnb = p.lnb_x != nullptr;
   CUtensorMap tmA, tmW1, tmW2, tmMid, tmOut, tmLn;
   if (int rc = make_tmap_bf16_2d(&tmA, A, p.M, p.K, lda, MT, 64)) return rc;
   if (int rc = make_tmap_bf16_2d(&tmW1, W1, p.N, p.K, ldw1, p.N, 64)) return rc;
@@ -287,7 +368,7 @@
   if (p.has_ln) if (int rc = make_tmap_bf16_2d(&tmLn, ln_out, p.M, p.N, ld_ln, MT, 64)) return rc;
   const int wblk = (p.N * 128 + 1023) & ~1023;
   const int ablk = p.kb > p.kbk ? p.kb : p.kbk;
-  const size_t smem = 1024 + (size_t)(p.kbk + (p.single ? 0 : p.kb)) * wblk + (size_t)(ablk + p.kb) * MBLK + 4 * 128 * sizeof(float) + 128;
+  const size_t smem = 1024 + (size_t)(p.kbk + (p.single ? 0 : p.kb)) * wblk + (size_t)(ablk + p.kb) * MBLK + 12 * 128 * sizeof(float) + 128;
   static bool attr = false;
   if (!attr) {
     SRFRD_CUDA(cudaFuncSetAttribute(mlp2_kernel, cudaFuncAttributeMaxDynamicSharedMemorySize, 200 * 1024));
@@ -339,6 +420,9 @@
   SRFRD_REQUIRE(!ep->gate || (ep->ldg % 8 == 0 && ((uintptr_t)ep->gate & 15) == 0), "mlp2_tn: bad gate");
   SRFRD_REQUIRE(!ep->residual || (ep->ldr % 8 == 0 && ((uintptr_t)ep->residual & 15) == 0), "mlp2_tn: bad residual");
   SRFRD_REQUIRE(!ep->ln_out || (ep->ln_w && ep->ln_b && ep->ld_ln % 8 == 0 && ep->ld_ln >= N), "mlp2_tn: bad LayerNorm arguments");
+  SRFRD_REQUIRE(!ep->lnb_x || (!ep->ln_out && ep->lnb_stats && ep->lnb_w && ep->lnb_dw && ep->lnb_db && ep->ldlx % 8 == 0 &&
+                                ep->ldlx >= N && ((uintptr_t)ep->lnb_x & 15) == 0),
+                "mlp2_tn: bad LayerNorm-backward arguments");
   SRFRD_REQUIRE(ep->drop1_p >= 0.f && ep->drop1_p < 1.f && ep->drop2_p >= 0.f && ep->drop2_p < 1.f, "mlp2_tn: dropout p must be in [0, 1)");
   MlpParams p = {};
   p.M = M; p.N = N; p.K = N; p.single = 0;
@@ -353,5 +437,9 @@
   if (p.residual_is_a) p.residual = nullptr;
   p.row_ids = ep->row_ids;
   p.ln_w = ep->ln_w; p.ln_b = ep->ln_b; p.ln_stats = ep->ln_stats; p.ln_eps = ep->ln_eps;
+  if (ep->lnb_x) {
+    p.lnb_x = (const bf16*)ep->lnb_x; p.ldlx = ep->ldlx; p.lnb_stats = ep->lnb_stats; p.ln_w = ep->lnb_w;
+    p.lnb_dw = ep->lnb_dw; p.lnb_db = ep->lnb_db;
+  }
   return mlp_launch(p, A, lda, W1, ldw1, W2, ldw2, ep->mid_out, ep->ldm, ep->out, ep->ldc, ep->ln_out, ep->ld_ln, stream);
 }
diff --git a/srfrd_b200/csrc/loss_scatter_adam.cu b/srfrd_b200/csrc/loss_scatter_adam.cu
--- a/srfrd_b200/csrc/loss_scatter_adam.cu
+++ b/srfrd_b200/csrc/loss_scatter_adam.cu
@@ -22,14 +22,17 @@
   const int* row_tok;
   const int* rows_dev;
   int group;
+  const bf16* ln_x; int ldx; const float *ln_w, *ln_b; float ln_eps;
+  const int64_t* ln_row_ids; bf16* dx; int lddx; float *ln_dw, *ln_db;
 };
 
 __device__ __forceinline__ float softplus(float x) { return fmaxf(x, 0.f) + log1pf(__expf(-fabsf(x))); }
 __device__ __forceinline__ float sigmoidf(float x) { return 1.f / (1.f + __expf(-x)); }
 
-template <int NC>
+template <int NC, bool FOLD>
 __global__ void __launch_bounds__(256, (NC <= 9 ? 2 : 1)) score_kernel(ScoreParams p) {
   __shared__ float red[2][8];
+  __shared__ float sdw[FOLD ? 8 * 32 * NC : 1], sdb[FOLD ? 8 * 32 * NC : 1];
   pdl_prologue_done();
   const int lane = threadIdx.x & 31, warp = threadIdx.x >> 5, nw = blockDim.x >> 5;
   const int64_t warp0 = (int64_t)blockIdx.x * nw + warp, nwarps = (int64_t)gridDim.x * nw;
@@ -45,6 +48,16 @@
 #pragma unroll
   for (int i = 0; i < NC; ++i) fk1[i] = fk2[i] = 0.f;
   const bool dh_vec = p.dh && (p.lddh == W) && (W % 4 == 0) && ((reinterpret_cast<uintptr_t>(p.dh) & 15) == 0);
+  constexpr bool fold = FOLD;
+  const float invW = 1.f / (float)W;
+  float lw[NC], lb[NC], adw[NC], adb[NC];
+#pragma unroll
+  for (int i = 0; i < NC; ++i) {
+    const int c = lane + 32 * i;
+    lw[i] = (fold && c < W) ? __ldg(p.ln_w + c) : 0.f;
+    lb[i] = (fold && c < W) ? __ldg(p.ln_b + c) : 0.f;
+    adw[i] = adb[i] = 0.f;
+  }
   if (p.rows_dev) p.T = min(p.T, (int64_t)__ldg(p.rows_dev));
   const int G = p.group;
   for (int64_t t0 = warp0 * G; t0 < p.T; t0 += nwarps * G) {
@@ -54,6 +67,7 @@
     if (p.row_tok && in) { my_tok = __ldg(p.row_tok + tl); in = my_tok >= 0; }
     const int64_t my_src = p.row_tok ? (int64_t)my_tok : tl;
     int64_t my_pid = 0, my_nid = 0, my_pf = 0, my_nf = 0;
+    bool my_keep = true;
     float my_a = 0.f, my_b = 0.f;
     bool my_active = false;
     if (in) {
@@ -71,9 +85,18 @@
         my_active = true;
       }
       if (p.fake_table && my_active) { my_pf = __ldg(p.prs + my_src); my_nf = __ldg(p.nrs + my_src); }
-    }
+      if (fold && p.ln_row_ids && my_active) my_keep = __ldg(p.ln_row_ids + tl) != 0;
+    }
+    const unsigned keep_mask = __ballot_sync(0xffffffffu, my_keep);
     unsigned mask = __ballot_sync(0xffffffffu, my_active);
-    if (p.dh) {
+    if (fold) {
+      const int nrow = (int)min((int64_t)G, p.T - t0), per_row = W >> 3;
+      for (int i = lane; i < nrow * per_row; i += 32) {
+        const int r = i / per_row;
+        if (!((mask >> r) & 1u))
+          *reinterpret_cast<uint4*>(p.dx + (t0 + r) * p.lddx + (i - r * per_row) * 8) = make_uint4(0, 0, 0, 0);
+      }
+    } else if (p.dh) {
       const int nrow = (int)min((int64_t)G, p.T - t0);
       if (dh_vec) {
         const int per_row = W >> 2, total = nrow * per_row;
@@ -102,7 +125,7 @@
         const int c = lane + 32 * i;
         k.hv[i] = k.ep[i] = k.en[i] = 0.f;
         if (c < W) {
-          k.hv[i] = p.h[k.t * p.ldh + c];
+          k.hv[i] = fold ? __bfloat162float(p.ln_x[k.t * p.ldx + c]) : p.h[k.t * p.ldh + c];
           if (c < p.D) {
             k.ep[i] = __ldg(p.item_table + k.pid * p.D + c);
             k.en[i] = __ldg(p.item_table + k.nid * p.D + c);
@@ -113,7 +136,26 @@
         }
       }
     };
-    auto finish = [&](const Tok& k) {
+    auto finish = [&](Tok& k) {
+      float xh[NC], rstd = 0.f;
+      if (fold) {
+        float s1 = 0.f, s2 = 0.f;
+#pragma unroll
+        for (int i = 0; i < NC; ++i) { s1 += k.hv[i]; s2 = fmaf(k.hv[i], k.hv[i], s2); }
+#pragma unroll
+        for (int o = 16; o; o >>= 1) {
+          s1 += __shfl_xor_sync(0xffffffffu, s1, o);
+          s2 += __shfl_xor_sync(0xffffffffu, s2, o);
+        }
+        const float mean = s1 * invW;
+        rstd = rsqrtf(fmaxf(s2 * invW - mean * mean, 0.f) + p.ln_eps);
+        const float nb = -mean * rstd;
+#pragma unroll
+        for (int i = 0; i < NC; ++i) {
+          xh[i] = lane + 32 * i < W ? fmaf(k.hv[i], rstd, nb) : 0.f;
+          k.hv[i] = lane + 32 * i < W ? fmaf(xh[i], lw[i], lb[i]) : 0.f;
+        }
+      }
       float sp = 0.f, sn = 0.f;
 #pragma unroll
       for (int i = 0; i < NC; ++i) { sp = fmaf(k.hv[i], k.ep[i], sp); sn = fmaf(k.hv[i], k.en[i], sn); }
@@ -142,6 +184,31 @@
           }
         }
       }
+      if (fold) {
+        float dy[NC], sg = 0.f, sgx = 0.f;
+#pragma unroll
+        for (int i = 0; i < NC; ++i) {
+          dy[i] = lane + 32 * i < W ? dzp * k.ep[i] + dzn * k.en[i] : 0.f;
+          const float g = dy[i] * lw[i];
+          adw[i] = fmaf(dy[i], xh[i], adw[i]);
+          adb[i] += dy[i];
+          sg += g;
+          sgx = fmaf(g, xh[i], sgx);
+        }
+#pragma unroll
+        for (int o = 16; o; o >>= 1) {
+          sg += __shfl_xor_sync(0xffffffffu, sg, o);
+          sgx += __shfl_xor_sync(0xffffffffu, sgx, o);
+        }
+        sg *= invW;
+        sgx *= invW;
+        const float keep = ((keep_mask >> (k.t - t0)) & 1u) ? 1.f : 0.f;
+#pragma unroll
+        for (int i = 0; i < NC; ++i) {
+          const int c = lane + 32 * i;
+          if (c < W) p.dx[k.t * p.lddx + c] = __float2bfloat16_rn(rstd * fmaf(-sgx, xh[i], fmaf(dy[i], lw[i], -sg)) * keep);
+        }
+      }
     };
     if (NC <= 4) {
       if (mask) {
@@ -173,6 +240,17 @@
         if (fk1[i] != 0.f) red_add_f32(p.d_fake + 1 * p.F + (c - p.D), fk1[i]);
         if (fk2[i] != 0.f) red_add_f32(p.d_fake + 2 * p.F + (c - p.D), fk2[i]);
       }
+    }
+  }
+  if (fold) {
+#pragma unroll
+    for (int i = 0; i < NC; ++i) { sdw[warp * 32 * NC + lane + 32 * i] = adw[i]; sdb[warp * 32 * NC + lane + 32 * i] = adb[i]; }
+    __syncthreads();
+    for (int c = threadIdx.x; c < W; c += blockDim.x) {
+      float a = 0.f, b = 0.f;
+      for (int w = 0; w < nw; ++w) { a += sdw[w * 32 * NC + c]; b += sdb[w * 32 * NC + c]; }
+      red_add_f32(p.ln_dw + c, a);
+      red_add_f32(p.ln_db + c, b);
     }
   }
   if (p.mode == 1 && p.loss_acc) {
@@ -526,14 +604,21 @@
   const int64_t cap = (int64_t)num_sms() * 8;
   if (blocks > cap) blocks = cap;
   const int nc = (W + 31) / 32;
-#define SCORE_CALL(NC) SRFRD_CUDA(launch_pdl(score_kernel<NC>, dim3((unsigned)blocks), dim3(256), 0, (cudaStream_t)stream, p))
-  if (nc <= 1) SCORE_CALL(1);
-  else if (nc <= 2) SCORE_CALL(2);
-  else if (nc <= 3) SCORE_CALL(3);
-  else if (nc <= 4) SCORE_CALL(4);
-  else if (nc <= 6) SCORE_CALL(6);
-  else if (nc <= 9) SCORE_CALL(9);
-  else SCORE_CALL(MAXC);
+#define SCORE_CALL(NC, FOLD) \
+  SRFRD_CUDA(launch_pdl(score_kernel<NC, FOLD>, dim3((unsigned)blocks), dim3(256), 0, (cudaStream_t)stream, p))
+  if (p.ln_x) {
+    SRFRD_REQUIRE(nc <= 4, "score: final-LayerNorm fold needs a width <= 128 (got %d)", W);
+    if (nc <= 2) SCORE_CALL(2, true);
+    else if (nc <= 3) SCORE_CALL(3, true);
+    else SCORE_CALL(4, true);
+  }
+  else if (nc <= 1) SCORE_CALL(1, false);
+  else if (nc <= 2) SCORE_CALL(2, false);
+  else if (nc <= 3) SCORE_CALL(3, false);
+  else if (nc <= 4) SCORE_CALL(4, false);
+  else if (nc <= 6) SCORE_CALL(6, false);
+  else if (nc <= 9) SCORE_CALL(9, false);
+  else SCORE_CALL(MAXC, false);
 #undef SCORE_CALL
   SRFRD_LAUNCH_CHECK();
   return 0;
@@ -582,14 +667,25 @@
                                              const int64_t* pos, const int64_t* neg, const int64_t* prs, const int64_t* nrs,
                                              const float* w_pos, const float* w_neg, const float* norm, int D, int F,
                                              float* loss_acc, float* dh, int lddh, float* d_item, float* d_fake,
-                                             const int* row_tok, const int* rows_dev, int64_t cap_rows, void* stream) {
-  SRFRD_REQUIRE(h && item_table && pos && neg && norm && loss_acc && row_tok && rows_dev, "score_loss_fused_packed: null pointer");
+                                             const int* row_tok, const int* rows_dev, int64_t cap_rows, void* stream,
+                                             const void* ln_x, int ldx, const float* ln_w, const float* ln_b, float ln_eps,
+                                             const int64_t* ln_row_ids, void* dx, int lddx, float* ln_dw, float* ln_db) {
+  SRFRD_REQUIRE((ln_x || h) && item_table && pos && neg && norm && loss_acc && row_tok && rows_dev,
+                "score_loss_fused_packed: null pointer");
+  SRFRD_REQUIRE(!ln_x || (ln_w && ln_b && dx && ln_dw && ln_db && (D + (fake_table ? F : 0)) % 8 == 0 && lddx % 8 == 0 &&
+                          ((uintptr_t)dx & 15) == 0),
+                "score_loss_fused_packed: bad final-LayerNorm arguments (width and dx pitch must be multiples of 8)");
   SRFRD_REQUIRE(!fake_table || (prs && nrs), "score_loss_fused_packed: fake ids required with a fake table");
   ScoreParams p = {};
   p.h = h; p.ldh = ldh; p.item_table = item_table; p.fake_table = fake_table; p.pos = pos; p.neg = neg; p.prs = prs;
   p.nrs = nrs; p.w_pos = w_pos; p.w_neg = w_neg; p.norm = norm; p.T = cap_rows; p.D = D; p.F = F;
   p.loss_acc = loss_acc; p.dh = dh; p.lddh = lddh; p.d_item = d_item; p.d_fake = d_fake; p.mode = 1;
   p.row_tok = row_tok; p.rows_dev = rows_dev; p.group = 8;
+  if (ln_x) {
+    p.h = nullptr; p.dh = nullptr;
+    p.ln_x = (const bf16*)ln_x; p.ldx = ldx; p.ln_w = ln_w; p.ln_b = ln_b; p.ln_eps = ln_eps; p.ln_row_ids = ln_row_ids;
+    p.dx = (bf16*)dx; p.lddx = lddx; p.ln_dw = ln_dw; p.ln_db = ln_db;
+  }
   return score_launch(p, stream);
 }
 
diff --git a/srfrd_b200/engine.py b/srfrd_b200/engine.py
--- a/srfrd_b200/engine.py
+++ b/srfrd_b200/engine.py
@@ -334,13 +334,15 @@
 
     def forward(self, seq: torch.Tensor, fake_ids: Optional[torch.Tensor], training: bool,
                 last_only: bool = False, save: Optional[bool] = None, packed: bool = False,
-                keep: Optional[torch.Tensor] = None) -> torch.Tensor:
+                keep: Optional[torch.Tensor] = None, final_ln: bool = True) -> torch.Tensor:
         s, P = self.spec, self.P
         B, L = seq.shape
         if L > s.max_len:
             raise RuntimeError(f"sequence length {L} exceeds max_len {s.max_len} (pos_embed rows, SRFR_model.py:12)")
         if packed:
-            return self._forward_packed(seq, fake_ids, training, last_only, save, keep)
+            return self._forward_packed(seq, fake_ids, training, last_only, save, keep, final_ln)
+        if not final_ln:
+            raise ValueError("final_ln=False needs the packed layout")
         T, H, Hp, nb = B * L, s.H, s.Hp, s.num_blocks
         ws = self._workspace(T, L)
         self.fwd_version += 1
@@ -411,7 +413,7 @@
                               version=self.fwd_version)
         return hfin.view(B, L, s.Doutp)[..., :s.Dout]
 
-    def backward(self, dh: torch.Tensor, version: Optional[int] = None) -> None:
+    def backward(self, dh: Optional[torch.Tensor], version: Optional[int] = None, final_ln_done: bool = False) -> None:
         s, P, sv = self.spec, self.P, self.saved
         if sv is None:
             raise RuntimeError("backward() without a training forward()")
@@ -420,7 +422,9 @@
                                "predict) ran on this model after the one being back-propagated and overwrote the shared "
                                "activation workspace; run backward() before the next forward()")
         if sv.get("plan") is not None:
-            return self._backward_packed(dh)
+            return self._backward_packed(dh, final_ln_done)
+        if final_ln_done:
+            raise ValueError("final_ln_done needs the packed layout")
         B, L = sv["B"], sv["L"]
         T, H, Hp, nb = B * L, s.H, s.Hp, s.num_blocks
         ws = self._ws
@@ -496,7 +500,7 @@
         self._join()
         self.saved = None
 
-    def _forward_packed(self, seq, fake_ids, training, last_only, save, keep):
+    def _forward_packed(self, seq, fake_ids, training, last_only, save, keep, final_ln=True):
         s, P = self.spec, self.P
         B, L = seq.shape
         H, Hp, nb = s.H, s.Hp, s.num_blocks
@@ -587,7 +591,7 @@
             if s.kind == "SRFR":
                 ops.gemm_tn(x[nb], self.sh["wc"], out_bf16=ws["c"][:T], bias=self.bias("bc"))
                 fin_in = ws["c"][:T]
-            if not last_only:
+            if not last_only and final_ln:
                 ops.layernorm_fwd(fin_in, P.view("last_layernorm.weight"), P.view("last_layernorm.bias"), LN_EPS,
                                   y_f32=ws["hfin"][:T], stats=ws["stF"][:T], H=s.Dout)
         if last_only:
@@ -598,7 +602,23 @@
         if training if save is None else save:
             self.saved = dict(seq=seq, aux_ids=aux_ids, B=B, L=L, p_drop=p_drop, seed=seed, step=step,
                               version=self.fwd_version, plan=plan, hyb=hyb, live=live)
-        return ws["hfin"][:T]
+        return ws["hfin"][:T] if final_ln else fin_in
+
+    def fold_ln(self, B: int, L: int) -> bool:
+        s = self.spec
+        return (self.packed_mode(B, L) == "tile" and s.Hp <= 128 and self.fuse_ffn
+                and os.environ.get("SRFRD_FUSE_LN", "1") != "0")
+
+    def final_ln_fold(self) -> dict:
+        s, P, ws, plan = self.spec, self.P, self._ws, self.saved["plan"]
+        T, nb = plan.cap, s.num_blocks
+        if s.kind == "SRFR":
+            x, dx, rid = ws["c"][:T], ws["gc"][:T], None
+        else:
+            x, dx, rid = ws[f"x{nb}"][:T], ws[f"gdz_{nb - 1}"][:T], plan.row_ids
+        return dict(ln_x=x, ln_w=P.view("last_layernorm.weight"), ln_b=P.view("last_layernorm.bias"), ln_eps=LN_EPS,
+                    ln_row_ids=rid, dx=dx, ln_dw=P.view("last_layernorm.weight", grad=True),
+                    ln_db=P.view("last_layernorm.bias", grad=True))
 
     def _fuse_oproj(self, hyb, L, fuse_ln) -> int:
         s = self.spec
@@ -606,7 +626,7 @@
             return 0
         return ops.attention_packed_oproj_supported(L, s.H, s.num_heads)
 
-    def _backward_packed(self, dh: torch.Tensor) -> None:
+    def _backward_packed(self, dh: Optional[torch.Tensor], final_ln_done: bool = False) -> None:
         s, P, sv = self.spec, self.P, self.saved
         plan, hyb, live = sv["plan"], sv.get("hyb"), sv.get("live")
         B, L = sv["B"], sv["L"]
@@ -620,15 +640,17 @@
         x = [ws[f"x{i}"][:T] for i in range(nb + 1)]
         dz_top = ws[f"gdz_{nb - 1}"][:T]
         fuse_oproj = self._fuse_oproj(hyb, L, Hp <= 128 and os.environ.get("SRFRD_FUSE_LN", "1") != "0") & 2
+        fold_ln = self.fold_ln(B, L)
         with ops.row_limit(plan.rows):
             if s.kind == "SRFR":
                 gc = ws["gc"][:T]
-                ops.layernorm_bwd(dh, ws["c"][:T], ws["stF"][:T], P.view("last_layernorm.weight"), gc,
-                                  G("last_layernorm.weight"), G("last_layernorm.bias"), H=s.D)
+                if not final_ln_done:
+                    ops.layernorm_bwd(dh, ws["c"][:T], ws["stF"][:T], P.view("last_layernorm.weight"), gc,
+                                      G("last_layernorm.weight"), G("last_layernorm.bias"), H=s.D)
                 with self._branch():
                     ops.gemm_wgrad(gc, x[nb], GM("last_conv.weight"), G("last_conv.bias"), Mo=s.D, No=H)
                 ops.gemm_tn(gc, self.sh["wcT"], out_bf16=dz_top, row_ids=row_ids)
-            else:
+            elif not final_ln_done:
                 ops.layernorm_bwd(dh, x[nb], ws["stF"][:T], P.view("last_layernorm.weight"), dz_top,
                                   G("last_layernorm.weight"), G("last_layernorm.bias"), row_ids=row_ids, H=s.Dout)
             for i in reversed(range(nb)):
@@ -641,7 +663,15 @@
                     ops.dropout_apply(dz, dz2, Hp, p_drop, seed, 12 + 4 * i, step)
                 with self._branch():
                     ops.gemm_wgrad(dz2, h1, GM(f"forward_layers.{i}.conv2.weight"), G(f"forward_layers.{i}.conv2.bias"), Mo=H, No=H)
-                if self.fuse_ffn and Hp <= 128:
+                if fold_ln:
+                    ops.mlp2_tn(dz2, self.sh[f"w2T{i}"], self.sh[f"w1T{i}"], da1, dr, gate=h1, drop1_p=p_drop,
+                                drop1_stream=11 + 4 * i, drop_seed=seed, drop_step=step, residual=dz, lnb_x=r,
+                                lnb_stats=ws[f"st2_{i}"][:T], lnb_w=P.view(f"forward_layernorms.{i}.weight"),
+                                lnb_dw=G(f"forward_layernorms.{i}.weight"), lnb_db=G(f"forward_layernorms.{i}.bias"))
+                    with self._branch():
+                        ops.gemm_wgrad(da1, y, GM(f"forward_layers.{i}.conv1.weight"), G(f"forward_layers.{i}.conv1.bias"),
+                                       Mo=H, No=H)
+                elif self.fuse_ffn and Hp <= 128:
                     ops.mlp2_tn(dz2, self.sh[f"w2T{i}"], self.sh[f"w1T{i}"], da1, gC, gate=h1, drop1_p=p_drop,
                                 drop1_stream=11 + 4 * i, drop_seed=seed, drop_step=step, residual=dz)
                     with self._branch():
@@ -654,8 +684,9 @@
                         ops.gemm_wgrad(da1, y, GM(f"forward_layers.{i}.conv1.weight"), G(f"forward_layers.{i}.conv1.bias"),
                                        Mo=H, No=H)
                     ops.gemm_tn(da1, self.sh[f"w1T{i}"], out_bf16=gC, residual=dz)
-                ops.layernorm_bwd(gC, r, ws[f"st2_{i}"][:T], P.view(f"forward_layernorms.{i}.weight"), dr,
-                                  G(f"forward_layernorms.{i}.weight"), G(f"forward_layernorms.{i}.bias"), H=H)
+                if not fold_ln:
+                    ops.layernorm_bwd(gC, r, ws[f"st2_{i}"][:T], P.view(f"forward_layernorms.{i}.weight"), dr,
+                                      G(f"forward_layernorms.{i}.weight"), G(f"forward_layernorms.{i}.bias"), H=H)
                 with self._branch():
                     ops.gemm_wgrad(dr, o, GM(f"attention_layers.{i}.out_proj.weight"),
                                    G(f"attention_layers.{i}.out_proj.bias"), Mo=H, No=H)
diff --git a/srfrd_b200/ops.py b/srfrd_b200/ops.py
--- a/srfrd_b200/ops.py
+++ b/srfrd_b200/ops.py
@@ -402,12 +402,15 @@
 
 
 def score_loss_fused_packed(h, item_table, fake_table, pos, neg, prs, nrs, w_pos, w_neg, norm, loss_acc, dh, d_item, d_fake,
-                            plan: PackedPlan):
+                            plan: PackedPlan, ln_x=None, ln_w=None, ln_b=None, ln_eps=0.0, ln_row_ids=None, dx=None,
+                            ln_dw=None, ln_db=None):
     D = item_table.shape[1]
     F = 0 if fake_table is None else fake_table.shape[1]
-    call("srfrd_score_loss_fused_packed", _p(h), h.stride(0), _p(item_table), _p(fake_table), _p(pos), _p(neg), _p(prs),
-         _p(nrs), _p(w_pos), _p(w_neg), _p(norm), D, F, _p(loss_acc), _p(dh), dh.stride(0), _p(d_item), _p(d_fake),
-         _p(plan.row_tok), _p(plan.rows), plan.cap, _stream())
+    st = lambda t: 0 if t is None else t.stride(0)
+    call("srfrd_score_loss_fused_packed", _p(h), st(h), _p(item_table), _p(fake_table), _p(pos), _p(neg), _p(prs),
+         _p(nrs), _p(w_pos), _p(w_neg), _p(norm), D, F, _p(loss_acc), _p(dh), st(dh), _p(d_item), _p(d_fake),
+         _p(plan.row_tok), _p(plan.rows), plan.cap, _stream(), _p(ln_x), st(ln_x), _p(ln_w), _p(ln_b), float(ln_eps),
+         _p(ln_row_ids), _p(dx), st(dx), _p(ln_dw), _p(ln_db))
 
 
 def embed_bwd_packed(dx0, seq, aux_ids, plan: PackedPlan, D, F, mode, item_scale, d_item, d_aux, d_pos):
@@ -444,7 +447,8 @@
 
 def mlp2_tn(A, W1, W2, mid_out, out, bias1=None, bias2=None, gate=None, relu1=False, drop1_p=0.0, drop2_p=0.0, drop1_stream=0,
             drop2_stream=0, drop_seed=0, drop_step=None, residual=None, residual_is_a=False, row_ids=None, ln_out=None,
-            ln_w=None, ln_b=None, ln_stats=None, ln_eps=0.0, M=None):
+            ln_w=None, ln_b=None, ln_stats=None, ln_eps=0.0, M=None, lnb_x=None, lnb_stats=None, lnb_w=None, lnb_dw=None,
+            lnb_db=None):
     _lib.require_device()
     M = A.shape[0] if M is None else M
     N = W1.shape[0]
@@ -452,5 +456,6 @@
                       float(drop2_p), int(drop1_stream), int(drop2_stream), int(drop_seed), _p(drop_step), _p(residual),
                       0 if residual is None else residual.stride(0), int(residual_is_a), _p(row_ids), _p(mid_out),
                       mid_out.stride(0), _p(out), out.stride(0), _p(ln_out), 0 if ln_out is None else ln_out.stride(0),
-                      _p(ln_w), _p(ln_b), _p(ln_stats), float(ln_eps))
+                      _p(ln_w), _p(ln_b), _p(ln_stats), float(ln_eps), _p(lnb_x), 0 if lnb_x is None else lnb_x.stride(0),
+                      _p(lnb_stats), _p(lnb_w), _p(lnb_dw), _p(lnb_db))
     call("srfrd_mlp2_tn", _p(A), A.stride(0), _p(W1), W1.stride(0), _p(W2), W2.stride(0), M, N, C.byref(ep), _stream())
diff --git a/srfrd_b200/trainer.py b/srfrd_b200/trainer.py
--- a/srfrd_b200/trainer.py
+++ b/srfrd_b200/trainer.py
@@ -169,13 +169,20 @@
             if self._l2 is not None:
                 self._l2.launch(P.data)
         packed = self.packed and eng.packed_ok(B, L)
-        hidden = eng.forward(st["seq"], st["rsq"], training=True, packed=packed, keep=st["pos"] if packed else None)
+        fold = packed and eng.fold_ln(B, L)
+        hidden = eng.forward(st["seq"], st["rsq"], training=True, packed=packed, keep=st["pos"] if packed else None,
+                             final_ln=not fold)
         ws = eng._ws
         ft = eng.fake_table()
         torch.cuda.current_stream().wait_stream(self.comm)
         prs_ = st["prs"].view(-1) if ft is not None else None
         nrs_ = st["nrs"].view(-1) if ft is not None else None
-        if packed:
+        if fold:
+            ops.score_loss_fused_packed(None, P.view(s.item_key), ft, pos, neg, prs_, nrs_, w_pos, w_neg, norm, acc, None,
+                                        P.view(s.item_key, grad=True), eng.fake_table_grad(), eng.saved["plan"],
+                                        **eng.final_ln_fold())
+            eng.backward(None, final_ln_done=True)
+        elif packed:
             plan = eng.saved["plan"]
             Tp = plan.cap
             ops.score_loss_fused_packed(ws["hfin"][:Tp], P.view(s.item_key), ft, pos, neg, prs_, nrs_, w_pos, w_neg, norm, acc,
```

Result: faster. 10.10 million, median of 6 (+2.1%).
